# monoamine11231/Example-GUI-OpenCL-Raytracer

Measured on AMD Instinct MI355X. Metric: Mrays/s at 1920x1080 depth 4, aggregate over n_gpus; rays = path segments + shadow rays as the reference casts them (value_traced: only those the kernel really traces), higher is better.
Workload: dtype f32; 1 GPU; C2: scenes/render.map (regenerated), camera raypng.c:17-21, 1920x1080, depth 4, 2 soft-shadow samples, 4x256^2 textures + 4096x3072 skybox (procedural); frame=1920x1080, arithmetic=fast

## Files before the change

### example_gui_opencl_raytracer_amd/api.py

```python
from __future__ import annotations

import ctypes as C
import os

import numpy as np

HERE = os.path.dirname(os.path.abspath(__file__))
LIB_PATH = os.environ.get("CLWRAP_LIB") or os.path.join(HERE, "libopencl_wrap_hip.so")

MAX_KERNELS = 16
MAX_BUFFERS = 32

CL_DEVICE_TYPE_GPU = 1 << 2
CL_MEM_READ_WRITE = 1 << 0
CL_MEM_WRITE_ONLY = 1 << 1
CL_MEM_READ_ONLY = 1 << 2
CL_MEM_COPY_HOST_PTR = 1 << 5

SYMBOLS = [
    "cl_wrap_init", "cl_wrap_load_global_data", "cl_wrap_load_single_data", "cl_wrap_load_images",
    "cl_wrap_output", "cl_wrap_release",
    "clw_ext_set_depth", "clw_ext_get_depth", "clw_ext_set_strict", "clw_ext_set_fuse",
    "clw_ext_set_id_offset", "clw_ext_set_row_bands", "clw_ext_set_async", "clw_ext_sync", "clw_ext_set_stream",
    "clw_ext_timing_reset", "clw_ext_timing_get", "clw_ext_set_timing_every", "clw_ext_set_pipeline", "clw_ext_load_images_raw",
    "clw_ext_bind_device_buffer", "clw_ext_device_ptr", "clw_ext_set_debug_rgb",
    "clw_ext_enable_counters", "clw_ext_read_counters", "clw_ext_set_tile_sched", "clw_ext_read_tile_costs", "clw_ext_unit", "clw_ext_set_grid", "clw_ext_set_variant",
    "clw_ext_last_trace_flags", "clw_ext_set_shadow_through", "clw_ext_set_tpt", "clw_ext_invalidate_scene", "clw_ext_read_counters_ex", "clw_ext_unit_scene",
    "clw_host_perspective", "clw_host_write_png", "clw_host_write_png_rgba", "clw_host_read_png",
    "clw_host_free", "clw_ext_version",
    "clw_ext_set_supersample", "clw_ext_get_supersample",
    "clw_ext_set_sample_cameras", "clw_ext_get_sample_cameras", "clw_ext_set_lens", "clw_host_lens_cameras", "clw_host_shutter_cameras",
    "clw_ext_set_sphere_motion", "clw_ext_get_sample_times", "clw_host_sample_times", "clw_host_spheres_at",
    "clw_ext_set_adaptive", "clw_ext_get_adaptive", "clw_ext_read_refine_mask", "clw_host_refine_mask",
    "clw_ext_set_seed_offset", "clw_ext_get_seed_offset", "clw_ext_set_accumulate", "clw_ext_get_accumulated", "clw_ext_reset_accumulation",
    "clw_host_frame_seed", "clw_host_jitter_camera",
    "clw_ext_set_split", "clw_ext_get_split", "clw_ext_get_tpt", "clw_ext_read_tile_order", "clw_ext_unit_sched",
    "clw_ext_render_gbuffer", "clw_ext_read_gbuffer", "clw_ext_gbuffer_device_ptr", "clw_ext_pick",
    "clw_ext_get_grid", "clw_ext_set_grid_pair",
    "clw_host_overlay", "clw_ext_render_overlay", "clw_ext_read_overlay", "clw_ext_overlay_device_ptr", "clw_ext_unit_overlay",
    "clw_host_object_stats", "clw_host_merge_object_stats", "clw_ext_object_stats", "clw_ext_unit_object_stats",
    "clw_host_projection_rays", "clw_host_projection_tables", "clw_host_ortho_camera",
    "clw_ext_set_projection", "clw_ext_get_projection", "clw_ext_unit_projection",
    "clw_host_ao_dirs", "clw_host_ao_open", "clw_host_ao_resolve", "clw_ext_render_ao", "clw_ext_read_ao", "clw_ext_ao_device_ptr",
    "clw_ext_unit_ao_open", "clw_ext_unit_ao_resolve",
    "clw_host_cast_rays", "clw_host_occluded_rays", "clw_ext_cast_rays", "clw_ext_occluded_rays", "clw_ext_cast_rays_device",
]

GB_DEPTH, GB_ID, GB_NORMAL, GB_POINT, GB_ALBEDO, GB_ALL = 1, 2, 4, 8, 16, 31
ID_NONE = 0xFFFFFFFF
ID_SPHERE, ID_PLANE, ID_LIGHT = 0, 1, 2
TIMING_GBUFFER = 0x47425546
GB_CHANNELS = {"depth": (GB_DEPTH, np.float32, 1), "id": (GB_ID, np.uint32, 1), "normal": (GB_NORMAL, np.float32, 3),
               "point": (GB_POINT, np.float32, 3), "albedo": (GB_ALBEDO, np.float32, 3)}

OV_OUTLINE, OV_FILL, OV_EDGES, OV_ALL = 1, 2, 4, 7
TIMING_OVERLAY = 0x4F564C59

OBJECT_STAT = np.dtype([("id", np.uint32), ("pixels", np.uint32), ("x0", np.uint32), ("y0", np.uint32), ("x1", np.uint32), ("y1", np.uint32),
                        ("depth_min", np.float32), ("depth_max", np.float32), ("sum_x", np.uint64), ("sum_y", np.uint64)])
TIMING_OBJECTS = 0x4F424A53

PROJ_PERSPECTIVE, PROJ_ORTHO, PROJ_EQUIRECT = 0, 1, 2
PROJ_MODELS = {"perspective": PROJ_PERSPECTIVE, "ortho": PROJ_ORTHO, "equirect": PROJ_EQUIRECT}

AO_FILTER, AO_COMPOSE = 1, 2
AO_FRAME, AO_COUNTS = 0, 1
TIMING_AO = 0x414F5452
TIMING_AO_RESOLVE = 0x414F5253

RAY_QUERY = np.dtype([("origin", np.float32, 3), ("tmax", np.float32), ("dir", np.float32, 3), ("ignore", np.uint32)])
HIT = np.dtype([("t", np.float32), ("id", np.uint32), ("normal", np.float32, 3), ("point", np.float32, 3)])
CAST_SPHERES, CAST_PLANES, CAST_LIGHTS, CAST_KINDS, CAST_OPAQUE = 1, 2, 4, 7, 8
CAST_KIND_NAMES = {"sphere": CAST_SPHERES, "plane": CAST_PLANES, "light": CAST_LIGHTS}
TIMING_CAST = 0x43415354


def id_kind(ids):
    return np.asarray(ids, np.uint32) >> np.uint32(30)


def id_index(ids):
    return np.asarray(ids, np.uint32) & np.uint32(0x3FFFFFFF)


def make_id(kind, index):
    return (np.asarray(kind, np.uint32) << np.uint32(30)) | np.asarray(index, np.uint32)


def library_version() -> str:
    return load_library().clw_ext_version().decode()


def kernel_source_hash() -> str:
    return library_version().rsplit("kernels:", 1)[-1]


class cl_wrap(C.Structure):
    _fields_ = [
        ("impl", C.c_void_p),
        ("kernels_num", C.c_uint32),
        ("buffers_num", C.c_uint32 * MAX_KERNELS),
        ("buffers_ids", (C.c_uint32 * MAX_BUFFERS) * MAX_KERNELS),
        ("buffers", (C.c_void_p * MAX_BUFFERS) * MAX_KERNELS),
    ]


class clw_camera(C.Structure):
    _fields_ = [("im_corner", C.c_float * 3), ("origin", C.c_float * 3), ("up", C.c_float * 3),
                ("right", C.c_float * 3), ("w_factor", C.c_float), ("h_factor", C.c_float),
                ("width", C.c_uint32), ("height", C.c_uint32)]


class clw_sample_camera(C.Structure):
    _fields_ = [("im_corner", C.c_float * 3), ("origin", C.c_float * 3), ("up", C.c_float * 3), ("right", C.c_float * 3)]


class clw_pick(C.Structure):
    _fields_ = [("id", C.c_uint32), ("depth", C.c_float), ("point", C.c_float * 3), ("normal", C.c_float * 3), ("albedo", C.c_float * 3)]


class clw_overlay(C.Structure):
    _fields_ = [("flags", C.c_uint32), ("radius", C.c_uint32), ("outline_rgb", C.c_uint32), ("fill_rgb", C.c_uint32), ("fill_alpha", C.c_uint32),
                ("edge_rgb", C.c_uint32)]


class clw_ao(C.Structure):
    _fields_ = [("flags", C.c_uint32), ("rays", C.c_uint32), ("radius", C.c_float), ("strength", C.c_uint32)]

# ... 108 lines not shown
        L.clw_ext_get_accumulated.argtypes = [W]
        L.clw_ext_get_accumulated.restype = u32
        L.clw_ext_reset_accumulation.argtypes = [W]
        L.clw_host_frame_seed.argtypes = [u32]
        L.clw_host_frame_seed.restype = u32
        L.clw_host_jitter_camera.argtypes = [C.POINTER(clw_camera), u32, u32, C.POINTER(clw_camera)]
        L.clw_host_jitter_camera.restype = C.c_int
    if hasattr(L, "clw_ext_render_gbuffer") or not os.environ.get("CLWRAP_LIB"):
        L.clw_ext_render_gbuffer.argtypes = [W, u32]
        L.clw_ext_render_gbuffer.restype = u32
        L.clw_ext_read_gbuffer.argtypes = [W, u32, vp, u32]
        L.clw_ext_read_gbuffer.restype = u32
        L.clw_ext_gbuffer_device_ptr.argtypes = [W, u32]
        L.clw_ext_gbuffer_device_ptr.restype = vp
        L.clw_ext_pick.argtypes = [W, u32, u32, C.POINTER(clw_pick)]
        L.clw_ext_pick.restype = C.c_int
    if hasattr(L, "clw_ext_get_grid") or not os.environ.get("CLWRAP_LIB"):
        L.clw_ext_get_grid.argtypes = [W, C.POINTER(clw_grid_info)]
        L.clw_ext_get_grid.restype = C.c_int
        L.clw_ext_set_grid_pair.argtypes = [W, C.c_int]
    if hasattr(L, "clw_ext_render_overlay") or not os.environ.get("CLWRAP_LIB"):
        OV = C.POINTER(clw_overlay)
        L.clw_host_overlay.argtypes = [vp, vp, u32, u32, OV, vp, u32, vp]
        L.clw_host_overlay.restype = C.c_int
        L.clw_ext_render_overlay.argtypes = [W, OV, vp, u32]
        L.clw_ext_render_overlay.restype = u32
        L.clw_ext_read_overlay.argtypes = [W, vp, u32]
        L.clw_ext_read_overlay.restype = u32
        L.clw_ext_overlay_device_ptr.argtypes = [W]
        L.clw_ext_overlay_device_ptr.restype = vp
        L.clw_ext_unit_overlay.argtypes = [W, vp, vp, u32, u32, OV, vp, u32, vp]
        L.clw_ext_unit_overlay.restype = u32
    if hasattr(L, "clw_ext_object_stats") or not os.environ.get("CLWRAP_LIB"):
        RC, SM = C.POINTER(clw_rect), C.POINTER(clw_object_summary)
        L.clw_host_object_stats.argtypes = [vp, vp, u32, u32, u32, RC, vp, vp, u32, SM]
        L.clw_host_object_stats.restype = C.c_int
        L.clw_host_merge_object_stats.argtypes = [vp, u32, vp, u32, vp, u32]
        L.clw_host_merge_object_stats.restype = u32
        L.clw_ext_object_stats.argtypes = [W, RC, vp, u32, SM]
        L.clw_ext_object_stats.restype = C.c_int
        L.clw_ext_unit_object_stats.argtypes = [W, vp, vp, u32, u32, u32, RC, vp, vp, u32, SM]
        L.clw_ext_unit_object_stats.restype = C.c_int
    if hasattr(L, "clw_ext_set_projection") or not os.environ.get("CLWRAP_LIB"):
        CM, PR = C.POINTER(clw_camera), C.POINTER(clw_projection)
        L.clw_host_projection_rays.argtypes = [CM, PR, C.c_uint64, C.c_uint64, vp]
        L.clw_host_projection_rays.restype = C.c_int
        L.clw_host_projection_tables.argtypes = [CM, PR, vp, vp]
        L.clw_host_projection_tables.restype = C.c_int
        L.clw_host_ortho_camera.argtypes = [C.c_float * 3, C.c_float * 3, C.c_float, u32, u32, CM, PR]
        L.clw_host_ortho_camera.restype = C.c_int
        L.clw_ext_set_projection.argtypes = [W, PR]
        L.clw_ext_get_projection.argtypes = [W, PR]
        L.clw_ext_unit_projection.argtypes = [W, CM, PR, C.c_uint64, C.c_uint64, vp]
        L.clw_ext_unit_projection.restype = C.c_int
    if hasattr(L, "clw_ext_render_ao") or not os.environ.get("CLWRAP_LIB"):
        AO = C.POINTER(clw_ao)
        L.clw_host_ao_dirs.argtypes = [u32, vp]
        L.clw_host_ao_dirs.restype = C.c_int
        L.clw_host_ao_open.argtypes = [vp, vp, vp, u32, u32, u32, vp, u32, vp, u32, AO, vp, vp]
        L.clw_host_ao_open.restype = C.c_int
        L.clw_host_ao_resolve.argtypes = [vp, vp, vp, u32, u32, AO, vp]
        L.clw_host_ao_resolve.restype = C.c_int
        L.clw_ext_render_ao.argtypes = [W, AO]
        L.clw_ext_render_ao.restype = u32
        L.clw_ext_read_ao.argtypes = [W, u32, vp, u32]
        L.clw_ext_read_ao.restype = u32
        L.clw_ext_ao_device_ptr.argtypes = [W, u32]
        L.clw_ext_ao_device_ptr.restype = vp
        L.clw_ext_unit_ao_open.argtypes = [W, vp, vp, vp, u32, u32, u32, AO, vp]
        L.clw_ext_unit_ao_open.restype = u32
        L.clw_ext_unit_ao_resolve.argtypes = [W, vp, vp, vp, u32, u32, AO, vp]
        L.clw_ext_unit_ao_resolve.restype = u32
    if hasattr(L, "clw_ext_cast_rays") or not os.environ.get("CLWRAP_LIB"):
        L.clw_host_cast_rays.argtypes = [vp, u32, u32, vp, u32, vp, u32, vp, u32, vp]
        L.clw_host_cast_rays.restype = C.c_int
        L.clw_host_occluded_rays.argtypes = [vp, u32, u32, vp, u32, vp, u32, vp, u32, vp]
        L.clw_host_occluded_rays.restype = C.c_int
        L.clw_ext_cast_rays.argtypes = [W, vp, u32, u32, vp]
        L.clw_ext_cast_rays.restype = u32
        L.clw_ext_occluded_rays.argtypes = [W, vp, u32, u32, vp]
        L.clw_ext_occluded_rays.restype = u32
        L.clw_ext_cast_rays_device.argtypes = [W, vp, u32, u32, vp, vp]
        L.clw_ext_cast_rays_device.restype = u32
    L.clw_ext_unit.argtypes = [W, C.c_int, vp, u32, vp, u32, u32, u32]
    L.clw_ext_read_tile_costs.argtypes = [W, vp, u32]
    L.clw_ext_read_tile_costs.restype = u32
    L.clw_ext_set_split.argtypes = [W, C.c_int, C.c_int]
    L.clw_ext_get_split.argtypes = [W, C.POINTER(u32), C.POINTER(u32), C.POINTER(u32)]
    L.clw_ext_get_tpt.argtypes = [W, C.POINTER(u32), C.POINTER(u32), C.POINTER(u32)]
    L.clw_ext_read_tile_order.argtypes = [W, vp, u32, C.POINTER(u32)]
    L.clw_ext_read_tile_order.restype = u32
    L.clw_ext_unit_sched.argtypes = [W, vp, u32, u32, C.c_int, u32, u32, u32, u32, vp, u32]
    L.clw_ext_unit_sched.restype = u32
    L.clw_ext_read_counters.argtypes = [W, C.POINTER(C.c_uint64 * 8)]
    L.clw_ext_read_counters_ex.argtypes = [W, C.POINTER(C.c_uint64 * 32), u32]
    L.clw_ext_invalidate_scene.argtypes = [W]
    L.clw_ext_unit_scene.argtypes = [W, u32, C.c_int, vp, u32, vp, u32, u32]
    L.clw_host_perspective.argtypes = [C.c_float * 3, C.c_float * 3, C.c_float, C.c_float, u32, u32,
                                       C.POINTER(clw_camera)]
    L.clw_host_perspective.restype = C.c_int
    L.clw_host_write_png.argtypes = [C.c_char_p, vp, u32, u32]
    L.clw_host_write_png.restype = C.c_int
    L.clw_host_write_png_rgba.argtypes = [C.c_char_p, vp, u32, u32]
    L.clw_host_write_png_rgba.restype = C.c_int
    L.clw_host_read_png.argtypes = [C.c_char_p, C.POINTER(u32), C.POINTER(u32), C.POINTER(vp)]
    L.clw_host_read_png.restype = C.c_int
    L.clw_host_free.argtypes = [vp]
    L.clw_ext_version.restype = C.c_char_p
    _lib = L
    return L


def _ptr(a):
    if a is None:
        return None
    if isinstance(a, np.ndarray):
        return a.ctypes.data_as(C.c_void_p)
    return C.cast(a, C.c_void_p)


def perspective(origin, look, fov, focal, width, height) -> clw_camera:
    L = load_library()
    cam = clw_camera()
    ok = L.clw_host_perspective((C.c_float * 3)(*origin), (C.c_float * 3)(*look), fov, focal, width, height,
                                C.byref(cam))
    if not ok:
        raise ValueError("rgen_perspective rejects this camera (cpu_ray.c:58-63)")
    return cam


def lens_cameras(cam: clw_camera, aperture: float, focus: float, n: int) -> np.ndarray:
    out = np.zeros((max(int(n), 0) ** 2 or 1, 12), np.float32)
    if not load_library().clw_host_lens_cameras(C.byref(cam), aperture, focus, n, _ptr(out)):
        raise ValueError("clw_host_lens_cameras rejects these arguments (n in 2, 4, 8; aperture >= 0; focus > 0)")
    return out


def shutter_cameras(cam0: clw_camera, cam1: clw_camera, n: int) -> np.ndarray:
    out = np.zeros((max(int(n), 0) ** 2 or 1, 12), np.float32)
    if not load_library().clw_host_shutter_cameras(C.byref(cam0), C.byref(cam1), n, _ptr(out)):
        raise ValueError("clw_host_shutter_cameras rejects these arguments (n in 2, 4, 8; cameras of one size and one pair of factors)")
    return out


def sample_times(n: int) -> np.ndarray:
    out = np.zeros(max(int(n), 0) ** 2 or 1, np.float32)
    if not load_library().clw_host_sample_times(n, _ptr(out)):
        raise ValueError("clw_host_sample_times rejects this factor (n in 2, 4, 8)")
    return out


def spheres_at(spheres: np.ndarray, disp, t: float) -> np.ndarray:
    spheres = np.ascontiguousarray(spheres)
    assert spheres.dtype.itemsize == 96
    disp = np.ascontiguousarray(disp, np.float32).reshape(-1, 3)
    assert len(disp) == len(spheres)
    out = spheres.copy()
    if not load_library().clw_host_spheres_at(_ptr(spheres), len(spheres), _ptr(disp), float(t), _ptr(out)):
        raise ValueError("clw_host_spheres_at rejects these arguments")
    return out


def refine_mask(xrgb, width: int, rows: int, n: int, threshold: int) -> np.ndarray:
    xrgb = np.ascontiguousarray(xrgb, np.uint32).reshape(-1)
    width, rows, n = int(width), int(rows), int(n)
    if n not in (2, 4, 8) or width <= 0 or rows <= 0 or xrgb.size != width * rows:
# ... 33 lines not shown
def ao_dirs(rays: int) -> np.ndarray:
    out = np.empty((16, max(int(rays), 0), 4), np.float32)
    if not 0 <= int(rays) < 2 ** 32 or not load_library().clw_host_ao_dirs(int(rays), _ptr(out)):
        raise ValueError("clw_host_ao_dirs rejects this number of rays (1..32)")
    return out


def ao_open(point, normal, ids, width: int, rows: int, first_row: int, spheres, planes, ao: clw_ao, dirs=None) -> np.ndarray:
    width, rows = int(width), int(rows)
    point = np.ascontiguousarray(point, np.float32).reshape(-1)
    normal = np.ascontiguousarray(normal, np.float32).reshape(-1)
    ids = np.ascontiguousarray(ids, np.uint32).reshape(-1)
    if width <= 0 or rows <= 0 or ids.size != width * rows or point.size != 3 * ids.size or normal.size != 3 * ids.size:
        raise ValueError("clw_host_ao_open rejects these arguments (point and normal of 3, ids of 1 entry per pixel of width * rows)")
    if dirs is None:
        dirs = ao_dirs(ao.rays)
    dirs = np.ascontiguousarray(dirs, np.float32)
    ns, np_ = (0 if spheres is None else len(spheres)), (0 if planes is None else len(planes))
    out = np.empty(ids.size, np.uint8)
    if dirs.size != 64 * ao.rays or not load_library().clw_host_ao_open(_ptr(point), _ptr(normal), _ptr(ids), width, rows, int(first_row),
                                                                        _ptr(spheres) if ns else None, ns, _ptr(planes) if np_ else None, np_,
                                                                        C.byref(ao), _ptr(dirs), _ptr(out)):
        raise ValueError("clw_host_ao_open rejects these parameters (rays in 1..32, radius > 0, strength in 0..256, known flags)")
    return out


def ao_resolve(open_u8, ids, frame, width: int, rows: int, ao: clw_ao) -> np.ndarray:
    width, rows = int(width), int(rows)
    open_u8 = np.ascontiguousarray(open_u8, np.uint8).reshape(-1)
    ids = np.ascontiguousarray(ids, np.uint32).reshape(-1)
    if frame is not None:
        frame = np.ascontiguousarray(frame, np.uint32).reshape(-1)
    if width <= 0 or rows <= 0 or open_u8.size != width * rows or ids.size != width * rows or (frame is not None and frame.size != width * rows):
        raise ValueError("clw_host_ao_resolve rejects these arguments (counts, ids and frame of width * rows entries each)")
    out = np.empty(width * rows, np.uint32)
    if not load_library().clw_host_ao_resolve(_ptr(open_u8), _ptr(ids), _ptr(frame), width, rows, C.byref(ao), _ptr(out)):
        raise ValueError("clw_host_ao_resolve rejects these parameters (rays in 1..32, radius > 0, strength in 0..256, known flags, a frame with AO_COMPOSE)")
    return out


def cast_flags(kinds=("sphere", "plane"), opaque_only: bool = False) -> int:
    if isinstance(kinds, (int, np.integer)):
        flags = int(kinds)
    else:
        flags = 0
        for k in kinds:
            flags |= CAST_KIND_NAMES[k]
    return flags | (CAST_OPAQUE if opaque_only else 0)


def make_rays(origins, dirs, tmax=np.inf, ignore=None) -> np.ndarray:
    origins = np.asarray(origins, np.float32).reshape(-1, 3)
    rays = np.empty(origins.shape[0], RAY_QUERY)
    rays["origin"] = origins
    rays["dir"] = np.asarray(dirs, np.float32).reshape(-1, 3)
    rays["tmax"] = np.asarray(tmax, np.float32)
    rays["ignore"] = ID_NONE if ignore is None else np.asarray(ignore, np.uint32)
    return rays


def _cast_args(rays, spheres, planes, lights):
    rays = np.ascontiguousarray(rays, RAY_QUERY).reshape(-1)
    arrs = [None if a is None else np.ascontiguousarray(a) for a in (spheres, planes, lights)]
    counts = [0 if a is None else int(a.shape[0]) for a in arrs]
    return rays, arrs, counts


def cast_rays_host(rays, flags: int, spheres, planes, lights=None) -> np.ndarray:
    rays, (s, p, l), (ns, np_, nl) = _cast_args(rays, spheres, planes, lights)
    out = np.empty(rays.size, HIT)
    if not 0 <= int(flags) < 2 ** 32 or not load_library().clw_host_cast_rays(_ptr(rays), rays.size, int(flags), _ptr(s), ns, _ptr(p), np_, _ptr(l), nl, _ptr(out)):
        raise ValueError("clw_host_cast_rays rejects these arguments (at least one ray, fewer than 2^30, a kind bit and only CAST_* bits in flags)")
    return out


def occluded_rays_host(rays, flags: int, spheres, planes, lights=None) -> np.ndarray:
    rays, (s, p, l), (ns, np_, nl) = _cast_args(rays, spheres, planes, lights)
    out = np.empty(rays.size, np.uint8)
    if not 0 <= int(flags) < 2 ** 32 or not load_library().clw_host_occluded_rays(_ptr(rays), rays.size, int(flags), _ptr(s), ns, _ptr(p), np_, _ptr(l), nl, _ptr(out)):
        raise ValueError("clw_host_occluded_rays rejects these arguments (at least one ray, fewer than 2^30, a kind bit and only CAST_* bits in flags)")
    return out


def _rect(rect):
    if rect is None:
        return None
    if not isinstance(rect, clw_rect):
        rect = clw_rect(*(int(v) for v in rect))
    return C.byref(rect)


def _summary(s: clw_object_summary) -> dict:
    return dict(objects=int(s.objects), pixels=int(s.pixels), foreign=int(s.foreign))


def _object_table(call, first_capacity: int = 16384):
    s = clw_object_summary()
    out = np.zeros(first_capacity, OBJECT_STAT)
    if not call(_ptr(out), out.size, C.byref(s)):
        return None
    if s.objects > out.size:
        out = np.zeros(s.objects, OBJECT_STAT)
        if not call(_ptr(out), out.size, C.byref(s)):
            return None
    return out[:min(s.objects, out.size)].copy(), _summary(s)


def object_stats(ids, depth, width: int, rows: int, counts, first_row: int = 0, rect=None):
    ids = np.ascontiguousarray(ids, np.uint32).reshape(-1)
    width, rows = int(width), int(rows)
    if width <= 0 or rows <= 0 or ids.size != width * rows:
        raise ValueError("clw_host_object_stats rejects these arguments (an id channel of width * rows words)")
    if depth is not None:
        depth = np.ascontiguousarray(depth, np.float32).reshape(-1)
        if depth.size != ids.size:
            raise ValueError("clw_host_object_stats rejects these arguments (a depth channel of width * rows words)")
    counts = np.ascontiguousarray(counts, np.uint32).reshape(3)
    L = load_library()
    got = _object_table(lambda out, cap, s: L.clw_host_object_stats(_ptr(ids), _ptr(depth), width, rows, int(first_row), _rect(rect), _ptr(counts),
                                                                    out, cap, s))
    if got is None:
        raise ValueError("clw_host_object_stats rejects these arguments (an empty rectangle, more than 2^24 - 1 primitives, 2^30 pixels or more)")
    return got


def merge_object_stats(a, b) -> np.ndarray:
    a, b = np.ascontiguousarray(a, OBJECT_STAT).reshape(-1), np.ascontiguousarray(b, OBJECT_STAT).reshape(-1)
    out = np.zeros(a.size + b.size or 1, OBJECT_STAT)
    n = load_library().clw_host_merge_object_stats(_ptr(a), a.size, _ptr(b), b.size, _ptr(out), out.size)
    return out[:n].copy()


def projection(model, axis=None, ortho_width: float = 0.0, span=(360.0, 180.0)) -> clw_projection:
    p = clw_projection()
    p.model = PROJ_MODELS[model] if isinstance(model, str) else int(model)
    if axis is not None:
        p.axis[:] = [float(v) for v in axis]
    p.ortho_width, p.h_span, p.v_span = float(ortho_width), float(span[0]), float(span[1])
    return p


def projection_rays(cam: clw_camera, proj: clw_projection, id_begin: int = 0, id_end: int | None = None) -> np.ndarray:
    id_end = cam.width * cam.height if id_end is None else int(id_end)
    rays = np.zeros((max(id_end - int(id_begin), 0), 16), np.float32)
    if not load_library().clw_host_projection_rays(C.byref(cam), C.byref(proj), int(id_begin), id_end, _ptr(rays)):
        raise ValueError("clw_host_projection_rays rejects these arguments (model 0..2, a finite axis, ortho_width >= 0, spans in [0, 360] / "
                         "[0, 180], reserved 0, ids inside the frame)")
    return rays


def projection_tables(cam: clw_camera, proj: clw_projection):
    col, row = np.zeros((cam.width, 4), np.float32), np.zeros((cam.height, 4), np.float32)
    if not load_library().clw_host_projection_tables(C.byref(cam), C.byref(proj), _ptr(col), _ptr(row)):
        raise ValueError("clw_host_projection_tables rejects these arguments (an equirectangular projection the library accepts)")
    return col, row


def ortho_camera(origin, look, view_width: float, width: int, height: int):
    cam, proj = clw_camera(), clw_projection()
    if not load_library().clw_host_ortho_camera((C.c_float * 3)(*origin), (C.c_float * 3)(*look), float(view_width), int(width), int(height),
                                                C.byref(cam), C.byref(proj)):
        raise ValueError("clw_host_ortho_camera rejects these arguments (a finite look that is not vertical, view_width > 0, a frame)")
    return cam, proj


def frame_seed(f: int) -> int:
# ... 66 lines not shown

    def load_images(self, kernel_id, arg_id, *paths, mem_flags=CL_MEM_COPY_HOST_PTR):
        args = [C.c_char_p(p.encode()) for p in paths]
        self.L.cl_wrap_load_images(C.byref(self.w), C.c_uint32(kernel_id), C.c_uint32(arg_id),
                                   C.c_uint64(mem_flags), C.c_uint32(len(paths)), *args)

    def output(self, array_size, output_size, kernel_run_id, kernel_id, arg_id, host_output=None):
        self.L.cl_wrap_output(C.byref(self.w), array_size, output_size, kernel_run_id, kernel_id, arg_id,
                              _ptr(host_output))

    def release(self):
        if self.w.impl:
            self.L.cl_wrap_release(C.byref(self.w))

    def buffer_handle(self, kernel_id, arg_id) -> C.c_void_p:
        return C.c_void_p(self.w.buffers[kernel_id][arg_id])

    def set_depth(self, d): self.L.clw_ext_set_depth(C.byref(self.w), d)
    def get_depth(self): return self.L.clw_ext_get_depth(C.byref(self.w))
    def set_strict(self, s): self.L.clw_ext_set_strict(C.byref(self.w), int(s))
    def set_fuse(self, f): self.L.clw_ext_set_fuse(C.byref(self.w), int(f))
    def set_id_offset(self, first_id): self.L.clw_ext_set_id_offset(C.byref(self.w), first_id)
    def set_row_bands(self, stride, phase): self.L.clw_ext_set_row_bands(C.byref(self.w), stride, phase)
    def set_async(self, a): self.L.clw_ext_set_async(C.byref(self.w), int(a))
    def sync(self): self.L.clw_ext_sync(C.byref(self.w))
    def set_stream(self, s): self.L.clw_ext_set_stream(C.byref(self.w), C.c_void_p(s))
    def unit(self, op: int, rows: np.ndarray, out_cols: int, aux: int = 0) -> np.ndarray:
        rows = np.ascontiguousarray(rows, np.float32)
        out = np.zeros((rows.shape[0], out_cols), np.float32)
        self.L.clw_ext_unit(C.byref(self.w), op, _ptr(rows), rows.shape[1], _ptr(out), out_cols, rows.shape[0], aux)
        return out

    def read_tile_costs(self) -> np.ndarray:
        n = self.L.clw_ext_read_tile_costs(C.byref(self.w), None, 0)
        out = np.zeros(n, np.uint32)
        if n:
            self.L.clw_ext_read_tile_costs(C.byref(self.w), _ptr(out), n)
        return out

    def read_tile_order(self):
        cap = C.c_uint32()
        n = self.L.clw_ext_read_tile_order(C.byref(self.w), None, 0, C.byref(cap))
        out = np.zeros(n, np.uint32)
        if n:
            self.L.clw_ext_read_tile_order(C.byref(self.w), _ptr(out), n, C.byref(cap))
        return out, int(cap.value)

    def unit_sched(self, cost: np.ndarray, tpr: int, trows: int, clamp_outliers: int, per_share_cap: int, split_slots: int, min_quota: int,
                   max_lg: int) -> np.ndarray:
        cost = np.ascontiguousarray(cost, np.uint32).reshape(-1)
        assert cost.size == tpr * trows
        a = (int(tpr), int(trows), int(clamp_outliers), int(per_share_cap), int(split_slots), int(min_quota), int(max_lg))
        n = self.L.clw_ext_unit_sched(C.byref(self.w), _ptr(cost), *a, None, 0)
        out = np.zeros(n, np.uint32)
        self.L.clw_ext_unit_sched(C.byref(self.w), _ptr(cost), *a, _ptr(out), n)
        return out

    def get_split(self):
        v = [C.c_uint32() for _ in range(3)]
        self.L.clw_ext_get_split(C.byref(self.w), *[C.byref(x) for x in v])
        return tuple(int(x.value) for x in v)

    def get_tpt(self):
        v = [C.c_uint32() for _ in range(3)]
        self.L.clw_ext_get_tpt(C.byref(self.w), *[C.byref(x) for x in v])
        return tuple(int(x.value) for x in v)

    def set_split(self, slots=-1, min_quota=-1): self.L.clw_ext_set_split(C.byref(self.w), int(slots), int(min_quota))
    def set_shadow_through(self, f): self.L.clw_ext_set_shadow_through(C.byref(self.w), float(f))
    def set_grid(self, on): self.L.clw_ext_set_grid(C.byref(self.w), int(on))

    def get_grid(self):
        g = clw_grid_info()
        if not self.L.clw_ext_get_grid(C.byref(self.w), C.byref(g)):
            return None
        return dict(built=int(g.built), pair=int(g.pair), res=tuple(int(x) for x in g.res), ncells=int(g.ncells), pairs=int(g.pairs),
                    cell=tuple(float(x) for x in g.cell), gmin=tuple(float(x) for x in g.gmin), reg_pad=float(g.reg_pad))

    def set_grid_pair(self, on=-1):
        self.L.clw_ext_set_grid_pair(C.byref(self.w), int(on))
    def set_tile_sched(self, on): self.L.clw_ext_set_tile_sched(C.byref(self.w), int(on))
    def set_variant(self, v): self.L.clw_ext_set_variant(C.byref(self.w), int(v))
    def last_trace_flags(self): return int(self.L.clw_ext_last_trace_flags(C.byref(self.w)))
    def set_tpt(self, max_lanes=-1, min_paths=-1, pool_mb=-1): self.L.clw_ext_set_tpt(C.byref(self.w), int(max_lanes), int(min_paths), int(pool_mb))
    def timing_reset(self): self.L.clw_ext_timing_reset(C.byref(self.w))
    def set_timing_every(self, n): self.L.clw_ext_set_timing_every(C.byref(self.w), int(n))
    def set_pipeline(self, on): self.L.clw_ext_set_pipeline(C.byref(self.w), int(on))

    def timing_get(self, kernel_id):
        n, ms = C.c_uint32(), C.c_double()
        self.L.clw_ext_timing_get(C.byref(self.w), kernel_id, C.byref(n), C.byref(ms))
        return n.value, ms.value

    def load_images_raw(self, kernel_id, arg_id, rgba: np.ndarray):
        rgba = np.ascontiguousarray(rgba, np.uint8)
        layers, h, w, c = rgba.shape
        assert c == 4
        self.L.clw_ext_load_images_raw(C.byref(self.w), kernel_id, arg_id, _ptr(rgba), w, h, layers)

    def bind_device_buffer(self, kernel_id, arg_id, device_ptr, size):
        self.L.clw_ext_bind_device_buffer(C.byref(self.w), kernel_id, arg_id, C.c_void_p(device_ptr), size)

    def device_ptr(self, kernel_id, arg_id): return self.L.clw_ext_device_ptr(C.byref(self.w), kernel_id, arg_id)
    def set_debug_rgb(self, ptr): self.L.clw_ext_set_debug_rgb(C.byref(self.w), C.c_void_p(ptr))
    def set_supersample(self, n): self.L.clw_ext_set_supersample(C.byref(self.w), int(n))
    def get_supersample(self): return int(self.L.clw_ext_get_supersample(C.byref(self.w)))

    def set_seed_offset(self, s): self.L.clw_ext_set_seed_offset(C.byref(self.w), int(s) & 0xFFFFFFFF)
    def get_seed_offset(self): return int(self.L.clw_ext_get_seed_offset(C.byref(self.w)))
    def set_accumulate(self, max_frames, jitter=True): self.L.clw_ext_set_accumulate(C.byref(self.w), int(max_frames), int(jitter))
    def get_accumulated(self): return int(self.L.clw_ext_get_accumulated(C.byref(self.w)))
    def reset_accumulation(self): self.L.clw_ext_reset_accumulation(C.byref(self.w))

    def render_gbuffer(self, channels=GB_ALL) -> int:
        return int(self.L.clw_ext_render_gbuffer(C.byref(self.w), int(channels)))

    def _read_pass(self, read, dtype) -> np.ndarray:
        nbytes = int(read(None, 0))
        out = np.zeros(nbytes // np.dtype(dtype).itemsize, dtype)
        if nbytes:
            assert read(_ptr(out), nbytes) == nbytes
        return out

    def read_gbuffer(self, channel) -> np.ndarray:
        _, dtype, per = next(v for v in GB_CHANNELS.values() if v[0] == channel)
        out = self._read_pass(lambda p, cap: self.L.clw_ext_read_gbuffer(C.byref(self.w), int(channel), p, cap), dtype)
        return out.reshape(-1, 3) if per == 3 else out

    def gbuffer_device_ptr(self, channel):
        return self.L.clw_ext_gbuffer_device_ptr(C.byref(self.w), int(channel))

    def pick(self, x, y):
        p = clw_pick()
        return p if self.L.clw_ext_pick(C.byref(self.w), int(x), int(y), C.byref(p)) else None

    def render_overlay(self, style: clw_overlay, sel) -> int:
        sel = _selection(sel)
        return int(self.L.clw_ext_render_overlay(C.byref(self.w), C.byref(style), _ptr(sel) if sel.size else None, sel.size))

    def read_overlay(self) -> np.ndarray:
        return self._read_pass(lambda p, cap: self.L.clw_ext_read_overlay(C.byref(self.w), p, cap), np.uint32)

    def overlay_device_ptr(self):
        return self.L.clw_ext_overlay_device_ptr(C.byref(self.w))

    def unit_overlay(self, frame, ids, width: int, rows: int, style: clw_overlay, sel):
        frame = np.ascontiguousarray(frame, np.uint32).reshape(-1)
        ids = np.ascontiguousarray(ids, np.uint32).reshape(-1)
        assert frame.size == int(width) * int(rows) == ids.size
        sel = _selection(sel)
        out = np.empty(frame.size, np.uint32)
        n = self.L.clw_ext_unit_overlay(C.byref(self.w), _ptr(frame), _ptr(ids), int(width), int(rows), C.byref(style),
                                        _ptr(sel) if sel.size else None, sel.size, _ptr(out))
        return out if n == frame.size and n else None

    def object_stats(self, rect=None):
        return _object_table(lambda out, cap, s: self.L.clw_ext_object_stats(C.byref(self.w), _rect(rect), out, cap, s))

    def unit_object_stats(self, ids, depth, width: int, rows: int, counts, first_row: int = 0, rect=None):
        ids = np.ascontiguousarray(ids, np.uint32).reshape(-1)
        assert ids.size == int(width) * int(rows)
        if depth is not None:
            depth = np.ascontiguousarray(depth, np.float32).reshape(-1)
            assert depth.size == ids.size
        counts = np.ascontiguousarray(counts, np.uint32).reshape(3)
        return _object_table(lambda out, cap, s: self.L.clw_ext_unit_object_stats(C.byref(self.w), _ptr(ids), _ptr(depth), int(width), int(rows), int(first_row),
# ... 133 lines not shown
```

### example_gui_opencl_raytracer_amd/build.py

```python
from __future__ import annotations

import os
import shutil
import subprocess
import sys

HERE = os.path.dirname(os.path.abspath(__file__))
CSRC = os.path.join(HERE, "csrc")
ROOT_DIR = os.path.dirname(HERE)
OBJ = os.path.join(HERE, "build")
LIB = os.path.join(HERE, "libopencl_wrap_hip.so")
ARCH = "gfx950"

HIPCC = os.environ.get("HIPCC") or shutil.which("hipcc") or "/opt/rocm/bin/hipcc"
CC = os.environ.get("CC") or "gcc"

DEVICE_DEPS = ["whitted_trace.inc", "whitted_hit.inc", "whitted_shade.inc", "whitted_bounce.inc", "whitted_pop.inc", "whitted_tpt.inc", "whitted_terms.inc",
               "whitted_gbuffer.inc", "whitted_projection.inc", "whitted_ao.inc", "whitted_cast.inc", "whitted_overlay.inc", "whitted_objects.inc", "whitted_launch.inc", "whitted_launch.h", "whitted_params.h",
               "projection_host.h"]
SHIM_FLAGS = ["-O2", "-std=c++17", "-Wall"]
SHIM_DEPS = ["hip_wrap_impl.h", "whitted_params.h", "whitted_launch.h", "launch_plan.h", "scene_prep.h", "ao_host.h", "cast_host.h", "overlay_host.h", "objects_host.h", "projection_host.h",
             "png_codec.h", "../../include/opencl_wrap.h", "../../include/hip_wrap_ext.h"]
UNITS = [
    ("whitted_fast.hip", "hip", ["-O3", f"--offload-arch={ARCH}", "-fno-slp-vectorize", "-ffp-contract=off"], DEVICE_DEPS),
    ("whitted_strict.hip", "hip", ["-O3", f"--offload-arch={ARCH}", "-fno-slp-vectorize", "-ffp-contract=off"], DEVICE_DEPS),
    ("hip_wrap.cpp", "hip", SHIM_FLAGS, SHIM_DEPS),
    ("hip_wrap_passes.cpp", "hip", SHIM_FLAGS, SHIM_DEPS),
    ("scene_prep.c", "c", ["-O2", "-std=c99", "-ffp-contract=off", "-Wall", "-Wextra"], ["scene_prep.h"]),
    ("overlay_host.c", "c", ["-O2", "-std=c99", "-ffp-contract=off", "-Wall", "-Wextra"],
     ["overlay_host.h", "../../include/hip_wrap_ext.h", "../../include/opencl_wrap.h"]),
    ("ao_host.c", "c", ["-O2", "-std=c99", "-ffp-contract=off", "-Wall", "-Wextra", "-D_DEFAULT_SOURCE"],
     ["ao_host.h", "scene_prep.h", "../../include/hip_wrap_ext.h", "../../include/opencl_wrap.h"]),
    ("cast_host.c", "c", ["-O2", "-std=c99", "-ffp-contract=off", "-Wall", "-Wextra", "-D_DEFAULT_SOURCE"],
     ["cast_host.h", "scene_prep.h", "../../include/hip_wrap_ext.h", "../../include/opencl_wrap.h"]),
    ("objects_host.c", "c", ["-O2", "-std=c99", "-ffp-contract=off", "-Wall", "-Wextra"],
     ["objects_host.h", "../../include/hip_wrap_ext.h", "../../include/opencl_wrap.h"]),
    ("projection_host.c", "c", ["-O2", "-std=c99", "-ffp-contract=off", "-Wall", "-Wextra", "-D_DEFAULT_SOURCE"],
     ["projection_host.h", "../../include/hip_wrap_ext.h", "../../include/opencl_wrap.h"]),
    ("launch_plan.c", "c", ["-O2", "-std=c99", "-ffp-contract=off", "-Wall", "-Wextra"],
     ["launch_plan.h", "whitted_params.h", "../../include/hip_wrap_ext.h", "../../include/opencl_wrap.h"]),
    ("host_camera.c", "c", ["-O2", "-std=c99", "-ffp-contract=off", "-Wall", "-Wextra", "-D_DEFAULT_SOURCE"],
     ["../../include/hip_wrap_ext.h", "../../include/opencl_wrap.h"]),
    ("png_codec.c", "c", ["-O2", "-std=c99", "-D_DEFAULT_SOURCE", "-pthread", "-Wall", "-Wextra"], ["png_codec.h"]),
]


def kernel_source_hash() -> str:
    import hashlib
    h = hashlib.sha256()
    for f in sorted(set(DEVICE_DEPS + ["whitted_fast.hip", "whitted_strict.hip"])):
        h.update(f.encode() + b"\0" + open(os.path.join(CSRC, f), "rb").read())
    h.update(" ".join(UNITS[0][2]).encode())
    return h.hexdigest()[:16]


def _newer(target: str, deps) -> bool:
    if not os.path.exists(target):
        return True
    t = os.path.getmtime(target)
    return any(os.path.getmtime(d) > t for d in deps if os.path.exists(d))


def build(force: bool = False, verbose: bool = False, tag: str = "", extra_device_flags=()) -> str:
    os.makedirs(OBJ, exist_ok=True)
    objs = []
    lib = LIB if not tag else LIB.replace(".so", f"{tag}.so")
    for src, kind, flags, deps in UNITS:
        spath = os.path.join(CSRC, src)
        opath = os.path.join(OBJ, src.rsplit(".", 1)[0] + tag + ".o")
        if src.endswith(".hip"):
            flags = flags + list(extra_device_flags)
        if src == "hip_wrap.cpp":
            flags = flags + [f'-DWT_SOURCE_HASH="{kernel_source_hash()}{tag}"']
            deps = deps + DEVICE_DEPS + ["whitted_fast.hip", "whitted_strict.hip"]
        objs.append(opath)
        dpaths = [spath, __file__] + [os.path.normpath(os.path.join(CSRC, d)) for d in deps]
        if not force and not _newer(opath, dpaths):
            continue
        cmd = ([HIPCC] if kind == "hip" else [CC]) + flags + ["-fPIC", "-c", spath, "-o", opath]
        if verbose:
            print(" ".join(cmd), flush=True)
        subprocess.run(cmd, check=True)
    if force or _newer(lib, objs):
        cmd = [HIPCC, "-shared", "-o", lib] + objs + ["-lz", "-lpthread", "-Wl,-rpath,/opt/rocm/lib"]
        if verbose:
            print(" ".join(cmd), flush=True)
        subprocess.run(cmd, check=True)
    if not tag:
        exe = os.path.join(ROOT_DIR, "tools", "raybench")
        src = os.path.join(ROOT_DIR, "tools", "raybench.c")
        if force or _newer(exe, [src, lib]):
            cmd = [CC, "-O2", "-std=c99", "-D_DEFAULT_SOURCE", "-DCL_TARGET_OPENCL_VERSION=300", "-Wall", "-I", os.path.join(ROOT_DIR, "include"),
                   src, "-o", exe, "-L", HERE, "-lopencl_wrap_hip", "-Wl,-rpath,$ORIGIN/../example_gui_opencl_raytracer_amd",
                   "-Wl,-rpath,/opt/rocm/lib"]
            if verbose:
                print(" ".join(cmd), flush=True)
            subprocess.run(cmd, check=True)
    return lib


if __name__ == "__main__":
    print(build(force="--force" in sys.argv, verbose=True))
```

### example_gui_opencl_raytracer_amd/csrc/hip_wrap.cpp

```cpp
#include "hip_wrap_impl.h"

using namespace clw;

namespace clw {
[[noreturn]] void die(const char* fmt, ...) {
    va_list ap;
    va_start(ap, fmt);
    printf("ERROR:\t");
    vprintf(fmt, ap);
    printf("\n");
    va_end(ap);
    fflush(stdout);
    exit(1);
}
}

namespace {

constexpr size_t COUNTER_WORDS = CLW_NUM_COUNTERS + 16 * (size_t)CLW_STAMP_SHARDS;
constexpr size_t GRID_MAX_PAIRS = (size_t)1 << 25;

bool same_bits(const std::vector<float>& a, const float* b, size_t n) {
    return a.size() == n && (n == 0 || !memcmp(a.data(), b, n * sizeof(float)));
}
// ... 363 lines not shown
        }
        I->tables_in_flight = true;
        plan.P.ss_times = I->d_motion; plan.P.ss_disp = I->d_motion + 64;
    }
}

void bind_accumulation(Impl* I, wt_plan_out& plan) {
    Impl::Accum& A = I->acc;
    if (!plan.fused || A.frame < 0) return;
    if (A.pixels != (size_t)plan.out_pixels || !A.sum) {
        if (A.frame != 0) die("Couldn't run the kernel");
        if (A.sum) { finish(I); (void)hipFree(A.sum); A.sum = nullptr; }
        HIP_OK(hipMalloc((void**)&A.sum, (size_t)plan.out_pixels * 12), "Couldn't allocate device memory");
        A.pixels = plan.out_pixels;
    }
    wait_tables_fence(I);
    I->tables_in_flight = true;
    plan.P.acc_sum = A.sum;
}

void bind_counters(Impl* I, wt_plan_out& plan) {
    if (!plan.need_counters) return;
    if (!I->d_counters) {
        HIP_OK(hipMalloc((void**)&I->d_counters, COUNTER_WORDS * sizeof(unsigned long long)), "Couldn't allocate device memory");
        HIP_OK(hipMemsetAsync(I->d_counters, 0, COUNTER_WORDS * sizeof(unsigned long long), I->stream), "Couldn't allocate device memory");
    }
    plan.P.counters = I->d_counters;
}

void classify_blocks(Impl* I, wt_plan_out& plan) {
    whitted_params& P = plan.P;
    const uint32_t ow = P.width >> P.ss_lg, orows = P.rows >> P.ss_lg;
    Impl::Adaptive& A = I->adapt;
    if (A.w != ow || A.rows != orows || A.ss != plan.ss || !A.mask) {
        A.free_all();
        HIP_OK(hipMalloc((void**)&A.mask, (size_t)plan.trows * plan.tpr), "Couldn't allocate device memory");
        HIP_OK(hipMalloc((void**)&A.order, (size_t)plan.grid * 4), "Couldn't allocate device memory");
        HIP_OK(hipMalloc((void**)&A.count, 8 * WT_LIST_COUNT_STRIDE * 4), "Couldn't allocate device memory");
        A.w = ow; A.rows = orows; A.ss = plan.ss;
    }
    wait_tables_fence(I);
    HIP_OK(hipMemsetAsync(A.count, 0, 8 * WT_LIST_COUNT_STRIDE * 4, I->stream), "Couldn't run the kernel");
    if (wt_fast_launch_classify(P.out, ow, orows, 3u - P.ss_lg, (unsigned)I->adaptive, A.mask, A.order, A.count, plan.per_share, I->stream) != hipSuccess)
        die("Couldn't run the kernel");
    I->tables_in_flight = true;
    A.blocks = plan.trows * plan.tpr;
    P.tile_order = A.order; P.list_count = A.count;
}

bool bind_tile_order(Impl* I, Impl::Sched& S, wt_plan_out& plan, const Strip* strip) {
    whitted_params& P = plan.P;
    if (!strip) S.last_rd = -1;
    if (!plan.use_order) return false;
    const size_t ntiles = (size_t)plan.trows * plan.tpr;
    if (S.w != P.width || S.rows != P.rows || S.cap != plan.per_share_cap || S.ss != plan.ss || !S.cost[0]) {
        S.free_all();
        for (int i = 0; i < 2; i++) {
            HIP_OK(hipMalloc((void**)&S.cost[i], ntiles * 4), "Couldn't allocate device memory");
            HIP_OK(hipMalloc((void**)&S.order[i], (size_t)plan.grid * 4), "Couldn't allocate device memory");
            HIP_OK(hipEventCreateWithFlags(&S.built[i], hipEventDisableTiming), "Couldn't create a timing event");
        }
        HIP_OK(hipEventCreateWithFlags(&S.traced, hipEventDisableTiming), "Couldn't create a timing event");
        S.w = P.width; S.rows = P.rows; S.cap = plan.per_share_cap; S.ss = plan.ss; S.o.wr = 0;
    }
    const int wr = S.o.wr;
    P.tile_cost = S.cost[wr];
    const wt_order_choice c = wt_order_choose(&S.o);
    if (c.wait_wr) HIP_OK(hipStreamWaitEvent(I->stream, S.built[wr], 0), "Couldn't run the kernel");
    if (c.wait_rd) HIP_OK(hipStreamWaitEvent(I->stream, S.built[c.rd], 0), "Couldn't run the kernel");
    P.tile_order = c.rd >= 0 ? S.order[c.rd] : nullptr;
    if (!strip) S.last_rd = c.rd;
    const bool have_cams = plan.n_cams != 0;
    const bool changed = !S.o.sig_valid || !same_raygen(plan.sig, S.sig) || S.sig_depth != I->depth || S.sig_scene != I->scene_generation || S.sig_has_cams != have_cams ||
                         (have_cams && memcmp(&S.sig_cams, &plan.cam_table, sizeof plan.cam_table)) || !same_bits(S.sig_motion, plan.motion_table, plan.motion_floats);
    if (P.cost_sum) HIP_OK(hipMemsetAsync(S.cost[wr], 0, ntiles * 4, I->stream), "Couldn't run the kernel");
    if (changed) {
        S.sig_motion.assign(plan.motion_table, plan.motion_table + plan.motion_floats);
        S.sig_has_cams = have_cams; if (have_cams) S.sig_cams = plan.cam_table;
        S.sig = plan.sig; S.sig_depth = I->depth; S.sig_scene = I->scene_generation;
    }
    return wt_order_rebuild(&S.o, changed, plan.flags & WT_F_GRID) != 0;
}

void bind_tail_pool(Impl* I, wt_plan_out& plan) {
    if (!plan.tail_wanted) return;
    whitted_params& P = plan.P;
    const size_t need = (size_t)plan.tpt_slice * 4u * plan.tpt_nslots;
    if (I->tpt_pool_bytes != need) {
        finish(I);
        if (I->d_tpt_pool) (void)hipFree(I->d_tpt_pool);
        if (I->d_tpt_flags) (void)hipFree(I->d_tpt_flags);
        I->d_tpt_pool = nullptr; I->d_tpt_flags = nullptr; I->tpt_pool_bytes = 0;
        if (hipMalloc((void**)&I->d_tpt_pool, need) == hipSuccess && hipMalloc((void**)&I->d_tpt_flags, plan.tpt_nslots * 4u) == hipSuccess) {
            HIP_OK(hipMemsetAsync(I->d_tpt_flags, 0, plan.tpt_nslots * 4u, I->stream), "Couldn't allocate device memory");
            I->tpt_pool_bytes = need;
        } else {
            (void)hipGetLastError();
            if (I->d_tpt_pool) (void)hipFree(I->d_tpt_pool);
            I->d_tpt_pool = nullptr;
        }
    }
    if (I->tpt_pool_bytes) { P.tpt_pool = I->d_tpt_pool; P.tpt_flags = I->d_tpt_flags; P.tpt_jump = I->d_tpt_jump; }
    else P.tpt_slice_words = P.tpt_cap = P.tpt_slots = P.tpt_max = P.tpt_min = 0u;
}

void sort_tile_costs(Impl* I, Impl::Sched& S, const wt_plan_out& plan, bool rebuild) {
    const int wr = S.o.wr;
    if (rebuild) {
        if (!I->sched_stream) HIP_OK(hipStreamCreateWithFlags(&I->sched_stream, hipStreamNonBlocking), "Couldn't create a command queue for the given device");
        HIP_OK(hipEventRecord(S.traced, I->stream), "Couldn't run the kernel");
        HIP_OK(hipStreamWaitEvent(I->sched_stream, S.traced, 0), "Couldn't run the kernel");
        if (wt_fast_launch_sched(S.cost[wr], S.order[wr], plan.tpr, plan.trows, plan.per_share, (plan.flags & WT_F_GRID) ? 1u : 0u, plan.per_share_cap,
                                 plan.split ? I->split_slots : 0u, I->split_min_quota, plan.split_max_lg, I->sched_stream) != hipSuccess)
            die("Couldn't run the kernel");
        HIP_OK(hipEventRecord(S.built[wr], I->sched_stream), "Couldn't run the kernel");
    }
    wt_order_launched(&S.o, rebuild);
}

bool trace_launch(cl_wrap* w, Impl* I, cl_uint kid, size_t array_size, const Strip* strip, TracePass pass) {
    Buffer* rays = rays_of(w, I, kid);
    const uint32_t total = total_of(I->kernels[kid]);
    Buffer* out = buffer_arg(w, kid, 10);
    ensure_allocated(I, out);
    if (wt_plan_range(array_size, total, out->size) == 0) return false;
    prepare_bound_scene(w, I, kid);

    wt_plan_in in;
    wt_plan_out plan;
    plan_input(I, rays, array_size, total, out->size, strip, pass, in);
    wt_plan(&in, &plan);
    if (plan.status == WT_PLAN_REFUSED) die("%s", plan.message);
    if (plan.samples_decided) keep_samples(I, plan);
    if (plan.status == WT_PLAN_NONE) return false;

    Impl::Sched& S = I->scheds[strip ? strip->slot : 0];
    bind_buffers(w, I, kid, rays, out, plan);
    bind_tables(I, plan);
    bind_accumulation(I, plan);
    bind_counters(I, plan);
    bool sort = false;
    if (pass == PASS_REFINE) classify_blocks(I, plan);
    else if (plan.P.tiled) sort = bind_tile_order(I, S, plan, strip);
    I->last_trace_flags = plan.flags;
    bind_tail_pool(I, plan);
    LaunchTimer t(I, kid, pass == PASS_PLAIN);
    hipError_t e = WT_LAUNCH(I, trace)(&plan.P, plan.flags, plan.grid, plan.dyn_lds, I->stream);
    if (e != hipSuccess) die("Couldn't run the kernel");
    t.done();
    if (plan.P.tile_cost) sort_tile_costs(I, S, plan, sort);
    return true;
}

void check_modes(const Impl* I, const Buffer* rays, bool accumulating) {
    wt_plan_in in{};
    char message[200];
    in.fuse = I->fuse; in.supersample = I->supersample; in.adaptive = I->adaptive; in.aperture = I->aperture;
    in.n_cams = (uint32_t)I->cams.size(); in.n_disp = (uint32_t)I->motion_disp.size();
    in.rays_generated = 1 + (int32_t)I->proj.model;
    if (rays) { in.rays_generated = rays->gen_valid ? 1 + (int32_t)I->proj.model : 0; in.rays_exposed = rays->exposed; }
    if (wt_plan_mode_check(&in, accumulating, message)) die("%s", message);
}

void run_accumulated(cl_wrap* w, Impl* I, cl_uint kid, size_t array_size, const Strip* strip) {
    Kernel& k = I->kernels[kid];
    Buffer* rays = rays_of(w, I, kid);
    check_modes(I, rays, true);
    Impl::Accum& A = I->acc;
    Impl::AccKey key;
    key.gen = rays->gen;
    key.total = total_of(k); key.n_out = (uint64_t)array_size;
    key.depth = I->depth; key.strict = I->strict; key.fuse = I->fuse; key.ss = I->supersample; key.max_frames = I->acc_max; key.jitter = I->acc_jitter;
    key.through = I->through; key.seed = I->seed_offset;
    const cl_uint args[6] = {1, 2, 3, 8, 9, 10};
    key.buf[0] = rays; key.size[0] = rays->size;
    for (int a = 0; a < 6; a++) { Buffer* b = buffer_arg(w, kid, args[a]); ensure_allocated(I, b); key.buf[1 + a] = b; key.dptr[1 + a] = b->dptr; key.size[1 + a] = b->size; }
    for (int a = 0; a < 3; a++) key.counts[a] = read_count(k, 4 + (cl_uint)a);
    { const Buffer* t = key.buf[4]; const Buffer* s = key.buf[5]; key.img[0] = t->w; key.img[1] = t->h; key.img[2] = t->layers; key.img[3] = s->w; key.img[4] = s->h; }
    key.epoch = A.epoch;
    if (!A.key_valid || !same_acc_key(key, A.key)) { A.K = 0; A.key = key; A.key_valid = true; }
    if (A.K >= (uint32_t)I->acc_max) return;
    A.frame = (int)A.K;
    const bool launched = trace_launch(w, I, kid, array_size, strip, PASS_PLAIN);
    A.frame = -1;
    if (launched) A.K++;
}

void run_raytracer(cl_wrap* w, Impl* I, cl_uint kid, size_t array_size, const Strip* strip = nullptr) {
    I->adapt.blocks = 0;
    if (I->acc_max > 0) { run_accumulated(w, I, kid, array_size, strip); return; }
    I->acc.key_valid = false;
    if (I->adaptive < 0) { trace_launch(w, I, kid, array_size, strip, PASS_PLAIN); return; }
    check_modes(I, nullptr, false);
    LaunchTimer t(I, kid);
    trace_launch(w, I, kid, array_size, strip, PASS_BASE);
    trace_launch(w, I, kid, array_size, strip, PASS_REFINE);
    t.done();
}

bool pipelined_output(cl_wrap* w, Impl* I, size_t array_size, size_t output_size, cl_uint kid, cl_uint out_kernel,
                      cl_int out_arg, void* host_output) {
    if (!I->pipeline || I->async || !host_output || !I->fuse || I->counting || I->debug_rgb || (I->variant & WT_V_LINEAR_IDS)) return false;
    if (I->acc_max > 0) return false;
    if (I->proj.model != CLW_PROJ_PERSPECTIVE) return false;
    if (I->adaptive >= 0) return false;
    if (out_kernel != kid || out_arg != 10 || !is_registered(w, kid, 10)) return false;
    Buffer* rays = find_rays(w, I, kid);
    uint32_t total;
    if (!rays || !rays->gen_valid || rays->exposed || !find_total(I->kernels[kid], total)) return false;
    const RaygenArgs& g = rays->gen;
    Buffer* out = (Buffer*)w->buffers[kid][10];
    const uint64_t n = g.n_items;
    if (g.band_stride > 1 || g.id_offset % g.width != 0 || n % g.width != 0) return false;
    if (array_size < n || total < n || out->size < n * 4 || output_size != n * 4) return false;
    const uint32_t rows = (uint32_t)(n / g.width);
    if (n * 4 < (16u << 20) || rows < 4 * 64 || I->depth > WT_SHALLOW_LEVELS + 1) return false;
    ensure_allocated(I, out);

    const int nch = Impl::MAX_CHUNKS;
    const uint32_t base = rows / nch / 64 * 64;
    if (!I->copy_stream) {
        HIP_OK(hipStreamCreateWithFlags(&I->copy_stream, hipStreamNonBlocking), "Couldn't create a command queue for the given device");
        for (hipEvent_t& e : I->chunk_done) HIP_OK(hipEventCreateWithFlags(&e, hipEventDisableTiming), "Couldn't create a timing event");
    }
    for (int c = 0; c < nch; c++) {
        Strip st{(uint32_t)c * base, c == nch - 1 ? rows - (uint32_t)c * base : base, 1 + c};
        run_raytracer(w, I, kid, array_size, &st);
        HIP_OK(hipEventRecord(I->chunk_done[c], I->stream), "Couldn't run the kernel");
    }
    for (int c = 0; c < nch; c++) {
// ... 192 lines not shown
    use_device(I);
    precheck_buffer_arg(wrap, kernel_id, arg_id);
    std::vector<uint8_t> all;
    uint32_t W = 0, H = 0;
    va_list vars;
    va_start(vars, image_num);
    for (cl_uint i = 0; i < image_num; i++) {
        const char* filename = va_arg(vars, const char*);
        uint32_t w = 0, h = 0;
        uint8_t* px = nullptr;
        int rc = wpng_read_rgba(filename, &w, &h, &px);
        switch (rc) {
            case WPNG_OK: break;
            case WPNG_ERR_OPEN: va_end(vars); die("Cannot open file \"%s\"", filename);
            case WPNG_ERR_NOT_PNG: va_end(vars); die("\"%s\" is not a PNG file", filename);
            case WPNG_ERR_FORMAT: va_end(vars); die("\"%s\" must have a depth of 8 bits and be RGB", filename);
            default: va_end(vars); die("Could not decode PNG file \"%s\" (code %d)", filename, rc);
        }
        if (i == 0) { W = w; H = h; all.reserve((size_t)w * h * 4 * image_num); }
        if (w != W || h != H) { free(px); va_end(vars); die("All images must have same dimensions"); }
        all.insert(all.end(), px, px + (size_t)w * h * 4);
        free(px);
    }
    va_end(vars);
    install_images(wrap, I, kernel_id, arg_id, all.data(), W, H, image_num);
}

void cl_wrap_output(cl_wrap* wrap, size_t array_size, size_t output_size, cl_uint kernel_run_id,
                    cl_uint kernel_id, cl_int arg_id, void* host_output) {
    Impl* I = impl_of(wrap);
    use_device(I);
    check_kernel_id(wrap, kernel_run_id);
    if (I->kernels[kernel_run_id].kind == K_RAYGEN) run_raygen(wrap, I, kernel_run_id, array_size);
    else if (pipelined_output(wrap, I, array_size, output_size, kernel_run_id, kernel_id, arg_id, host_output)) return;
    else run_raytracer(wrap, I, kernel_run_id, array_size);

    if (!host_output) {
        if (!I->async) finish(I);
        return;
    }
    check_kernel_id(wrap, kernel_id);
    if (arg_id < 0 || arg_id >= __MAX_BUFFERS || !is_registered(wrap, kernel_id, (cl_uint)arg_id))
        die("Failed to transfer device memory to host");
    Buffer* b = (Buffer*)wrap->buffers[kernel_id][arg_id];
    materialise_rays(I, b);
    ensure_allocated(I, b);
    if (output_size > b->size) die("Failed to transfer device memory to host");
    if (output_size &&
        hipMemcpyAsync(host_output, b->dptr, output_size, hipMemcpyDeviceToHost, I->stream) != hipSuccess)
        die("Failed to transfer device memory to host");
    finish(I);
}

void cl_wrap_release(cl_wrap* wrap) {
    if (!wrap || !wrap->impl) return;
    Impl* I = (Impl*)wrap->impl;
    use_device(I);
    (void)hipStreamSynchronize(I->stream);
    for (Buffer* b : I->live) {
        if (b->owned && b->dptr) (void)hipFree(b->dptr);
        delete b;
    }
    if (I->d_geom) (void)hipFree(I->d_geom);
    if (I->d_ptex) (void)hipFree(I->d_ptex);
    if (I->d_counters) (void)hipFree(I->d_counters);
    if (I->d_tpt_pool) (void)hipFree(I->d_tpt_pool);
    if (I->d_tpt_flags) (void)hipFree(I->d_tpt_flags);
    if (I->d_tpt_jump) (void)hipFree(I->d_tpt_jump);
    if (I->d_cams) (void)hipFree(I->d_cams);
    if (I->d_motion) (void)hipFree(I->d_motion);
    if (I->acc.sum) (void)hipFree(I->acc.sum);
    I->gb.release();
    I->ov.release();
    I->obj.release();
    I->ao.release();
    I->cast.free_buffers();
    I->ptab.free_all();
    I->adapt.free_all();
    if (I->tables_fence) (void)hipEventDestroy(I->tables_fence);
    for (uint32_t* q : {I->d_grid_start, I->d_grid_items, I->d_grid_box}) if (q) (void)hipFree(q);
    if (I->d_grid_geom) (void)hipFree(I->d_grid_geom);
    if (I->sched_stream) (void)hipStreamSynchronize(I->sched_stream);
    for (auto& sc : I->scheds) sc.free_all();
    if (I->sched_stream) (void)hipStreamDestroy(I->sched_stream);
    if (I->copy_stream) (void)hipStreamDestroy(I->copy_stream);
    for (hipEvent_t e : I->chunk_done) if (e) (void)hipEventDestroy(e);
    for (auto& t : I->timing) { (void)hipEventDestroy(t.start); (void)hipEventDestroy(t.stop); }
    for (auto& p : I->free_events) { (void)hipEventDestroy(p.first); (void)hipEventDestroy(p.second); }
    if (I->own_stream) (void)hipStreamDestroy(I->own_stream);
    delete I;
    memset(wrap, 0, sizeof *wrap);
}

void clw_ext_set_depth(cl_wrap* wrap, int depth) {
    if (depth < 1 || depth > CLW_MAX_DEPTH) die("Trace depth must be in [1, %d]", CLW_MAX_DEPTH);
    impl_of(wrap)->depth = depth;
}
int clw_ext_get_depth(const cl_wrap* wrap) { return impl_of(wrap)->depth; }
void clw_ext_set_strict(cl_wrap* wrap, int strict) { impl_of(wrap)->strict = strict ? 1 : 0; }
void clw_ext_set_fuse(cl_wrap* wrap, int fuse) { impl_of(wrap)->fuse = fuse ? 1 : 0; }
void clw_ext_set_id_offset(cl_wrap* wrap, uint64_t first_id) { impl_of(wrap)->id_offset = first_id; }
void clw_ext_set_row_bands(cl_wrap* wrap, uint32_t stride, uint32_t phase) {
    if (stride == 0 || phase >= stride) die("Row bands need 0 <= phase < stride");
    Impl* I = impl_of(wrap);
    I->band_stride = stride; I->band_phase = phase;
}
void clw_ext_set_async(cl_wrap* wrap, int async) { impl_of(wrap)->async = async ? 1 : 0; }
void clw_ext_sync(cl_wrap* wrap) { Impl* I = impl_of(wrap); use_device(I); finish(I); }
void clw_ext_set_stream(cl_wrap* wrap, void* hip_stream) {
    Impl* I = impl_of(wrap);
    hipStream_t next = hip_stream ? (hipStream_t)hip_stream : I->own_stream;
    if (next != I->stream && I->tables_in_flight) {
        use_device(I);
        if (!I->tables_fence) HIP_OK(hipEventCreateWithFlags(&I->tables_fence, hipEventDisableTiming), "Couldn't create a timing event");
        HIP_OK(hipEventRecord(I->tables_fence, I->stream), "Couldn't run the kernel");
        I->tables_fence_pending = true; I->tables_in_flight = false;
    }
    I->stream = next;
}
void clw_ext_unit(cl_wrap* wrap, int op, const float* in, uint32_t stride_in, float* out, uint32_t stride_out, uint32_t n,
                  uint32_t aux) {
    Impl* I = impl_of(wrap);
    use_device(I);
    if (n == 0) return;
    float *din = nullptr, *dout = nullptr;
    HIP_OK(hipMalloc((void**)&din, (size_t)n * stride_in * 4), "Couldn't allocate device memory");
    HIP_OK(hipMalloc((void**)&dout, (size_t)n * stride_out * 4), "Couldn't allocate device memory");
    HIP_OK(hipMemcpy(din, in, (size_t)n * stride_in * 4, hipMemcpyHostToDevice), "Couldn't transfer the data from host to the device");
    HIP_OK(hipMemset(dout, 0, (size_t)n * stride_out * 4), "Couldn't allocate device memory");
    HIP_OK(hipDeviceSynchronize(), "The device kernel failed");
    hipError_t e = WT_LAUNCH(I, unit)(op, din, dout, n, stride_in, stride_out, aux, I->stream);
    if (e != hipSuccess) die("Couldn't run the kernel");
    finish(I);
    HIP_OK(hipMemcpy(out, dout, (size_t)n * stride_out * 4, hipMemcpyDeviceToHost), "Failed to transfer device memory to host");
    (void)hipFree(din); (void)hipFree(dout);
}
void clw_ext_unit_scene(cl_wrap* wrap, cl_uint kernel_id, int op, const float* in, uint32_t stride_in, float* out,
                        uint32_t stride_out, uint32_t n) {
    Impl* I = impl_of(wrap);
    use_device(I);
    check_kernel_id(wrap, kernel_id);
    if (I->kernels[kernel_id].kind != K_RAYTRACER) die("Wrong kernel ID given");
    if (n == 0) return;
    whitted_params P{};
    int flags = 0;
    size_t dyn_lds = 0;
    bind_scene(wrap, I, kernel_id, P, flags, dyn_lds);
    P.depth = I->depth;
    float *din = nullptr, *dout = nullptr;
    HIP_OK(hipMalloc((void**)&din, (size_t)n * stride_in * 4), "Couldn't allocate device memory");
    HIP_OK(hipMalloc((void**)&dout, (size_t)n * stride_out * 4), "Couldn't allocate device memory");
    HIP_OK(hipMemcpy(din, in, (size_t)n * stride_in * 4, hipMemcpyHostToDevice), "Couldn't transfer the data from host to the device");
    HIP_OK(hipMemset(dout, 0, (size_t)n * stride_out * 4), "Couldn't allocate device memory");
    HIP_OK(hipDeviceSynchronize(), "The device kernel failed");
    hipError_t e = WT_LAUNCH(I, unit_scene)(&P, flags, op, din, dout, n, stride_in, stride_out, dyn_lds, I->stream);
    if (e != hipSuccess) die("Couldn't run the kernel");
    finish(I);
    HIP_OK(hipMemcpy(out, dout, (size_t)n * stride_out * 4, hipMemcpyDeviceToHost), "Failed to transfer device memory to host");
    (void)hipFree(din); (void)hipFree(dout);
}
uint32_t clw_ext_read_tile_costs(cl_wrap* wrap, uint32_t* out, uint32_t capacity) {
    Impl* I = impl_of(wrap);
    use_device(I);
    finish(I);
    const Impl::Sched& S = I->scheds[0];
    if (!S.cost[0]) return 0;
    uint32_t n = ((S.rows + 7) / 8) * ((S.w + 7) / 8);
    if (out && capacity >= n) HIP_OK(hipMemcpy(out, S.cost[S.o.wr ^ 1], (size_t)n * 4, hipMemcpyDeviceToHost), "Failed to transfer device memory to host");
    return n;
}
uint32_t clw_ext_read_tile_order(cl_wrap* wrap, uint32_t* out, uint32_t capacity, uint32_t* per_share_cap) {
    Impl* I = impl_of(wrap);
    use_device(I);
    finish(I);
    if (I->sched_stream) HIP_OK(hipStreamSynchronize(I->sched_stream), "The device kernel failed");
    const Impl::Sched& S = I->scheds[0];
    if (per_share_cap) *per_share_cap = 0;
    if (S.last_rd < 0 || !S.order[S.last_rd]) return 0;
    if (per_share_cap) *per_share_cap = S.cap;
    const uint32_t n = 8u * S.cap;
    if (out && capacity >= n) HIP_OK(hipMemcpy(out, S.order[S.last_rd], (size_t)n * 4, hipMemcpyDeviceToHost), "Failed to transfer device memory to host");
    return n;
}
uint32_t clw_ext_unit_sched(cl_wrap* wrap, const uint32_t* cost, uint32_t tpr, uint32_t trows, int clamp_outliers, uint32_t per_share_cap,
                            uint32_t split_slots, uint32_t min_quota, uint32_t max_lg, uint32_t* out, uint32_t out_words) {
    Impl* I = impl_of(wrap);
    use_device(I);
    if (tpr == 0 || trows == 0 || tpr > 0xFFFu || trows > 0xFFFu || max_lg > 4u) die("clw_ext_unit_sched: %u x %u tiles, max_lg %u", tpr, trows, max_lg);
    const uint32_t per_share = ((trows + 7u) / 8u) * tpr;
    if (per_share_cap < per_share) die("clw_ext_unit_sched: per_share_cap %u is below the %u tiles of a share", per_share_cap, per_share);
    const uint64_t words = 8ull * ((uint64_t)per_share << max_lg) + 8ull * per_share_cap;
    if (words > 0xFFFFFFFFull) die("clw_ext_unit_sched: the table is too large");
    if (!out || out_words < words) return (uint32_t)words;
    const size_t ntiles = (size_t)trows * tpr;
    unsigned *dcost = nullptr, *dorder = nullptr;
    HIP_OK(hipMalloc((void**)&dcost, ntiles * 4), "Couldn't allocate device memory");
    HIP_OK(hipMalloc((void**)&dorder, (size_t)words * 4), "Couldn't allocate device memory");
    HIP_OK(hipMemcpy(dcost, cost, ntiles * 4, hipMemcpyHostToDevice), "Couldn't transfer the data from host to the device");
    std::vector<uint32_t> fill((size_t)words, CLW_SCHED_SENTINEL);
    HIP_OK(hipMemcpy(dorder, fill.data(), (size_t)words * 4, hipMemcpyHostToDevice), "Couldn't transfer the data from host to the device");
    HIP_OK(hipDeviceSynchronize(), "The device kernel failed");
    if (wt_fast_launch_sched(dcost, dorder, tpr, trows, per_share, clamp_outliers ? 1u : 0u, per_share_cap, split_slots, min_quota, max_lg, I->stream) != hipSuccess)
        die("Couldn't run the kernel");
    finish(I);
    HIP_OK(hipMemcpy(out, dorder, (size_t)words * 4, hipMemcpyDeviceToHost), "Failed to transfer device memory to host");
    (void)hipFree(dcost); (void)hipFree(dorder);
    return (uint32_t)words;
}
void clw_ext_set_split(cl_wrap* wrap, int slots, int min_quota) {
    Impl* I = impl_of(wrap);
    if (slots >= 0) I->split_slots = (unsigned)std::max(1, slots);
    if (min_quota >= 0) I->split_min_quota = (unsigned)min_quota;
    for (auto& sc : I->scheds) sc.reset();
}
void clw_ext_get_split(const cl_wrap* wrap, uint32_t* slots, uint32_t* min_quota, uint32_t* extra_per_share) {
    const Impl* I = impl_of(wrap);
    if (slots) *slots = I->split_slots;
    if (min_quota) *min_quota = I->split_min_quota;
    if (extra_per_share) *extra_per_share = WT_SPLIT_EXTRA_PER_SHARE;
}
void clw_ext_set_shadow_through(cl_wrap* wrap, float factor) { impl_of(wrap)->through = factor; }
void clw_ext_set_grid(cl_wrap* wrap, int on) { impl_of(wrap)->use_grid = on ? 1 : 0; }
int clw_ext_get_grid(const cl_wrap* wrap, clw_grid_info* out) {
    const Impl* I = impl_of(wrap);
    if (!I->d_geom || !out) return 0;
    memset(out, 0, sizeof *out);
    if (!I->grid_ok) return 1;
    out->built = 1; out->pair = I->grid_pair ? 1 : 0;
    out->ncells = I->grid.ncells; out->pairs = (uint64_t)I->grid_pairs; out->reg_pad = I->grid.reg_pad;
    for (int a = 0; a < 3; a++) { out->res[a] = I->grid.res[a]; out->cell[a] = I->grid.cell[a]; out->gmin[a] = I->grid.gmin[a]; }
    return 1;
}
void clw_ext_set_grid_pair(cl_wrap* wrap, int on) {
    if (on < -1 || on > 1) die("The grid's shadow walk must be -1 (default), 0 (single) or 1 (paired)");
    Impl* I = impl_of(wrap);
    I->grid_pair_req = on;
    I->prep_s = I->prep_p = I->prep_l = nullptr;
    I->acc.epoch++;
}
void clw_ext_set_tile_sched(cl_wrap* wrap, int on) { Impl* I = impl_of(wrap); I->sched = on ? 1 : 0; for (auto& sc : I->scheds) sc.reset(); }
void clw_ext_set_variant(cl_wrap* wrap, int variant) { impl_of(wrap)->variant = variant; }
int clw_ext_last_trace_flags(cl_wrap* wrap) { return impl_of(wrap)->last_trace_flags; }
void clw_ext_set_tpt(cl_wrap* wrap, int max_lanes, int min_paths, int pool_mb) {
    Impl* I = impl_of(wrap);
    if (max_lanes >= 0) I->tpt_max = (unsigned)std::min(max_lanes, 64);
    if (min_paths >= 0) I->tpt_min = (unsigned)min_paths;
    if (pool_mb >= 0) I->tpt_pool_mb = (unsigned)pool_mb;
}
void clw_ext_get_tpt(const cl_wrap* wrap, uint32_t* max_lanes, uint32_t* min_paths, uint32_t* pool_mb) {
    const Impl* I = impl_of(wrap);
    if (max_lanes) *max_lanes = I->tpt_max;
    if (min_paths) *min_paths = I->tpt_min;
    if (pool_mb) *pool_mb = I->tpt_pool_mb;
}
void clw_ext_set_debug_rgb(cl_wrap* wrap, void* p) { impl_of(wrap)->debug_rgb = (float*)p; }
void clw_ext_set_supersample(cl_wrap* wrap, int n) {
    if (n != 1 && n != 2 && n != 4 && n != 8) die("The supersampling factor must be 1, 2, 4 or 8");
    impl_of(wrap)->supersample = n;
}
int clw_ext_get_supersample(const cl_wrap* wrap) { return impl_of(wrap)->supersample; }
void clw_ext_set_adaptive(cl_wrap* wrap, int threshold) {
    if (threshold < -1 || threshold > 256) die("The adaptive supersampling threshold must be in [0, 256], or -1 for off");
    impl_of(wrap)->adaptive = threshold;
}
int clw_ext_get_adaptive(const cl_wrap* wrap) { return impl_of(wrap)->adaptive; }
uint32_t clw_ext_read_refine_mask(cl_wrap* wrap, uint8_t* out, uint32_t cap) {
    Impl* I = impl_of(wrap);
    use_device(I);
    finish(I);
    const uint32_t n = I->adapt.blocks;
    if (out && n && cap >= n) HIP_OK(hipMemcpy(out, I->adapt.mask, n, hipMemcpyDeviceToHost), "Failed to transfer device memory to host");
    return n;
}
void clw_ext_set_sample_cameras(cl_wrap* wrap, const clw_sample_camera* cams, uint32_t count) {
    Impl* I = impl_of(wrap);
    if (cams && count) I->cams.assign(cams, cams + count); else I->cams.clear();
    I->aperture = 0.0f;
}
uint32_t clw_ext_get_sample_cameras(const cl_wrap* wrap, clw_sample_camera* out, uint32_t cap) {
    const Impl* I = impl_of(wrap);
    const uint32_t n = (uint32_t)I->cams_used.size();
    if (out && n && cap >= n) memcpy(out, I->cams_used.data(), (size_t)n * sizeof(clw_sample_camera));
    return n;
}
void clw_ext_set_sphere_motion(cl_wrap* wrap, const float* disp, uint32_t ns, const float* times, uint32_t count) {
    Impl* I = impl_of(wrap);
    bool any = false;
    if (disp) for (size_t i = 0; i < 3 * (size_t)ns; i++) {
        if (!std::isfinite(disp[i])) die("Moving spheres: displacement %u of sphere %u is not finite", (unsigned)(i % 3), (unsigned)(i / 3));
        any |= disp[i] != 0.0f;
    }
    if (times) for (uint32_t k = 0; k < count; k++) if (!std::isfinite(times[k])) die("Moving spheres: sample time %u is not finite", (unsigned)k);
    I->motion_disp.clear(); I->motion_times.clear(); I->motion_explicit_times = false;
    if (!any) return;
    I->motion_disp.assign(disp, disp + 3 * (size_t)ns);
    if (times) { I->motion_times.assign(times, times + count); I->motion_explicit_times = true; }
}
uint32_t clw_ext_get_sample_times(const cl_wrap* wrap, float* out, uint32_t cap) {
    const Impl* I = impl_of(wrap);
    const uint32_t n = (uint32_t)I->times_used.size();
    if (out && n && cap >= n) memcpy(out, I->times_used.data(), (size_t)n * sizeof(float));
    return n;
}
void clw_ext_set_lens(cl_wrap* wrap, float aperture, float focus) {
    if (!(aperture >= 0.0f) || !std::isfinite(aperture)) die("The lens aperture must be a finite number >= 0");
    if (!(focus > 0.0f) || !std::isfinite(focus)) die("The lens focus distance must be a finite number > 0");
    Impl* I = impl_of(wrap);
    I->aperture = aperture; I->focus = focus;
    I->cams.clear();
}

void clw_ext_set_seed_offset(cl_wrap* wrap, uint32_t s) { impl_of(wrap)->seed_offset = s; }
uint32_t clw_ext_get_seed_offset(const cl_wrap* wrap) { return impl_of(wrap)->seed_offset; }
void clw_ext_set_accumulate(cl_wrap* wrap, int max_frames, int jitter) {
    if (max_frames < 0 || max_frames > 65536) die("Frame accumulation: the number of frames must be in [0, 65536] (0 = off)");
    if (jitter != 0 && jitter != 1) die("Frame accumulation: jitter must be 0 or 1");
    Impl* I = impl_of(wrap);
    I->acc_max = max_frames; I->acc_jitter = jitter;
}
uint32_t clw_ext_get_accumulated(cl_wrap* wrap) { Impl* I = impl_of(wrap); return I->acc_max > 0 ? I->acc.K : 0u; }
void clw_ext_reset_accumulation(cl_wrap* wrap) { impl_of(wrap)->acc.epoch++; }

void clw_ext_set_projection(cl_wrap* wrap, const clw_projection* proj) {
    Impl* I = impl_of(wrap);
    clw_projection p{};
// ... 142 lines not shown
```

### example_gui_opencl_raytracer_amd/csrc/hip_wrap_impl.h

```cpp
#ifndef HIP_WRAP_IMPL_H
#define HIP_WRAP_IMPL_H
#include <hip/hip_runtime.h>

#include <algorithm>
#include <cstdarg>
#include <cstdint>
#include <cstdio>
#include <cstdlib>
#include <cmath>
#include <cstring>
#include <string>
#include <vector>

#include "../../include/hip_wrap_ext.h"
#include "ao_host.h"
#include "cast_host.h"
#include "launch_plan.h"
#include "objects_host.h"
#include "overlay_host.h"
#include "png_codec.h"
#include "projection_host.h"
#include "scene_prep.h"
#include "whitted_launch.h"
#include "whitted_params.h"

namespace clw {

[[noreturn]] void die(const char* fmt, ...);

#define HIP_OK(call, what)                                                        \
    do {                                                                          \
        hipError_t e_ = (call);                                                   \
        if (e_ != hipSuccess) die("%s (%s)", what, hipGetErrorString(e_));        \
    } while (0)

enum KernelKind { K_RAYGEN = 0, K_RAYTRACER = 1 };

typedef wt_raygen RaygenArgs;

struct Buffer {
    void* dptr = nullptr;
    size_t size = 0;
    bool owned = true;
    bool lazy = false;
    bool image = false;
    uint32_t w = 0, h = 0, layers = 0;
    std::vector<uint8_t> shadow;
    bool gen_valid = false;
    bool exposed = false;
    bool gen_materialised = false;
    RaygenArgs gen{};
    clw_projection gen_proj{};
};

struct ArgValue {
    bool set = false;
    size_t size = 0;
    uint8_t bytes[32] = {0};
};

struct Kernel {
    KernelKind kind;
    std::string name;
    ArgValue values[__MAX_BUFFERS];
};

struct TimingEntry { hipEvent_t start, stop; cl_uint kernel; };

struct Impl {
    int device = 0;
    hipStream_t own_stream = nullptr;
    hipStream_t stream = nullptr;
    std::vector<Kernel> kernels;
    std::vector<Buffer*> live;
    int depth = 15;
    int strict = 0;
    int fuse = 1;
    int async = 0;
    int variant = 0;
    int last_trace_flags = -1;
    int counting = 0;
    float through = 0.8f;
    int stamps = 0;
    uint64_t id_offset = 0;
    uint32_t band_stride = 1, band_phase = 0;
    int supersample = 1;
    float* debug_rgb = nullptr;
    int adaptive = -1;
    struct Adaptive {
        uint8_t* mask = nullptr; uint32_t* order = nullptr; uint32_t* count = nullptr;
        uint32_t w = 0, rows = 0; int ss = 0;
        uint32_t blocks = 0;
        void free_all() {
            for (void* q : {(void*)mask, (void*)order, (void*)count}) if (q) (void)hipFree(q);
            mask = nullptr; order = nullptr; count = nullptr; w = rows = 0; ss = 0;
        }
    } adapt;
    std::vector<clw_sample_camera> cams;
    float aperture = 0.0f, focus = 1.0f;
    std::vector<clw_sample_camera> cams_used;
    float* d_cams = nullptr;
    wt_cam_table cams_dev{}; bool cams_dev_valid = false;
    hipEvent_t tables_fence = nullptr; bool tables_fence_pending = false, tables_in_flight = false;
// ... 53 lines not shown
    struct Objects {
        uint32_t* ids = nullptr; float* depth = nullptr;
        uint32_t n = 0;
        void* table = nullptr; void* result = nullptr;
        uint32_t slots = 0;
        void alloc_buffers(uint32_t items) {
            HIP_OK(hipMalloc((void**)&ids, (size_t)items * 4), "Couldn't allocate device memory");
            HIP_OK(hipMalloc((void**)&depth, (size_t)items * 4), "Couldn't allocate device memory");
        }
        void free_buffers() { if (ids) (void)hipFree(ids); if (depth) (void)hipFree(depth); ids = nullptr; depth = nullptr; n = 0; }
        void size_table(uint32_t count) {
            if (slots == count) return;
            free_table();
            HIP_OK(hipMalloc(&table, 16 + (size_t)count * sizeof(clw_object_stat)), "Couldn't allocate device memory");
            HIP_OK(hipMalloc(&result, sizeof(clw_object_summary) + (size_t)count * sizeof(clw_object_stat)), "Couldn't allocate device memory");
            slots = count;
        }
        void free_table() { if (table) (void)hipFree(table); if (result) (void)hipFree(result); table = result = nullptr; slots = 0; }
        void release() { free_buffers(); free_table(); }
    } obj;
    struct AO : RangePass {
        float* point = nullptr; float* normal = nullptr; uint32_t* ids = nullptr; uint8_t* open = nullptr; uint32_t* frame = nullptr;
        float* dirs = nullptr; uint32_t dirs_K = 0;
        void alloc_buffers(uint32_t items) {
            HIP_OK(hipMalloc((void**)&point, (size_t)items * 12), "Couldn't allocate device memory");
            HIP_OK(hipMalloc((void**)&normal, (size_t)items * 12), "Couldn't allocate device memory");
            HIP_OK(hipMalloc((void**)&ids, (size_t)items * 4), "Couldn't allocate device memory");
            HIP_OK(hipMalloc((void**)&open, (size_t)items), "Couldn't allocate device memory");
            HIP_OK(hipMalloc((void**)&frame, (size_t)items * 4), "Couldn't allocate device memory");
        }
        void free_buffers() {
            for (void* q : {(void*)point, (void*)normal, (void*)ids, (void*)open, (void*)frame}) if (q) (void)hipFree(q);
            point = normal = nullptr; ids = nullptr; open = nullptr; frame = nullptr; n = 0; written = 0;
        }
        void release() { free_buffers(); if (dirs) (void)hipFree(dirs); dirs = nullptr; drop_done(); }
    } ao;
    struct Cast {
        void* rays = nullptr; void* hits = nullptr; uint8_t* blocked = nullptr;
        uint32_t cap = 0;
        void free_buffers() {
            for (void* q : {rays, hits, (void*)blocked}) if (q) (void)hipFree(q);
            rays = hits = nullptr; blocked = nullptr; cap = 0;
        }
    } cast;
    const Buffer *prep_s = nullptr, *prep_p = nullptr, *prep_l = nullptr;
    uint32_t prep_ns = 0, prep_np = 0, prep_nl = 0;
    float* d_geom = nullptr; size_t geom_f4 = 0;
    float* d_ptex = nullptr;
    bool have_lpt = false;
    uint64_t scene_generation = 0;
    uint32_t *d_grid_start = nullptr, *d_grid_items = nullptr, *d_grid_box = nullptr;
    float* d_grid_geom = nullptr;
    wprep_grid grid{}; bool grid_ok = false, grid_pair = false; int use_grid = 1;
    size_t grid_pairs = 0;
    int grid_pair_req = -1;
    unsigned long long* d_counters = nullptr;
    int sched = 1;
    struct Sched {
        unsigned* cost[2] = {nullptr, nullptr}; unsigned* order[2] = {nullptr, nullptr};
        hipEvent_t built[2] = {nullptr, nullptr};
        wt_order_state o{};
        hipEvent_t traced = nullptr;
        uint32_t w = 0, rows = 0, cap = 0;
        int ss = 1;
        int last_rd = -1;
        RaygenArgs sig{}; int sig_depth = 0; uint64_t sig_scene = 0;
        wt_cam_table sig_cams{}; bool sig_has_cams = false;
        std::vector<float> sig_motion;
        void reset() { o.have[0] = o.have[1] = 0; o.sig_valid = 0; o.newest = 0; last_rd = -1; }
        void free_all() {
            for (int i = 0; i < 2; i++) {
                if (cost[i]) (void)hipFree(cost[i]);
                if (order[i]) (void)hipFree(order[i]);
                if (built[i]) (void)hipEventDestroy(built[i]);
                cost[i] = order[i] = nullptr; built[i] = nullptr;
            }
            if (traced) { (void)hipEventDestroy(traced); traced = nullptr; }
            reset();
        }
    };
    hipStream_t sched_stream = nullptr;
    static constexpr int MAX_CHUNKS = 4;
    Sched scheds[1 + MAX_CHUNKS];
    int pipeline = 1;
    hipStream_t copy_stream = nullptr;
    hipEvent_t chunk_done[MAX_CHUNKS] = {nullptr, nullptr, nullptr, nullptr};
    std::vector<TimingEntry> timing;
    unsigned occ_tiles_per_depth = WT_OCC_TILES_PER_DEPTH;
    uint32_t* d_tpt_pool = nullptr; uint32_t* d_tpt_flags = nullptr; size_t tpt_pool_bytes = 0;
    uint32_t* d_tpt_jump = nullptr;
    unsigned tpt_max = WT_TPT_MAX_LANES, tpt_min = WT_TPT_MIN_PATHS, tpt_pool_mb = WT_TPT_POOL_MB;
    int tpt_clock = 0;
    unsigned split_slots = WT_SPLIT_SLOTS;
    unsigned split_min_quota = WT_SPLIT_MIN_QUOTA;
    bool timing_on = false;
    uint32_t timing_every = 1, timing_tick = 0;
    std::vector<std::pair<hipEvent_t, hipEvent_t>> free_events;
};

inline Impl* impl_of(const cl_wrap* w) {
    if (!w || !w->impl) die("cl_wrap is not initialised");
    return (Impl*)w->impl;
}

inline void use_device(Impl* I) {
    int cur = -1;
    if (hipGetDevice(&cur) != hipSuccess || cur != I->device) HIP_OK(hipSetDevice(I->device), "Cannot select the HIP device");
}

inline bool is_registered(const cl_wrap* w, cl_uint kernel_id, cl_uint arg_id) {
    for (cl_uint i = 0; i < w->buffers_num[kernel_id]; i++)
        if (w->buffers_ids[kernel_id][i] == arg_id) return true;
    return false;
}

inline Buffer* lookup_handle(Impl* I, const void* handle) {
    for (Buffer* b : I->live)
        if ((const void*)b == handle) return b;
    return nullptr;
}

inline void ensure_allocated(Impl* I, Buffer* b) {
    (void)I;
    if (b->dptr || b->size == 0) return;
    HIP_OK(hipMalloc(&b->dptr, b->size), "Couldn't allocate device memory");
    b->lazy = false;
}

inline std::pair<hipEvent_t, hipEvent_t> take_events(Impl* I) {
    if (!I->free_events.empty()) {
        auto p = I->free_events.back();
        I->free_events.pop_back();
        return p;
    }
    hipEvent_t a, b;
    HIP_OK(hipEventCreate(&a), "Couldn't create a timing event");
    HIP_OK(hipEventCreate(&b), "Couldn't create a timing event");
    return {a, b};
}

struct LaunchTimer {
    Impl* I; cl_uint kernel; bool on; std::pair<hipEvent_t, hipEvent_t> ev;
    LaunchTimer(Impl* I_, cl_uint k, bool wanted = true) : I(I_), kernel(k), on(wanted && I_->timing_on && I_->timing.size() < 16384 && (I_->timing_tick++ % I_->timing_every) == 0) {
        if (on) { ev = take_events(I); HIP_OK(hipEventRecord(ev.first, I->stream), "Couldn't run the kernel"); }
    }
    void done() {
        if (on) { HIP_OK(hipEventRecord(ev.second, I->stream), "Couldn't run the kernel"); I->timing.push_back({ev.first, ev.second, kernel}); }
    }
};

inline void finish(Impl* I) {
    hipError_t e = hipStreamSynchronize(I->stream);
    if (e != hipSuccess) { printf("%d\n", (int)e); die("The device kernel failed"); }
}

template <class T> struct DeviceTemp {
    T* p = nullptr;
    explicit DeviceTemp(size_t bytes) { HIP_OK(hipMalloc((void**)&p, bytes), "Couldn't allocate device memory"); }
    DeviceTemp(const void* host, size_t bytes) {
        if (!host) return;
        HIP_OK(hipMalloc((void**)&p, bytes), "Couldn't allocate device memory");
        HIP_OK(hipMemcpy(p, host, bytes, hipMemcpyHostToDevice), "Couldn't transfer the data from host to the device");
    }
    ~DeviceTemp() { if (p) (void)hipFree(p); }
    DeviceTemp(const DeviceTemp&) = delete;
    DeviceTemp& operator=(const DeviceTemp&) = delete;
// ... 53 lines not shown
```

### example_gui_opencl_raytracer_amd/csrc/launch_plan.c

```c
#include "launch_plan.h"

#include <stdarg.h>
#include <stdio.h>
#include <string.h>

static int refuse(char* message, const char* fmt, ...) {
    va_list ap;
    va_start(ap, fmt);
    vsnprintf(message, 200, fmt, ap);
    va_end(ap);
    return WT_PLAN_REFUSED;
}

static uint64_t min_u64(uint64_t a, uint64_t b) { return a < b ? a : b; }

static void camera_of(const wt_raygen* g, clw_camera* c) {
    memcpy(c->im_corner, g->corner, 12); memcpy(c->origin, g->origin, 12); memcpy(c->up, g->up, 12); memcpy(c->right, g->right, 12);
    c->w_factor = g->w_factor; c->h_factor = g->h_factor; c->width = g->width; c->height = g->height;
}

static inline uint64_t range_of(uint64_t array_size, uint32_t total, uint64_t out_size) {
    const uint64_t rounded = (array_size + WT_LAUNCH_ROUND - 1) / WT_LAUNCH_ROUND * WT_LAUNCH_ROUND;
    const uint64_t n = min_u64(rounded, total);
    return min_u64(n, out_size / 4);
// ... 171 lines not shown
    const int moving = in->n_disp != 0;
    if (moving) {
        if (ss == 1) return o->status = refuse(o->message, "Moving spheres need samples: a displacement table with supersampling factor 1 (clw_ext_set_supersample / CLWRAP_SUPERSAMPLE)");
        if (in->explicit_times && in->n_times != (uint32_t)(ss * ss))
            return o->status = refuse(o->message, "Moving spheres: %u sample times, but supersampling factor %d needs %d", (unsigned)in->n_times, ss, ss * ss);
        if (in->n_disp != 3 * (uint64_t)in->ns)
            return o->status = refuse(o->message, "Moving spheres: the displacement table is for %u spheres, the scene has %u", (unsigned)(in->n_disp / 3), (unsigned)in->ns);
        if ((flags & WT_F_GRID) || in->ns > WT_GRID_MIN_SPHERES)
            return o->status = refuse(o->message, "Moving spheres: scenes of more than %u spheres (the uniform grid is built for one set of centres) are not supported", (unsigned)WT_GRID_MIN_SPHERES);
        if (flags & WT_F_GEOM_LDS) {
            if (in->geom_f4 + in->ns <= WT_GEOM_LDS_MAX_F4) dyn_lds += in->ns * 16u;
            else { flags &= ~WT_F_GEOM_LDS; dyn_lds = 0; }
        }
    }
    o->fused = in->fuse && in->rays_generated && !in->rays_exposed && !projection;
    if (o->fused) {
        const int st = plan_fused(in, o, who, moving);
        if (st != WT_PLAN_LAUNCH) return o->status = st;
    } else {
        if (ss > 1) return o->status = refuse(o->message, "%s needs the fused raygen + trace launch (CLWRAP_FUSE=1, rays generated by this library and not rewritten)", who);
        if ((uint64_t)P->n_items * 64 > in->rays_size) return o->status = refuse(o->message, "Couldn't run the kernel");
        o->out_pixels = P->n_items;
        P->id_offset = in->id_offset;
        P->width = 1; P->height = 1;
        P->unit_dirs = (in->rays_generated && !in->rays_exposed && !projection && in->ns <= WT_GRID_MIN_SPHERES) ? 1u : 0u;
        if (in->rays_generated) {
            P->id_offset = in->gen.id_offset; P->width = in->gen.width; P->height = in->gen.height;
            P->band_stride = in->gen.band_stride; P->band_phase = in->gen.band_phase;
        } else if (in->band_stride > 1) return o->status = refuse(o->message, "Row bands need a raygen launch");
        flags |= WT_F_RAYS;
    }
    if (in->depth > WT_SHALLOW_LEVELS + 1) flags |= WT_F_DEEP;
    if (!(flags & WT_F_GEOM_LDS)) P->vis = 0;
    if (in->counting || in->stamps || in->tpt_clock) {
        if (in->counting) flags |= WT_F_COUNT;
        P->tpt_clock = in->tpt_clock ? 1u : 0u;
        o->need_counters = 1;
    }
    if (P->tiled) {
        o->trows = (P->rows + 7) / 8; o->tpr = (P->width + 7) / 8;
        o->per_share = ((o->trows + 7) / 8) * o->tpr;
        o->per_share_cap = o->per_share;
    }
    const uint32_t base_grid = grid_of(P);
    o->grid = base_grid;
    if ((flags & WT_F_DEEP) && !in->strict && (uint64_t)base_grid >= (uint64_t)in->occ_tiles_per_depth * (unsigned)in->depth && !(in->variant & WT_V_NO_OCC))
        flags |= WT_F_OCC;
    if ((flags & WT_F_DEEP) && !(flags & WT_F_OCC) && !(in->variant & WT_V_NO_TAIL) && in->tpt_max != 0u && !moving) {
        const uint64_t tpt_per_node = (in->strict ? 29u : 27u) + (in->strict ? 4u : 1u) * (uint64_t)in->nl;
        const uint64_t tpt_fixed = (25u + 36u) * 64u + (uint64_t)in->depth * 3u * 64u;
        const uint64_t tpt_nslots = 8u * (uint64_t)WT_TPT_SLOTS_PER_XCC;
        const uint64_t tpt_slice = min_u64(WT_TPT_SLICE_WORDS_MAX, ((uint64_t)in->tpt_pool_mb << 18) / tpt_nslots) & ~(uint64_t)63;
        const uint64_t tpt_cap = min_u64(tpt_slice > tpt_fixed ? ((tpt_slice - tpt_fixed) / tpt_per_node) & ~(uint64_t)63 : 0, 64960u);
        o->tail_wanted = tpt_cap >= WT_TPT_MIN_CAP;
        o->tpt_slice = (uint32_t)tpt_slice; o->tpt_cap = (uint32_t)tpt_cap; o->tpt_nslots = (uint32_t)tpt_nslots;
    }
    o->split_max_lg = ss == 1 ? 4u : (ss == 2 ? 2u : (ss == 4 ? 1u : 0u));
    if (in->pass == WT_PASS_REFINE) {
        if (o->trows > WT_TILE_LIST_MAX || o->tpr > WT_TILE_LIST_MAX)
            return o->status = refuse(o->message, "Adaptive supersampling: %u x %u blocks are more than a tile list can address (4095 each way)", o->tpr, o->trows);
    } else if (P->tiled && in->sched && !(in->variant & WT_V_NO_TILE_ORDER) && o->trows <= WT_TILE_LIST_MAX && o->tpr <= WT_TILE_LIST_MAX) {
        o->use_order = 1;
        o->split = o->tail_wanted && !(flags & WT_F_GRID) && in->split_min_quota != 0u && !(in->variant & WT_V_NO_SPLIT) && o->split_max_lg != 0u;
        if (o->split) { o->per_share_cap = o->per_share + WT_SPLIT_EXTRA_PER_SHARE; o->grid = 8 * o->per_share_cap; }
        P->cost_sum = (o->tail_wanted && !(flags & WT_F_GRID)) ? 1u : 0u;
    }
    if ((flags & WT_F_DEEP) && !(flags & WT_F_COUNT) && !(in->variant & WT_V_FULL_STACK)) flags |= in->depth <= 8 ? WT_F_D8 : (in->depth <= 16 ? WT_F_D16 : 0);
    if (!in->strict && flags == WT_F_GEOM_LDS && in->ns >= 1u && in->ns <= WT_SHAPE_MAX_SPHERES && in->np <= WT_SHAPE_MAX_PLANES && in->nl == WT_SHAPE_LIGHTS &&
        (in->np == 0u || P->lpt) && !(in->variant & WT_V_NO_SHAPE))
        flags = (int)WT_SHAPE_FLAGS(in->ns, in->np, in->nl);
    if (P->ss_lg) flags |= WT_F_SS;
    if (P->ss_lg && moving) flags |= WT_F_MOVE;
    if (in->pass == WT_PASS_REFINE) flags |= WT_F_LIST;
    if (in->strict && !(flags & WT_F_DEEP) && (flags & (WT_F_COUNT | WT_F_GRID)) && (P->seed_offset != 0u || (o->fused && in->acc_frame >= 0))) flags |= WT_F_ACC;
    if (o->tail_wanted) {
        P->tpt_slice_words = o->tpt_slice; P->tpt_cap = o->tpt_cap; P->tpt_slots = WT_TPT_SLOTS_PER_XCC;
        P->tpt_max = in->tpt_max < 64u ? in->tpt_max : 64u; P->tpt_min = in->tpt_min;
    }
    o->flags = flags;
    o->dyn_lds = dyn_lds;
    return o->status = WT_PLAN_LAUNCH;
}

wt_order_choice wt_order_choose(wt_order_state* s) {
    wt_order_choice c;
    c.rd = s->have[s->newest] ? s->newest : -1;
    if (c.rd >= 0 && s->frame - s->newest_frame <= 1 && s->have[c.rd ^ 1]) c.rd ^= 1;
    s->frame++;
    c.wait_wr = s->have[s->wr] != 0;
    c.wait_rd = c.rd >= 0 && c.rd != s->wr;
    return c;
}

int wt_order_rebuild(wt_order_state* s, int sig_changed, int grid_build) {
    int rebuild = !s->sig_valid || sig_changed;
    if (rebuild) { s->sig_valid = 1; s->sig_age = 0; }
    else if (grid_build && s->sig_age < 2) rebuild = 1;
    if (s->sig_age < 255) s->sig_age++;
    return rebuild;
}

void wt_order_launched(wt_order_state* s, int rebuilt) {
    if (rebuilt) { s->have[s->wr] = 1; s->newest = s->wr; s->newest_frame = s->frame - 1; }
    s->wr ^= 1;
}

uint64_t wt_plan_range(uint64_t array_size, uint32_t total, uint64_t out_size) { return range_of(array_size, total, out_size); }
int wt_plan_projection(const wt_plan_in* in) { return projection_of(in); }
uint32_t wt_plan_lane_sample(uint32_t lane, uint32_t n) { return lane_sample(lane, n); }
uint32_t wt_plan_grid(const whitted_params* P) { return grid_of(P); }
void wt_plan_fused_range(const wt_raygen* g, uint32_t n_items, whitted_params* P) { fused_range(g, n_items, P); }
wt_geom_class wt_plan_geometry(int strict, int variant, uint32_t ns, uint32_t np, uint32_t geom_f4, int have_lpt, int grid_usable) {
    return geometry_of(strict, variant, ns, np, geom_f4, have_lpt, grid_usable);
}

wt_cast_class wt_plan_cast(int variant, uint32_t ns, uint32_t geom_f4, int grid_usable, uint32_t n, uint32_t batches_req) {
    const wt_geom_class gc = geometry_of(0, variant, ns, 0u, geom_f4, 0, grid_usable);
    wt_cast_class c = {gc.flags, (gc.flags & WT_F_GEOM_LDS) ? gc.dyn_lds : 0u, 0u, 1u};
    if (n == 0u || n >= (1u << 30)) return c;
    if (gc.flags & WT_F_GEOM_LDS) c.batches = WT_CAST_BATCHES_LDS;
    if (batches_req > 0u) c.batches = batches_req < WT_CAST_BATCHES_MAX ? batches_req : WT_CAST_BATCHES_MAX;
    const uint32_t waves = (n + 63u) / 64u;
    c.groups = (waves + c.batches - 1u) / c.batches;
    return c;
}

void wt_plan_sizes(uint32_t out[3]) {
    out[0] = (uint32_t)sizeof(wt_plan_in); out[1] = (uint32_t)sizeof(wt_plan_out); out[2] = (uint32_t)offsetof(wt_plan_out, message);
}

void wt_plan_many(const wt_plan_in* in, size_t n, int32_t* status, int32_t* flags) {
    static wt_plan_out o;
    for (size_t i = 0; i < n; i++) {
        status[i] = wt_plan_mode_check(&in[i], in[i].acc_frame >= 0, o.message);
        if (!status[i]) status[i] = wt_plan(&in[i], &o);
        flags[i] = status[i] == WT_PLAN_LAUNCH ? o.flags : -1;
    }
}
```

### example_gui_opencl_raytracer_amd/csrc/launch_plan.h

```cpp
#ifndef LAUNCH_PLAN_H
#define LAUNCH_PLAN_H
#include <stddef.h>
#include <stdint.h>

#include "../../include/hip_wrap_ext.h"
#include "whitted_params.h"

#ifdef __cplusplus
extern "C" {
#endif

enum { WT_V_GEOM_GLOBAL = 1, WT_V_LINEAR_IDS = 2, WT_V_NO_TILE_ORDER = 4, WT_V_NO_GRID = 8, WT_V_NO_TAIL = 16, WT_V_NO_OCC = 64,
       WT_V_NO_LPT = 128, WT_V_NO_VIS = 256, WT_V_TIMELINE = 512, WT_V_VIS_VERIFY = 1024, WT_V_FULL_STACK = 2048, WT_V_NO_SPLIT = 4096,
       WT_V_NO_SHAPE = 8192, WT_V_UNTRIMMED = 16384 };

enum {
    WT_LAUNCH_ROUND = 256,
    WT_GEOM_LDS_MAX_F4 = 1024,
    WT_SHALLOW_LEVELS = 3,
    WT_GRID_MIN_SPHERES = 256,
    WT_OCC_TILES_PER_DEPTH = 9000,
    WT_TPT_MAX_LANES = 40, WT_TPT_MIN_PATHS = 4, WT_TPT_POOL_MB = 8192, WT_TPT_MIN_CAP = 160, WT_TPT_SLOTS_PER_XCC = 1024,
    WT_TPT_SLICE_WORDS_MAX = 1 << 18,
    WT_SPLIT_EXTRA_PER_SHARE = 1024, WT_SPLIT_MIN_QUOTA = 1500, WT_SPLIT_SLOTS = 512,
    WT_TILE_LIST_MAX = 0xFFF
};

typedef struct {
    float corner[3], origin[3], up[3], right[3];
    float w_factor, h_factor;
    uint32_t width, height;
    uint64_t id_offset;
    uint32_t n_items;
    uint32_t band_stride, band_phase;
} wt_raygen;

enum { WT_PASS_PLAIN = 0, WT_PASS_BASE = 1, WT_PASS_REFINE = 2 };

typedef struct {
    int32_t depth, strict, fuse, counting, stamps, tpt_clock, variant;
    int32_t supersample;
    int32_t adaptive;
    uint32_t seed_offset;
    int32_t acc_frame, acc_jitter;
    float aperture, focus, through;
    uint32_t tpt_max, tpt_pool_mb, tpt_min, split_min_quota, occ_tiles_per_depth;
    int32_t sched;
    uint32_t diag;
    uint64_t id_offset;
    uint32_t band_stride;
    int32_t scene_ok;
    uint32_t ns, np, nl, geom_f4;
    int32_t have_lpt, grid_usable;
    int32_t args_ok;
    int32_t rays_generated, rays_exposed;
    wt_raygen gen;
    uint64_t rays_size;
    uint64_t array_size, out_size;
    uint32_t total;
    int32_t has_strip;
    uint32_t strip_row0, strip_rows;
    int32_t pass;
    const clw_sample_camera* cams;
    const float* times;
    const float* disp;
    uint32_t n_cams, n_times, n_disp;
    int32_t explicit_times;
} wt_plan_in;

enum { WT_PLAN_LAUNCH = 0, WT_PLAN_NONE = 1 , WT_PLAN_REFUSED = 2 };

typedef struct {
    int32_t status;
    int32_t flags;
    uint32_t grid, dyn_lds;
    whitted_params P;
    uint64_t out_offset;
    uint32_t out_pixels;
    int32_t fused;
    int32_t need_counters;
    int32_t ss;
    uint32_t trows, tpr, per_share, per_share_cap;
    int32_t use_order;
    int32_t split;
    uint32_t split_max_lg;
    int32_t tail_wanted;
    uint32_t tpt_slice, tpt_cap, tpt_nslots;
    wt_raygen sig;
    int32_t samples_decided;
    uint32_t n_cams, n_times;
    uint32_t motion_floats;
    char message[200];
    clw_sample_camera cams_used[64];
    float times_used[64];
    wt_cam_table cam_table;
    float motion_table[2 * WT_CAM_TABLE_FLOATS];
} wt_plan_out;

int wt_plan(const wt_plan_in* in, wt_plan_out* out);
int wt_plan_mode_check(const wt_plan_in* in, int accumulating, char* message);
int wt_plan_projection(const wt_plan_in* in);
uint64_t wt_plan_range(uint64_t array_size, uint32_t total, uint64_t out_size);
uint32_t wt_plan_lane_sample(uint32_t lane, uint32_t n);
uint32_t wt_plan_grid(const whitted_params* P);
void wt_plan_fused_range(const wt_raygen* g, uint32_t n_items, whitted_params* P);
typedef struct { int32_t flags; uint32_t dyn_lds, lpt, vis; } wt_geom_class;
wt_geom_class wt_plan_geometry(int strict, int variant, uint32_t ns, uint32_t np, uint32_t geom_f4, int have_lpt, int grid_usable);
enum { WT_CAST_BATCHES_LDS = 1, WT_CAST_BATCHES_MAX = 64 };
typedef struct { int32_t flags; uint32_t dyn_lds, groups, batches; } wt_cast_class;
wt_cast_class wt_plan_cast(int variant, uint32_t ns, uint32_t geom_f4, int grid_usable, uint32_t n, uint32_t batches_req);

typedef struct {
    int32_t have[2];
    int32_t wr;
    int32_t newest;
    int32_t sig_valid, sig_age;
    uint64_t frame, newest_frame;
} wt_order_state;
typedef struct { int32_t rd , wait_wr, wait_rd ; } wt_order_choice;
wt_order_choice wt_order_choose(wt_order_state* s);
int wt_order_rebuild(wt_order_state* s, int sig_changed, int grid_build);
void wt_order_launched(wt_order_state* s, int rebuilt);

int wt_fast_has_trace(int flags);
int wt_strict_has_trace(int flags);
void wt_plan_sizes(uint32_t out[3]);
void wt_plan_many(const wt_plan_in* in, size_t n, int32_t* status, int32_t* flags);

#ifdef __cplusplus
}
#endif
#endif
```

### example_gui_opencl_raytracer_amd/csrc/whitted_hit.inc

```
            cost++;
            if (COUNT) {
                c_iter++;
                unsigned long long live = __builtin_amdgcn_ballot_w64(true);
                if (lane == (unsigned)__builtin_ctzll(live)) c_witer += 64u;
            }
            const rayq r = UNIT_CT ? wt_rayq<true>(o, d) : wt_rayq<false>(o, d, P.unit_dirs != 0u);

            if (COUNT) c_probe++;
            bool lit = false;
            float tl = INFINITY;
            f3 lcol = mk3(0, 0, 0);
            auto probe_chunk = [&](auto nc, const unsigned base) {
                constexpr int N = decltype(nc)::value;
                float4 l0[N]; float bq[N], Dq[N]; bool ok[N]; bool any = false;
#pragma unroll
                for (int k = 0; k < N; k++) l0[k] = wt_geom<GEOM_LDS>(P, sg, g_lgt + 2 * (base + k));
#pragma unroll
                for (int k = 0; k < N; k++) {
                    const sph_pre pre = wt_sphere_pre(r.o, l0[k]);
                    ok[k] = wt_sphere_disc(pre, r.d, r.a4, bq[k], Dq[k]);
                    any |= ok[k];
                }
                if (__builtin_amdgcn_ballot_w64(any)) {
#pragma unroll
                    for (int k = 0; k < N; k++) {
                        float t;
                        const bool hit = wt_sphere_root(bq[k], Dq[k], r.a2, t) && ok[k];
                        if (hit && !(t >= tl)) {
                            float4 l1 = wt_geom<GEOM_LDS>(P, sg, g_lgt + 2 * (base + k) + 1);
                            tl = t;
                            f3 hp = wt_madd3(d, t, o);
                            float dist = wt_sqrt(dot3(o - hp, o - hp));
                            lcol = mk3(l1.x, l1.y, l1.z) * (1 / dist * dist);
                            lit = true;
                        }
                    }
                }
            };
            for (unsigned base = 0; base < SH::nl(P); base += 4u) {
                const unsigned left = SH::nl(P) - base;
                if (left >= 4u) probe_chunk(wt_int<4>{}, base);
                else if (left == 3u) probe_chunk(wt_int<3>{}, base);
                else if (left == 2u) probe_chunk(wt_int<2>{}, base);
                else probe_chunk(wt_int<1>{}, base);
            }
            if (__builtin_amdgcn_ballot_w64(lit)) {
                if (lit) {
                    if (GRID) {
                        if (wt_grid_occluded(P, r, tl)) lit = false;
                    }
                    for (unsigned i = 0; !GRID && i < SH::ns(P); i++) {
                        float4 s = wt_sphere_at<GEOM_LDS>(P, sg, i, WT_MOTION);
                        float t;
                        bool hit = wt_sphere(r, s, t);
                        if (hit && t <= tl && !(__float_as_uint(s.w) >> 31)) lit = false;
                    }
                    for (unsigned i = 0; i < SH::np(P); i++) {
                        float4 n = wt_geom<GEOM_LDS>(P, sg, g_pln + 2 * i);
                        float4 p0 = wt_geom<GEOM_LDS>(P, sg, g_pln + 2 * i + 1);
                        float t;
                        bool hit = wt_plane(r, n, p0, t);
                        if (hit && t <= tl) lit = false;
                    }
                }
            }
            WT_STAMP(WT_ST_PROBE);
            if (lit) {
                WT_HIT_COLOUR(lcol);
                ended = true;
            } else {
                if (COUNT) c_seg++;
                float tbest = INFINITY;
                int best = -1;
                if (GRID) {
                    best = wt_grid_nearest(P, r, tbest);
                } else {
                    for (unsigned base = 0; base < SH::ns(P); base += 4u) {
                        float4 s4[4]; float bq[4], Dq[4]; bool ok[4]; bool any = false;
#pragma unroll
                        for (int k = 0; k < 4; k++) s4[k] = wt_sphere_at<GEOM_LDS>(P, sg, min(base + k, SH::ns(P) - 1u), WT_MOTION);
#pragma unroll
                        for (int k = 0; k < 4; k++) {
                            const sph_pre pre = wt_sphere_pre(r.o, s4[k]);
                            ok[k] = wt_sphere_disc(pre, r.d, r.a4, bq[k], Dq[k]) && (base + k < SH::ns(P));
                            any |= ok[k];
                        }
                        if (__builtin_amdgcn_ballot_w64(any)) {
#pragma unroll
                            for (int k = 0; k < 4; k++) {
                                if (__builtin_amdgcn_ballot_w64(ok[k]) == 0) continue;
                                float t;
                                const bool hit = wt_sphere_root(bq[k], Dq[k], r.a2, t) && ok[k];
                                if (hit && !(t >= tbest)) { tbest = t; best = (int)(base + k); }
                            }
                        }
                    }
                }
                for (unsigned i = 0; i < SH::np(P); i++) {
                    float4 n = wt_geom<GEOM_LDS>(P, sg, g_pln + 2 * i);
                    float4 p0 = wt_geom<GEOM_LDS>(P, sg, g_pln + 2 * i + 1);
                    float t;
                    bool hit = wt_plane(r, n, p0, t);
                    if (hit && !(t >= tbest)) { tbest = t; best = (int)(SH::ns(P) + i); }
                }
                WT_STAMP(WT_ST_NEAREST);
                if (best < 0) {
                    if (COUNT) c_sky++;
                    WT_HIT_COLOUR(wt_texel_rgb(wt_skybox_fetch(P, d)));
                    ended = true;
                } else {
                    ip = wt_madd3(d, tbest, o);
                    prim = (unsigned)best;
                    textured = false;
                    if ((unsigned)best < SH::ns(P)) {
                        float4 s = wt_sphere_at<GEOM_LDS>(P, sg, (unsigned)best, WT_MOTION);
                        nrm = wt_normalize(ip - mk3(s.x, s.y, s.z));
                    } else {
                        unsigned pi = (unsigned)best - SH::ns(P);
                        float4 n = wt_geom<GEOM_LDS>(P, sg, g_pln + 2 * pi);
                        nrm = mk3(n.x, n.y, n.z);
                        if (n.w != 0.0f) {
                            if (COUNT) c_tex++;
                            texpx = wt_plane_texel_fetch(P, pi, ip);
                            textured = true;
                        }
                    }
                    wt_mat_set_b(m, wt_mat_f4(P, prim, 1u, SH::ns(P)));
                    {
                        const float4 a_ = wt_mat_f4(P, prim, 0u, SH::ns(P));
                        m.rgb = mk3(a_.x, a_.y, a_.z);
                        wt_mat_set_c(m, wt_mat_f4(P, prim, 2u, SH::ns(P)));
                    }
                    ip = wt_madd3(nrm, WT_EPSILON, ip);
                    cost += 3u;
                    {
                        const f3 c_ = textured ? wt_texel_rgb(texpx) : m.rgb;
                        WT_HIT_AMBIENT(c_ * f, m.ambient);
                    }
                    view = wt_normalize(o - ip);
                    ks = f * m.specular; kd = f * m.diffuse;
                    shade = true;
                }
            }
```

### example_gui_opencl_raytracer_amd/csrc/whitted_launch.h

```cpp
#ifndef WHITTED_LAUNCH_H
#define WHITTED_LAUNCH_H
#include <hip/hip_runtime.h>
#include "projection_host.h"
#include "whitted_params.h"

#define WT_BOTH(ret, name, args) extern "C" ret wt_fast_##name args; extern "C" ret wt_strict_##name args;
#define WT_FAST_ONLY(ret, name, args) extern "C" ret wt_fast_##name args;

WT_BOTH(hipError_t, launch_trace, (const whitted_params* P, int flags, unsigned grid, size_t dyn_lds, hipStream_t s))
WT_BOTH(int, has_trace, (int flags))
WT_BOTH(hipError_t, launch_raygen, (const raygen_params* P, hipStream_t s))
WT_BOTH(hipError_t, launch_raygen_proj, (const raygen_params* P, const wt_projection* T, hipStream_t s))
WT_BOTH(hipError_t, launch_sched, (const unsigned* cost, unsigned* order, unsigned tpr, unsigned trows, unsigned per_share, unsigned clamp_outliers,
                                   unsigned per_share_cap, unsigned split_slots, unsigned min_quota, unsigned max_lg, hipStream_t s))
WT_FAST_ONLY(hipError_t, launch_classify, (const unsigned* frame, unsigned width, unsigned rows, unsigned lgb, unsigned threshold, unsigned char* mask,
                                           unsigned* order, unsigned* count, unsigned cap, hipStream_t s))
WT_BOTH(hipError_t, launch_cams, (const wt_cam_table* T, float* dst, hipStream_t s))
WT_BOTH(hipError_t, launch_unit, (int op, const float* in, float* out, unsigned n, unsigned stride_in, unsigned stride_out, unsigned aux, hipStream_t s))
WT_BOTH(hipError_t, launch_unit_scene, (const whitted_params* P, int flags, int op, const float* in, float* out, unsigned n, unsigned stride_in,
                                        unsigned stride_out, size_t dyn_lds, hipStream_t s))
WT_BOTH(hipError_t, launch_gbuffer, (const whitted_params* P, int flags, unsigned grid, size_t dyn_lds, float* depth, unsigned* id, float* normal,
                                     float* point, float* albedo, const wt_projection* T, hipStream_t s))
WT_BOTH(hipError_t, launch_overlay, (const unsigned* frame, const unsigned* ids, unsigned* out, unsigned width, unsigned rows, unsigned flags,
                                     const unsigned style[5], const unsigned* sel, unsigned count, hipStream_t s))
WT_BOTH(hipError_t, launch_objects, (const unsigned* ids, const unsigned* depth, unsigned width, unsigned rows, unsigned first_row,
                                     const unsigned clip[4], const unsigned counts[3], void* table, void* result, hipStream_t s))
WT_BOTH(hipError_t, launch_ao_trace, (const whitted_params* P, int flags, const float* point, const float* normal, const unsigned* ids,
                                      const float* dirs, unsigned char* open, unsigned width, unsigned rows, unsigned first_row, unsigned K,
                                      float radius, hipStream_t s))
WT_BOTH(hipError_t, launch_ao_resolve, (const unsigned char* open, const unsigned* ids, const unsigned* frame, unsigned* out, unsigned width,
                                        unsigned rows, unsigned ao_flags, unsigned K, unsigned strength, hipStream_t s))
WT_BOTH(hipError_t, launch_cast, (const whitted_params* P, int flags, unsigned groups, unsigned batches, size_t dyn_lds, const void* rays, unsigned n,
                                  unsigned cast_flags, void* hits, unsigned char* blocked, hipStream_t s))
#undef WT_BOTH
#undef WT_FAST_ONLY

#ifdef WT_STRICT
#if WT_STRICT
#define WT_NAME(name) wt_strict_##name
#else
#define WT_NAME(name) wt_fast_##name
#endif
#define WT_LAUNCHER(name) extern "C" hipError_t WT_NAME(launch_##name)
#else
#define WT_LAUNCH(I, name) ((I)->strict ? wt_strict_launch_##name : wt_fast_launch_##name)
#endif
#endif
```

### example_gui_opencl_raytracer_amd/csrc/whitted_launch.inc

```
namespace WT_NS {
#include "whitted_trace.inc"
#include "whitted_gbuffer.inc"
#include "whitted_projection.inc"
#include "whitted_ao.inc"
#include "whitted_cast.inc"
#include "whitted_overlay.inc"
#include "whitted_objects.inc"
}

template <int FLAGS>
static hipError_t wt_launch_one(const whitted_params* P, unsigned grid, size_t dyn_lds, hipStream_t s) {
    hipLaunchKernelGGL(WT_NS::wt_trace<FLAGS>, dim3(grid), dim3(WT_BLOCK), dyn_lds, s, *P);
    return hipGetLastError();
}

typedef hipError_t (*wt_trace_launcher)(const whitted_params*, unsigned, size_t, hipStream_t);
static wt_trace_launcher wt_find_trace(int flags) {
#if !WT_STRICT
    if (flags & WT_F_SHAPE) {
        switch (flags) {
#define WT_SHAPE_CASE(ns, np) case WT_SHAPE_FLAGS(ns, np, WT_SHAPE_LIGHTS): return wt_launch_one<WT_SHAPE_FLAGS(ns, np, WT_SHAPE_LIGHTS)>; \
                              case WT_SHAPE_FLAGS(ns, np, WT_SHAPE_LIGHTS) | WT_F_SS: return wt_launch_one<WT_SHAPE_FLAGS(ns, np, WT_SHAPE_LIGHTS) | WT_F_SS>; \
                              case WT_SHAPE_FLAGS(ns, np, WT_SHAPE_LIGHTS) | WT_F_SS | WT_F_LIST: return wt_launch_one<WT_SHAPE_FLAGS(ns, np, WT_SHAPE_LIGHTS) | WT_F_SS | WT_F_LIST>; \
                              case WT_SHAPE_FLAGS(ns, np, WT_SHAPE_LIGHTS) | WT_F_SS | WT_F_MOVE: return wt_launch_one<WT_SHAPE_FLAGS(ns, np, WT_SHAPE_LIGHTS) | WT_F_SS | WT_F_MOVE>;
#define WT_SHAPE_CASES(ns) WT_SHAPE_CASE(ns, 0) WT_SHAPE_CASE(ns, 1) WT_SHAPE_CASE(ns, 2)
            WT_SHAPE_CASES(1) WT_SHAPE_CASES(2) WT_SHAPE_CASES(3) WT_SHAPE_CASES(4)
#undef WT_SHAPE_CASES
#undef WT_SHAPE_CASE
        }
        return nullptr;
    }
#endif
    switch (flags & (255 | WT_F_SS | WT_F_MOVE | WT_F_LIST | WT_F_ACC)) {
#define WT_CASE(F) case F: return wt_launch_one<F>;
#define WT_CASE2(F) WT_CASE(F) WT_CASE((F) | WT_F_SS) WT_CASE((F) | WT_F_SS | WT_F_LIST)
#define WT_CASE3(F) WT_CASE2(F) WT_CASE((F) | WT_F_SS | WT_F_MOVE)
        WT_CASE3(0) WT_CASE3(1) WT_CASE3(2) WT_CASE3(3) WT_CASE3(4) WT_CASE3(5) WT_CASE3(6) WT_CASE3(7)
        WT_CASE(8) WT_CASE(9) WT_CASE(10) WT_CASE(11) WT_CASE(12) WT_CASE(13) WT_CASE(14) WT_CASE(15)
        WT_CASE2(16) WT_CASE2(17) WT_CASE2(18) WT_CASE2(19) WT_CASE(24) WT_CASE(25) WT_CASE(26) WT_CASE(27)
        WT_CASE3(66) WT_CASE3(70) WT_CASE(74) WT_CASE(78) WT_CASE2(82) WT_CASE(90)
        WT_CASE3(130) WT_CASE3(134) WT_CASE(138) WT_CASE(142) WT_CASE2(146) WT_CASE(154)
#if WT_STRICT
        WT_CASE3(1 | WT_F_ACC) WT_CASE3(5 | WT_F_ACC) WT_CASE(9 | WT_F_ACC) WT_CASE(13 | WT_F_ACC)
        WT_CASE2(16 | WT_F_ACC) WT_CASE2(17 | WT_F_ACC) WT_CASE(24 | WT_F_ACC) WT_CASE(25 | WT_F_ACC)
#endif
#if !WT_STRICT
        WT_CASE3(98) WT_CASE3(102) WT_CASE(106) WT_CASE(110) WT_CASE2(114) WT_CASE(122)
        WT_CASE3(162) WT_CASE3(166) WT_CASE(170) WT_CASE(174) WT_CASE2(178) WT_CASE(186)
        WT_CASE3(34) WT_CASE3(35) WT_CASE3(38) WT_CASE3(39) WT_CASE(42) WT_CASE(43) WT_CASE(46) WT_CASE(47)
        WT_CASE2(50) WT_CASE2(51) WT_CASE(58) WT_CASE(59)
#endif
#undef WT_CASE3
#undef WT_CASE2
#undef WT_CASE
    }
    return nullptr;
}

WT_LAUNCHER(trace)(const whitted_params* P, int flags, unsigned grid, size_t dyn_lds,
                                      hipStream_t s) {
    const wt_trace_launcher run = wt_find_trace(flags);
    return run ? run(P, grid, dyn_lds, s) : hipErrorInvalidValue;
}

extern "C" int WT_NAME(has_trace)(int flags) { return wt_find_trace(flags) != nullptr; }

WT_LAUNCHER(raygen)(const raygen_params* P, hipStream_t s) {
    unsigned grid = (P->n_items + WT_RG_BLOCK - 1) / WT_RG_BLOCK;
    hipLaunchKernelGGL(WT_NS::wt_raygen, dim3(grid), dim3(WT_RG_BLOCK), 0, s, *P);
    return hipGetLastError();
}

WT_LAUNCHER(sched)(const unsigned* cost, unsigned* order, unsigned tpr, unsigned trows,
                                      unsigned per_share, unsigned clamp_outliers, unsigned per_share_cap, unsigned split_slots,
                                      unsigned min_quota, unsigned max_lg, hipStream_t s) {
    hipLaunchKernelGGL(WT_NS::wt_sched_build, dim3(8), dim3(256), 0, s, cost, order, tpr, trows, per_share, clamp_outliers, per_share_cap,
                       split_slots, min_quota, max_lg);
    return hipGetLastError();
}

#if !WT_STRICT
WT_LAUNCHER(classify)(const unsigned* frame, unsigned width, unsigned rows, unsigned lgb, unsigned threshold,
                                         unsigned char* mask, unsigned* order, unsigned* count, unsigned cap, hipStream_t s) {
    const unsigned b = 1u << lgb, nbc = (width + b - 1u) / b, nbr = (rows + b - 1u) / b;
    const unsigned per_wave = 64u >> (2u * lgb), wpr = (nbc + per_wave - 1u) / per_wave;
    const unsigned long long waves = (unsigned long long)nbr * wpr;
    if (lgb > 2u || waves == 0ull || waves > 0xFFFFFFFFull) return hipErrorInvalidValue;
    hipLaunchKernelGGL(WT_NS::wt_refine_classify, dim3((unsigned)((waves + 3ull) / 4ull)), dim3(256), 0, s, frame, width, rows, lgb, threshold, nbc, nbr,
                       wpr, mask, order, count, cap);
    return hipGetLastError();
}
#endif

WT_LAUNCHER(cams)(const wt_cam_table* T, float* dst, hipStream_t s) {
    hipLaunchKernelGGL(WT_NS::wt_cams_store, dim3(1), dim3(64), 0, s, *T, (float4*)dst);
    return hipGetLastError();
}

WT_LAUNCHER(unit)(int op, const float* in, float* out, unsigned n, unsigned stride_in,
                                     unsigned stride_out, unsigned aux, hipStream_t s) {
    hipLaunchKernelGGL(WT_NS::wt_unit, dim3((n + 63) / 64), dim3(64), 0, s, op, in, out, n, stride_in, stride_out, aux);
    return hipGetLastError();
}

WT_LAUNCHER(unit_scene)(const whitted_params* P, int flags, int op, const float* in, float* out, unsigned n,
                                           unsigned stride_in, unsigned stride_out, size_t dyn_lds, hipStream_t s) {
    const dim3 grid((n + 63) / 64), block(64);
    if (flags & WT_F_GRID) hipLaunchKernelGGL((WT_NS::wt_unit_scene<false, true>), grid, block, 0, s, *P, op, in, out, n, stride_in, stride_out);
    else if (flags & WT_F_GEOM_LDS) hipLaunchKernelGGL((WT_NS::wt_unit_scene<true, false>), grid, block, dyn_lds, s, *P, op, in, out, n, stride_in, stride_out);
    else hipLaunchKernelGGL((WT_NS::wt_unit_scene<false, false>), grid, block, 0, s, *P, op, in, out, n, stride_in, stride_out);
    return hipGetLastError();
}

WT_LAUNCHER(gbuffer)(const whitted_params* P, int flags, unsigned grid, size_t dyn_lds, float* depth, unsigned* id,
                                        float* normal, float* point, float* albedo, const wt_projection* T, hipStream_t s) {
    const WT_NS::wt_gbuffer_out G = {depth, id, normal, point, albedo};
    const dim3 g(grid), block(WT_BLOCK);
    if (T->model != CLW_PROJ_PERSPECTIVE) {
        if (flags & WT_F_GRID) hipLaunchKernelGGL((WT_NS::wt_gbuffer<false, true, true>), g, block, 0, s, *P, G, *T);
        else if (flags & WT_F_GEOM_LDS) hipLaunchKernelGGL((WT_NS::wt_gbuffer<true, false, true>), g, block, dyn_lds, s, *P, G, *T);
        else hipLaunchKernelGGL((WT_NS::wt_gbuffer<false, false, true>), g, block, 0, s, *P, G, *T);
    } else if (flags & WT_F_GRID) hipLaunchKernelGGL((WT_NS::wt_gbuffer<false, true, false>), g, block, 0, s, *P, G, *T);
    else if (flags & WT_F_GEOM_LDS) hipLaunchKernelGGL((WT_NS::wt_gbuffer<true, false, false>), g, block, dyn_lds, s, *P, G, *T);
    else hipLaunchKernelGGL((WT_NS::wt_gbuffer<false, false, false>), g, block, 0, s, *P, G, *T);
    return hipGetLastError();
}

WT_LAUNCHER(raygen_proj)(const raygen_params* P, const wt_projection* T, hipStream_t s) {
    if (P->n_items == 0u || P->width == 0u || (T->model != CLW_PROJ_ORTHO && T->model != CLW_PROJ_EQUIRECT) ||
        (T->model == CLW_PROJ_EQUIRECT && (!T->col || !T->row || T->width != P->width || T->height != P->height)))
        return hipErrorInvalidValue;
    unsigned grid = (P->n_items + WT_RG_BLOCK - 1) / WT_RG_BLOCK;
    hipLaunchKernelGGL(WT_NS::wt_raygen_proj, dim3(grid), dim3(WT_RG_BLOCK), 0, s, *P, *T);
    return hipGetLastError();
}

WT_LAUNCHER(overlay)(const unsigned* frame, const unsigned* ids, unsigned* out, unsigned width, unsigned rows, unsigned flags,
                                        const unsigned style[5], const unsigned* sel, unsigned count, hipStream_t s) {
    const unsigned long long tpr = (width + (WT_OV_TILE_W - 1ull)) / WT_OV_TILE_W, trows = (rows + (WT_OV_TILE_H - 1ull)) / WT_OV_TILE_H;
    if (width == 0u || rows == 0u || width > 0x7FFFFFFFu || tpr * trows > 0x7FFFFFFFull || count > 64u || flags < 1u || flags > 7u ||
        ((flags & WT_OV_OUTLINE) && (style[0] < 1u || style[0] > 4u)))
        return hipErrorInvalidValue;
    WT_NS::wt_overlay_args A = {};
    A.frame = frame; A.ids = ids; A.out = out; A.width = width; A.rows = rows; A.tiles_per_row = (unsigned)tpr;
    A.radius = style[0]; A.outline_rgb = style[1] & 0x00FFFFFFu; A.fill_rgb = style[2] & 0x00FFFFFFu; A.fill_alpha = style[3];
    A.edge_rgb = style[4] & 0x00FFFFFFu; A.count = count;
// ... 96 lines not shown
```

### example_gui_opencl_raytracer_amd/csrc/whitted_params.h

```cpp
#ifndef WHITTED_PARAMS_H
#define WHITTED_PARAMS_H
#include <stdint.h>

#define CLW_MAX_DEPTH 32
#define CLW_NUM_COUNTERS 32
#define CLW_STAMP_SHARDS 1024

#define WT_BLOCK 64
#ifndef WT_VIS_MAX_SPHERES
#define WT_VIS_MAX_SPHERES 16
#endif
enum { WT_F_COUNT = 1, WT_F_DEEP = 2, WT_F_GEOM_LDS = 4, WT_F_RAYS = 8, WT_F_GRID = 16,
       WT_F_OCC = 32 ,
       WT_F_D8 = 64, WT_F_D16 = 128 ,
       WT_F_SHAPE = 256 ,
       WT_F_SS = 1 << 17 ,
       WT_F_MOVE = 1 << 18 ,
       WT_F_LIST = 1 << 19 ,
       WT_F_ACC = 1 << 20  };
#define WT_SHAPE_FLAGS(ns, np, nl) (WT_F_GEOM_LDS | WT_F_SHAPE | ((ns) << 9) | ((np) << 12) | ((nl) << 14))
enum { WT_SHAPE_MAX_SPHERES = 4, WT_SHAPE_MAX_PLANES = 2, WT_SHAPE_LIGHTS = 3 };

typedef struct {
    float corner[3], origin[3], up[3], right[3];
    float w_factor, h_factor;
    uint32_t width, height;
    uint64_t id_offset;
    uint32_t n_items;
    uint32_t tiled;
    uint32_t rows;
    uint32_t row_offset;
    uint32_t band_stride, band_phase;
    const uint32_t* tile_order;
    uint32_t* tile_cost;
    uint32_t* tpt_pool;
    uint32_t* tpt_flags;
    const uint32_t* tpt_jump;
    uint32_t tpt_slice_words, tpt_cap, tpt_slots, tpt_max, tpt_min;
    uint32_t tpt_clock;
    uint32_t cost_sum;
    int32_t depth;
    uint32_t untrimmed;
    const float* geom;
    const float* ptex;
    const uint8_t* spheres_raw;
    const uint8_t* planes_raw;
    uint32_t ns, np, nl;
    float through;
    uint32_t geom_f4;
    uint32_t unit_dirs;
    uint32_t lpt;
    uint32_t vis;
    uint32_t diag;
    const uint32_t* grid_start;
    const uint32_t* grid_items;
    const uint32_t* grid_box;
    const float* grid_geom;
    float grid_min[3], grid_inv[3], grid_cell[3];
    uint32_t grid_pair;
    int32_t grid_res[3];
    const uint32_t* tex; int32_t tex_w, tex_h, tex_layers;
    const uint32_t* sky; int32_t sky_w, sky_h;
    const float* rays;
    uint32_t* out;
    float* out_rgb;
    unsigned long long* counters;
    uint32_t ss_lg;
    const float* ss_cams;
    const float* ss_disp;
    const float* ss_times;
    const uint32_t* list_count;
    float* acc_sum;
    float acc_scale;
    uint32_t seed_offset;
} whitted_params;

#define WT_LIST_COUNT_STRIDE 32
#define WT_CAM_TABLE_FLOATS (64 * 12)
typedef struct { float v[WT_CAM_TABLE_FLOATS]; } wt_cam_table;

typedef struct {
    float corner[3], origin[3], up[3], right[3];
    float w_factor, h_factor;
    uint32_t width, height;
    uint64_t id_offset;
    uint32_t n_items;
    uint32_t band_stride, band_phase;
    float* rays;
} raygen_params;

#endif
```

### example_gui_opencl_raytracer_amd/csrc/whitted_trace.inc

```

#ifndef WT_STRICT
#error "WT_STRICT must be defined (0: fast, 1: strict)"
#endif

#define WT_EPSILON 0.001f
#define WT_THROUGH 0.8f
#define WT_DEFAULT_N 1.0f
#define WT_SOFT 2
#ifndef WT_LDS_LEVELS
#if WT_STRICT
#define WT_LDS_LEVELS 3
#else
#define WT_LDS_LEVELS 2
#endif
#endif
#ifndef WT_LDS_LEVELS_DEEP
#define WT_LDS_LEVELS_DEEP 3
#endif
#ifndef WT_LDS_LEVELS_DEEP_OCC
#define WT_LDS_LEVELS_DEEP_OCC 1
#endif
#ifndef WT_MIN_WAVES
#define WT_MIN_WAVES (WT_STRICT ? 2 : 3)
#endif
// ... 968 lines not shown
            if (__builtin_amdgcn_ballot_w64(live != 0u) == 0) break;
        }
        const float4 n = wt_geom<GEOM_LDS>(P, sg, g_pln + 2 * i);
        const float4 p0 = wt_geom<GEOM_LDS>(P, sg, g_pln + 2 * i + 1);
        const float num = wt_plane_pre(ip, n, p0);
        bool skip[NR / WT_SOFT];
#pragma unroll
        for (int k = 0; k < NR / WT_SOFT; k++) skip[k] = false;
        if (CULL && SH::lpt(P) && chunk != ~0u) {
            const float4 mu = wt_geom<GEOM_LDS>(P, sg, g_pln + 2 * SH::np(P) + 2 * SH::nl(P) + chunk * SH::np(P) + i);
            const float mus[3] = {mu.x, mu.y, mu.z};
            const float an = 1e-5f * fabsf(num) * mu.w;
#pragma unroll
            for (int k = 0; k < NR / WT_SOFT && k < 3; k++) {
                const bool cannot = (num * mus[k] < 0.0f) && (fabsf(mus[k]) > __builtin_fmaf(4e-6f, dlc[k], an));
                skip[k] = __builtin_amdgcn_ballot_w64(!cannot) == 0;
            }
        }
#pragma unroll
        for (int q = 0; q < NR; q++) {
            if (!skip[q / WT_SOFT]) {
                if (wt_plane_blocks(num, n, rd[q], tl[q])) op[q] = 0.0f;
            }
        }
    }
}

template <bool MOVE = false>
__device__ __forceinline__ void wt_stage_scene(const whitted_params& P, float4* s_geom, unsigned tid, unsigned nthreads) {
    for (unsigned i = tid; i < P.geom_f4; i += nthreads) s_geom[i] = ((const float4*)P.geom)[i];
    if (MOVE) for (unsigned i = tid; i < P.ns; i += nthreads) s_geom[P.geom_f4 + i] = ((const float4*)P.ss_disp)[i];
    __syncthreads();
}

#include "whitted_terms.inc"

template <int FLAGS>
struct wt_cfg {
    static constexpr bool deep = (FLAGS & 2) != 0, occ = (FLAGS & 32) != 0, grid = (FLAGS & 16) != 0;
    static constexpr int lds_levels = deep ? (occ ? WT_LDS_LEVELS_DEEP_OCC : WT_LDS_LEVELS_DEEP) : WT_LDS_LEVELS;
    static constexpr int max_levels = !deep ? 3 : ((FLAGS & 64) ? 7 : ((FLAGS & 128) ? 15 : CLW_MAX_DEPTH - 1));
    static constexpr int min_waves = deep ? (occ ? WT_OCC_WAVES : WT_MIN_WAVES) : ((grid && !WT_STRICT) ? WT_GRID_SHALLOW_WAVES : WT_SHALLOW_WAVES);
};
template <bool SUM>
__device__ __forceinline__ unsigned wt_wave_reduce(unsigned c) {
#define WT_DPP_STEP(ctrl, rows) do { const unsigned t_ = (unsigned)__builtin_amdgcn_update_dpp(0, (int)c, ctrl, rows, 0xF, false); \
                                     c = SUM ? c + t_ : max(c, t_); } while (0)
    WT_DPP_STEP(0x111, 0xF);
    WT_DPP_STEP(0x112, 0xF);
    WT_DPP_STEP(0x114, 0xF);
    WT_DPP_STEP(0x118, 0xF);
    WT_DPP_STEP(0x142, 0xA);
    WT_DPP_STEP(0x143, 0xC);
#undef WT_DPP_STEP
    return (unsigned)__builtin_amdgcn_readlane((int)c, 63);
}

__device__ __forceinline__ float wt_ss_resolve(float v, const unsigned lg) {
#define WT_SS_DPP(ctrl) v = v + __int_as_float(__builtin_amdgcn_update_dpp(0, __float_as_int(v), ctrl, 0xF, 0xF, false))
    WT_SS_DPP(0xB1);
    if (lg >= 2u) WT_SS_DPP(0x4E);
    if (lg >= 3u) WT_SS_DPP(0x141);
    WT_SS_DPP(0x128);
#undef WT_SS_DPP
    if (lg >= 2u) {
        const auto p = __builtin_amdgcn_permlane16_swap(__float_as_uint(v), __float_as_uint(v), false, false);
        v = __uint_as_float(p[0]) + __uint_as_float(p[1]);
    }
    if (lg >= 3u) {
        const auto p = __builtin_amdgcn_permlane32_swap(__float_as_uint(v), __float_as_uint(v), false, false);
        v = __uint_as_float(p[0]) + __uint_as_float(p[1]);
    }
    return v;
}

__device__ __forceinline__ void wt_acc_fold(float* __restrict__ s, const float scale, float& r, float& g, float& b) {
    float sr = r, sg = g, sb = b;
    if (scale != 1.0f) { sr = s[0] + r; sg = s[1] + g; sb = s[2] + b; }
    s[0] = sr; s[1] = sg; s[2] = sb;
    r = fminf(sr * scale, 1.0f); g = fminf(sg * scale, 1.0f); b = fminf(sb * scale, 1.0f);
}

typedef const __attribute__((address_space(4))) whitted_params* wt_kparams_t;
template <int FLAGS>
__device__ __forceinline__ void wt_trace_body(const wt_kparams_t Pk, const unsigned wg) {
    constexpr bool COUNT = (FLAGS & WT_F_COUNT) != 0;
    constexpr bool DEEP = (FLAGS & WT_F_DEEP) != 0;
    constexpr bool GEOM_LDS = (FLAGS & WT_F_GEOM_LDS) != 0;
    constexpr bool FROM_RAYS = (FLAGS & WT_F_RAYS) != 0;
    constexpr bool GRID = (FLAGS & WT_F_GRID) != 0;
    constexpr bool SS = (FLAGS & WT_F_SS) != 0;
    constexpr bool MOVE = SS && !GRID && (FLAGS & WT_F_MOVE) != 0;
    constexpr bool LIST = SS && (FLAGS & WT_F_LIST) != 0;
    constexpr bool SEEDED = !wt_acc_flagged(FLAGS) || (FLAGS & WT_F_ACC) != 0;
    constexpr bool ACC = SEEDED && !FROM_RAYS;
    constexpr bool UNIT_CT = !WT_STRICT && GEOM_LDS && !FROM_RAYS && !GRID;
    constexpr bool CLASSES = WT_STRICT != 0 && GEOM_LDS && !GRID;

    constexpr int LDSL = wt_cfg<FLAGS>::lds_levels;
    __shared__ float s_stk[LDSL * WT_REC * WT_BLOCK];
    __shared__ unsigned short s_tpt_bs[(DEEP && !wt_cfg<FLAGS>::occ) ? WT_TPT_MAX_BATCHES + 2 : 1];
    __shared__ unsigned s_tpt_px[(DEEP && !wt_cfg<FLAGS>::occ) ? 3 * 64 : 1];
    constexpr bool SPHCULL = DEEP && !GRID && (wt_cfg<FLAGS>::occ || WT_STRICT != 0);
    __shared__ int s_cull[SPHCULL ? 8 : 1];
    extern __shared__ float4 s_geom[];

    const whitted_params& P = *(const whitted_params*)Pk;
#if WT_TIMELINE
    const unsigned long long tl_entry = __builtin_amdgcn_s_memrealtime();
#endif
    if (LIST) { if ((wg >> 3) >= P.list_count[WT_LIST_COUNT_STRIDE * (wg & 7u)]) return; }

    if (GEOM_LDS) wt_stage_scene<MOVE>(P, s_geom, threadIdx.x, WT_BLOCK);
    const float4* sg = s_geom;
#if WT_TIMELINE
    const unsigned long long tl_staged = __builtin_amdgcn_s_memrealtime();
#endif
    WT_STAMP_DECL

    const unsigned tid = threadIdx.x;
    const unsigned lane = tid & 63u;

    bool valid;
    unsigned item;
    unsigned x = 0, y = 0;
    unsigned tile = 0xFFFFFFFFu;
    unsigned part_lg = 0u, part = 0u;
    if (P.tiled) {
        const unsigned tpr = (P.width + 7u) >> 3;
        const unsigned b = wg;
        unsigned trow, tcol;
        if (P.tile_order) {
            const unsigned t = P.tile_order[b];
            tcol = t & 0xFFFu; trow = (t >> 12) & 0xFFFu;
            part_lg = (t >> 24) & 7u; part = (t >> 27) & 15u;
            tile = (t == 0xFFFFFFFFu) ? t : trow * tpr + tcol;
        } else {
            const unsigned k = b & 7u, j = b >> 3;
            trow = (j / tpr) * 8u + k;
            tcol = j % tpr;
            tile = trow * tpr + tcol;
        }
        x = tcol * 8u + (lane & 7u);
        y = trow * 8u + (lane >> 3);
        valid = (tile != 0xFFFFFFFFu) && (x < P.width) && (y < P.rows) && ((lane >> (6u - part_lg)) == part);
        item = y * P.width + x;
    } else {
        item = wg * WT_BLOCK + tid;
        valid = item < P.n_items;
        if (P.band_stride > 1u) { y = item / P.width; x = item % P.width; }
    }
#if WT_TIMELINE
    asm volatile("" :: "v"(item), "v"(x), "v"(y));
    const unsigned long long tl_mapped = __builtin_amdgcn_s_memrealtime();
#endif
    unsigned long long gid = P.id_offset + item;
    unsigned gy = y;
    if (P.band_stride > 1u) {
        gy = ((y >> 3) * P.band_stride + P.band_phase) * 8u + (y & 7u);
        gid = (unsigned long long)gy * P.width + x;
    } else if (P.tiled) {
        gy = P.row_offset + y;
    }

    constexpr int SCRL = wt_cfg<FLAGS>::max_levels - LDSL;
    float deep[SCRL > 0 ? SCRL * WT_REC : 1];

    f3 o = mk3(0, 0, 0), d = mk3(0, 0, 1), rgb = mk3(0, 0, 0);
    int depth = 0;
    if (valid) {
        if (FROM_RAYS) {
            const float4* rr = (const float4*)(P.rays + 16 * (size_t)item);
            float4 ro = rr[0], rd = rr[1], rc = rr[2];
            o = mk3(ro.x, ro.y, ro.z); d = mk3(rd.x, rd.y, rd.z); rgb = mk3(rc.x, rc.y, rc.z);
            depth = __float_as_int(rr[3].x);
        } else if (SS && P.ss_cams) {
            const float4* c = (const float4*)P.ss_cams + 3u * lane;
            const float4 c0 = c[0], c1 = c[1], c2 = c[2];
            d = wt_primary_dir_xy(mk3(c0.x, c0.y, c0.z), mk3(c2.y, c2.z, c2.w), mk3(c1.z, c1.w, c2.x), P.w_factor, P.h_factor, x, gy);
            o = mk3(c0.w, c1.x, c1.y);
        } else {
            if (P.tiled || P.band_stride > 1u) d = wt_primary_dir_xy(P.corner, P.right, P.up, P.w_factor, P.h_factor, x, gy);
            else d = wt_primary_dir(P.corner, P.right, P.up, P.w_factor, P.h_factor, (unsigned)gid, P.width);
            o = mk3(P.origin[0], P.origin[1], P.origin[2]);
        }
    }
    wt_motion mv = {false, 0.0f, 0u};
    if (MOVE) { mv.on = true; mv.t = P.ss_times[lane]; mv.off = P.geom_f4; }
    float n1 = WT_DEFAULT_N, f = 1.0f;
    int sp = 0;
    unsigned rng = (unsigned)gid;
    if (SEEDED) rng += P.seed_offset;
    const int D = P.depth;
    bool active = valid && depth < D;

    unsigned c_seg = 0, c_shadow = 0, c_probe = 0, c_sky = 0, c_tex = 0, c_push = 0, c_iter = 0, c_witer = 0;
    unsigned c_traced = 0;
    unsigned c_known = 0, c_visbad = 0;
    unsigned c_tptrun = 0, c_tptfail = 0, c_tptnodes = 0;

    typedef wt_shape<FLAGS> SH;
    const unsigned g_pln = SH::ns(P), g_lgt = SH::ns(P) + 2 * SH::np(P);

    const unsigned long long t_begin = ((GRID || WT_COST_LIFETIME) && P.tile_cost) ? __builtin_amdgcn_s_memtime() : 0ull;
#if WT_TIMELINE
    const unsigned long long tl_begin = __builtin_amdgcn_s_memrealtime();
    unsigned long long tl_end = tl_begin;
#endif
    unsigned cost = 0;
#ifndef WT_LCH
#define WT_LCH 3
#endif
    constexpr int LCH = WT_LCH, NR = LCH * WT_SOFT;

    constexpr bool TPT = DEEP && !wt_cfg<FLAGS>::occ;
    unsigned tpt_thresh = (TPT && P.tpt_cap != 0u) ? (part_lg != 0u ? 64u : P.tpt_max) : 0u;
    WT_STAMP(WT_ST_PROLOG);
    for (;;) {
    while ((unsigned)__builtin_popcountll(__builtin_amdgcn_ballot_w64(active)) > tpt_thresh) {
        if (active) {
            WT_STAMP(WT_ST_LOOP);
            bool ended = false, shade = false;
            f3 ip, nrm, view;
            mat_t m;
            float ks, kd;
            unsigned prim, texpx;
            bool textured;
#include "whitted_hit.inc"
            WT_STAMP(WT_ST_RESOLVE);
            if (shade) {
#include "whitted_shade.inc"
#include "whitted_bounce.inc"
            WT_STAMP(WT_ST_BOUNCE);
            }
#include "whitted_pop.inc"
            WT_STAMP(WT_ST_POP);
        }
    }
    if (!TPT || __builtin_amdgcn_ballot_w64(active) == 0) break;
    {
        bool tpt_done = false;
#include "whitted_tpt.inc"
        if (tpt_done) break;
        tpt_thresh = 0u;
    }
    }
    if (P.tiled && P.tile_cost) {
        unsigned c = cost;
        if (GRID || WT_COST_LIFETIME) c = (unsigned)min((__builtin_amdgcn_s_memtime() - t_begin) >> 8, 0xFFFFFFFFull);
        else if (P.untrimmed) {
            if (P.cost_sum) for (int off = 32; off > 0; off >>= 1) c += (unsigned)__shfl_xor((int)c, off);
            else for (int off = 32; off > 0; off >>= 1) c = max(c, (unsigned)__shfl_xor((int)c, off));
        }
        else if (P.cost_sum) c = wt_wave_reduce<true>(c);
        else c = wt_wave_reduce<false>(c);
#if WT_TIMELINE
        if (P.diag && P.diag < 256u) c = ((unsigned)((tl_begin >> (P.diag - 1u)) & 0xFFFFull) << 16) | (unsigned)((__builtin_amdgcn_s_memrealtime() >> (P.diag - 1u)) & 0xFFFFull);
        tl_end = __builtin_amdgcn_s_memrealtime();
#endif
        if (lane == 0 && tile != 0xFFFFFFFFu && y < P.rows) {
            if (P.cost_sum && !(WT_TIMELINE && P.diag)) atomicAdd(P.tile_cost + tile, c);
            else P.tile_cost[tile] = c;
        }
    }


    if (SS) {
        const unsigned lg = P.ss_lg, m = (1u << lg) - 1u;
        const float inv = __uint_as_float((127u - 2u * lg) << 23);
        const float mr = wt_ss_resolve(fminf(fmaxf(rgb.x, 0.0f), 1.0f), lg) * inv;
        const float mg = wt_ss_resolve(fminf(fmaxf(rgb.y, 0.0f), 1.0f), lg) * inv;
        const float mb = wt_ss_resolve(fminf(fmaxf(rgb.z, 0.0f), 1.0f), lg) * inv;
        if (valid && (lane & (m | (m << 3))) == 0u) {
            const size_t px = (size_t)(y >> lg) * (P.width >> lg) + (x >> lg);
            float vr = mr, vg = mg, vb = mb;
            if (ACC && P.acc_sum) wt_acc_fold(P.acc_sum + 3 * px, P.acc_scale, vr, vg, vb);
            if (P.out_rgb) {
                float* q = P.out_rgb + 3 * px;
                q[0] = vr; q[1] = vg; q[2] = vb;
            }
            P.out[px] = ((unsigned)(vr * 255.0f) << 16) | ((unsigned)(vg * 255.0f) << 8) | (unsigned)(vb * 255.0f);
        }
    } else
    if (valid) {
        if (ACC && P.acc_sum) {
            rgb = mk3(fminf(fmaxf(rgb.x, 0.0f), 1.0f), fminf(fmaxf(rgb.y, 0.0f), 1.0f), fminf(fmaxf(rgb.z, 0.0f), 1.0f));
            wt_acc_fold(P.acc_sum + 3 * (size_t)item, P.acc_scale, rgb.x, rgb.y, rgb.z);
        }
        if (P.out_rgb) {
            float* q = P.out_rgb + 3 * (size_t)item;
            q[0] = rgb.x; q[1] = rgb.y; q[2] = rgb.z;
        }
        float cr = fminf(fmaxf(rgb.x, 0.0f), 1.0f) * 255.0f;
        float cg = fminf(fmaxf(rgb.y, 0.0f), 1.0f) * 255.0f;
        float cb = fminf(fmaxf(rgb.z, 0.0f), 1.0f) * 255.0f;
        P.out[item] = ((unsigned)cr << 16) | ((unsigned)cg << 8) | (unsigned)cb;
    }

#ifdef WT_STAMPS
    WT_STAMP(WT_ST_LOOP);
    __syncthreads();
    if (P.counters && lane == 0) {
        unsigned long long* sh = P.counters + CLW_NUM_COUNTERS + 16u * (wg & 1023u);
        for (int k = 0; k < WT_ST_N; k++) atomicAdd(sh + k, (unsigned long long)s_st[k]);
        atomicAdd(sh + WT_ST_N, 1ull);
    }
#endif
    if (COUNT) {
        unsigned v[14] = {c_seg, c_shadow, c_probe, c_sky, c_tex, c_push, c_iter, c_witer, c_traced, c_known, c_visbad, c_tptfail, c_tptrun, c_tptnodes};
#pragma unroll
        for (int k = 0; k < 14; k++) {
            unsigned x = v[k];
            for (int off = 32; off > 0; off >>= 1) x += __shfl_xor(x, off);
            if (lane == 0 && x) atomicAdd(P.counters + (k < 10 ? k : 18 + k), (unsigned long long)x);
        }
    }
#if WT_TIMELINE
    if (P.diag >= 256u && P.tiled && P.tile_cost && lane == 0 && tile != 0xFFFFFFFFu && y < P.rows) {
        __builtin_amdgcn_s_waitcnt(0);
        if (P.diag == 256u) P.tile_cost[tile] = ((unsigned)min(tl_begin - tl_entry, 0xFFFFull) << 16) | (unsigned)min(__builtin_amdgcn_s_memrealtime() - tl_end, 0xFFFFull);
        else P.tile_cost[tile] = ((unsigned)min(tl_staged - tl_entry, 1023ull) << 22) | ((unsigned)min(tl_mapped - tl_staged, 2047ull) << 11) | (unsigned)min(tl_begin - tl_mapped, 2047ull);
    }
#endif
}
template <int FLAGS>
__global__ void __launch_bounds__(WT_BLOCK, wt_cfg<FLAGS>::min_waves) wt_trace(const whitted_params P_arg) {
    const wt_kparams_t Pk = (wt_kparams_t)__builtin_amdgcn_kernarg_segment_ptr();
    wt_trace_body<FLAGS>(Pk, blockIdx.x);
}

__global__ void __launch_bounds__(64) wt_cams_store(const wt_cam_table T_arg, float4* __restrict__ dst) {
    typedef const __attribute__((address_space(4))) float4* kargs_t;
    const float4* src = (const float4*)(kargs_t)__builtin_amdgcn_kernarg_segment_ptr();
    (void)T_arg;
#pragma unroll
    for (unsigned k = 0; k < WT_CAM_TABLE_FLOATS / 4u / 64u; k++) dst[k * 64u + threadIdx.x] = src[k * 64u + threadIdx.x];
}

#define WT_RG_BLOCK 256
__global__ void __launch_bounds__(WT_RG_BLOCK) wt_raygen(const raygen_params P) {
    constexpr int RS = WT_RG_BLOCK + 1;
    __shared__ float4 s_rec[4 * RS];
    const unsigned tid = threadIdx.x;
    const size_t base = (size_t)blockIdx.x * WT_RG_BLOCK;
    const size_t item = base + tid;
    float4 r0 = make_float4(0, 0, 0, 0), r1 = r0;
    if (item < P.n_items) {
        unsigned long long gid = P.id_offset + item;
        if (P.band_stride > 1u) {
            const unsigned y = (unsigned)(item / P.width), x = (unsigned)(item % P.width);
            gid = (unsigned long long)(((y >> 3) * P.band_stride + P.band_phase) * 8u + (y & 7u)) * P.width + x;
        }
        f3 d = wt_primary_dir(P.corner, P.right, P.up, P.w_factor, P.h_factor, (unsigned)gid, P.width);
        r0 = make_float4(P.origin[0], P.origin[1], P.origin[2], 0.0f);
        r1 = make_float4(d.x, d.y, d.z, 0.0f);
    }
    s_rec[0 * RS + tid] = r0;
    s_rec[1 * RS + tid] = r1;
    s_rec[2 * RS + tid] = make_float4(0, 0, 0, 0);
    s_rec[3 * RS + tid] = make_float4(0, 0, 0, 0);
    __syncthreads();
    float4* dst = (float4*)P.rays + base * 4;
    const size_t limit = ((size_t)P.n_items - base < WT_RG_BLOCK ? (size_t)P.n_items - base : WT_RG_BLOCK) * 4;
#pragma unroll
    for (int k = 0; k < 4; k++) {
        size_t q = (size_t)k * WT_RG_BLOCK + tid;
        if (q < limit) dst[q] = s_rec[(q & 3) * RS + (q >> 2)];
    }
}

__global__ void __launch_bounds__(256) wt_sched_build(const unsigned* __restrict__ cost, unsigned* __restrict__ order,
                                                      unsigned tpr, unsigned trows, unsigned per_share, unsigned clamp_outliers,
                                                      unsigned per_share_cap, unsigned split_slots, unsigned min_quota, unsigned max_lg) {
    __shared__ unsigned hist[256];
    __shared__ unsigned base[256];
    __shared__ unsigned s_max, s_cnt, s_entries;
    __shared__ unsigned long long s_sum;
    const unsigned k = blockIdx.x, tid = threadIdx.x;
    hist[tid] = 0;
    if (tid == 0) { s_max = 1u; s_cnt = 0u; s_sum = 0ull; s_entries = 0u; }
    __syncthreads();
    unsigned cnt = 0u;
    unsigned long long sum = 0ull;
    for (unsigned j = tid; j < per_share; j += 256) {
        const unsigned trow = (j / tpr) * 8u + k;
        if (trow < trows) { sum += cost[trow * tpr + (j % tpr)]; cnt++; }
    }
    atomicAdd(&s_sum, sum); atomicAdd(&s_cnt, cnt);
    __syncthreads();
    unsigned quota = 0xFFFFFFFFu;
    if (split_slots != 0u) {
        const unsigned long long q = s_sum / split_slots;
        quota = (unsigned)(q > 0x7FFFFFFFull ? 0x7FFFFFFFull : q);
        if (quota < min_quota) quota = min_quota;
        if (quota == 0u) quota = 1u;
        bool fitted = false;
        for (int trial = 0; trial < 24; trial++) {
            if (tid == 0) s_entries = 0u;
            __syncthreads();
            unsigned e = 0u;
            for (unsigned j = tid; j < per_share; j += 256) {
                const unsigned trow = (j / tpr) * 8u + k;
                if (trow < trows) { unsigned lg = 0u; const unsigned c = cost[trow * tpr + (j % tpr)]; while (lg < max_lg && (c >> lg) > quota) lg++; e += 1u << lg; }
            }
            atomicAdd(&s_entries, e);
            __syncthreads();
            const bool fits = s_entries <= per_share_cap;
            __syncthreads();
            if (fits) { fitted = true; break; }
            quota = quota > 0x3FFFFFFFu ? 0xFFFFFFFFu : quota * 2u;
        }
// ... 86 lines not shown
}
#endif

enum { WT_U_SPHERE = 0, WT_U_PLANE = 1, WT_U_REFLECT = 2, WT_U_REFRACT = 3, WT_U_SCHLICK = 4, WT_U_CUBE = 5,
       WT_U_XORSHIFT = 6, WT_U_EMOD = 7, WT_U_SINCOS = 8, WT_U_POW = 9, WT_U_NORMALIZE = 10 };
__global__ void __launch_bounds__(64) wt_unit(int op, const float* __restrict__ in, float* __restrict__ out, unsigned n,
                                              unsigned stride_in, unsigned stride_out, unsigned aux) {
    const unsigned i = blockIdx.x * 64 + threadIdx.x;
    if (i >= n) return;
    const float* a = in + (size_t)i * stride_in;
    float* r = out + (size_t)i * stride_out;
    switch (op) {
        case WT_U_SPHERE: {
            const rayq q = wt_rayq<false>(mk3(a[0], a[1], a[2]), mk3(a[3], a[4], a[5]));
            float t;
            bool hit = wt_sphere(q, make_float4(a[6], a[7], a[8], a[9] * a[9]), t);
            r[0] = hit ? 1.0f : 0.0f; r[1] = hit ? t : 0.0f;
        } break;
        case WT_U_PLANE: {
            const rayq q = wt_rayq<false>(mk3(a[0], a[1], a[2]), mk3(a[3], a[4], a[5]));
            float t;
            bool hit = wt_plane(q, make_float4(a[6], a[7], a[8], 0.0f), make_float4(a[9], a[10], a[11], 0.0f), t);
            r[0] = hit ? 1.0f : 0.0f; r[1] = hit ? t : 0.0f;
        } break;
        case WT_U_REFLECT: {
            f3 v = wt_reflect(mk3(a[0], a[1], a[2]), mk3(a[3], a[4], a[5]));
            r[0] = v.x; r[1] = v.y; r[2] = v.z;
        } break;
        case WT_U_REFRACT: {
            f3 v = mk3(0, 0, 0);
            bool ok = wt_refract(a[0], a[1], mk3(a[2], a[3], a[4]), mk3(a[5], a[6], a[7]), v);
            r[0] = ok ? 1.0f : 0.0f; r[1] = v.x; r[2] = v.y; r[3] = v.z;
        } break;
        case WT_U_SCHLICK:
            r[0] = wt_schlick(a[0], a[1], mk3(a[2], a[3], a[4]), mk3(a[5], a[6], a[7]));
            break;
        case WT_U_CUBE: {
            int u, v;
            wt_cube_uv(mk3(a[0], a[1], a[2]), aux, u, v);
            r[0] = __int_as_float(u); r[1] = __int_as_float(v);
        } break;
        case WT_U_XORSHIFT: {
            unsigned st = __float_as_uint(a[0]);
            float v = wt_xorshift(st);
            r[0] = __uint_as_float(st); r[1] = v;
        } break;
        case WT_U_EMOD:
            r[0] = __int_as_float(wt_emod(__float_as_int(a[0]), __float_as_int(a[1])));
            break;
        case WT_U_SINCOS: {
            float sn, cs;
            if (aux) wt_sincos_angle<true>(a[0], sn, cs); else wt_sincos_angle<false>(a[0], sn, cs);
            r[0] = sn; r[1] = cs;
        } break;
        case WT_U_POW:
            r[0] = wt_pow(a[0], a[1]);
            break;
        case WT_U_NORMALIZE: {
            float len;
            f3 v = wt_normalize_len(mk3(a[0], a[1], a[2]), len);
            r[0] = v.x; r[1] = v.y; r[2] = v.z; r[3] = len;
        } break;
        default: break;
    }
}

enum { WT_US_HIT = 0, WT_US_SHADOW = 1, WT_US_TEXEL = 2 };
template <bool GEOM_LDS, bool GRID>
__global__ void __launch_bounds__(64) wt_unit_scene(const whitted_params P, int op, const float* __restrict__ in,
                                                    float* __restrict__ out, unsigned n, unsigned stride_in, unsigned stride_out) {
    extern __shared__ float4 s_geom[];
    const unsigned tid = threadIdx.x, lane = tid & 63u;
    constexpr bool UNIT_CT = false;
    if (GEOM_LDS) wt_stage_scene(P, s_geom, tid, 64u);
    const float4* sg = s_geom;
    typedef wt_shape<0> SH;
    const unsigned g_pln = P.ns, g_lgt = P.ns + 2 * P.np;
    const unsigned i = blockIdx.x * 64 + tid;
    if (i >= n) return;
    const float* a = in + (size_t)i * stride_in;
    float* res = out + (size_t)i * stride_out;
    WT_STAMP_DECL
    constexpr bool COUNT = false, FROM_RAYS = false;
    unsigned cost = 0, c_iter = 0, c_witer = 0, c_probe = 0, c_seg = 0, c_sky = 0, c_tex = 0;
    const wt_motion mv = {false, 0.0f, 0u};
    (void)lane; (void)c_iter; (void)c_witer; (void)c_probe; (void)c_seg; (void)c_sky; (void)c_tex;
    if (op == WT_US_HIT) {
        f3 o = mk3(a[0], a[1], a[2]), d = mk3(a[3], a[4], a[5]), rgb = mk3(0, 0, 0);
        const float f = 1.0f;
        bool ended = false, shade = false;
        f3 ip = mk3(0, 0, 0), nrm = mk3(0, 0, 0), view = mk3(0, 0, 0);
        mat_t m;
        m.rgb = mk3(0, 0, 0); m.ambient = m.diffuse = m.specular = m.shininess = 0.0f;
        m.transparent = m.dielectric = 0u; m.n = 0.0f; m.reflectivity = 0.0f;
        float ks = 0.0f, kd = 0.0f;
        unsigned prim = 0u, texpx = 0u;
        bool textured = false;
        {
#include "whitted_hit.inc"
            res[0] = lit ? 1.0f : 0.0f;
            if (lit) { res[1] = rgb.x; res[2] = rgb.y; res[3] = rgb.z; }
        }
        (void)ended; (void)view; (void)ks; (void)kd; (void)cost;
        res[4] = shade ? 1.0f : 0.0f;
        if (shade) {
            if (textured) m.rgb = wt_texel_rgb(texpx);
            res[5] = ip.x; res[6] = ip.y; res[7] = ip.z; res[8] = nrm.x; res[9] = nrm.y; res[10] = nrm.z;
            res[11] = m.rgb.x; res[12] = m.rgb.y; res[13] = m.rgb.z; res[14] = m.ambient; res[15] = m.diffuse; res[16] = m.specular;
            res[17] = m.shininess; res[18] = (float)m.transparent; res[19] = (float)m.dielectric; res[20] = m.n; res[21] = m.reflectivity;
        }
    } else if (op == WT_US_SHADOW) {
        const f3 to = mk3(a[0], a[1], a[2]), from = mk3(a[3], a[4], a[5]);
        constexpr int NR = WT_SOFT * 3;
        f3 rd[NR]; float tl[NR], a4[NR], a2[NR], opq[NR];
#pragma unroll
        for (int q = 0; q < NR; q++) { rd[q] = mk3(0, 0, 0); tl[q] = 0.0f; a4[q] = 0.0f; a2[q] = 0.0f; opq[q] = 0.0f; }
        rd[0] = wt_normalize_len(to - from, tl[0]);
        const rayq rq = wt_shadow_rayq_scene<GEOM_LDS>(P, from, rd[0]);
        a4[0] = rq.a4; a2[0] = rq.a2; opq[0] = 1.0f;
        if (GRID) {
            opq[0] = wt_grid_shadow(P, from, rd[0], rq.a4, rq.a2, tl[0]);
            for (unsigned k = 0; k < P.np; k++) {
                const float4 pn = wt_geom<GEOM_LDS>(P, sg, g_pln + 2 * k);
                const float4 p0 = wt_geom<GEOM_LDS>(P, sg, g_pln + 2 * k + 1);
                if (wt_plane_blocks(wt_plane_pre(from, pn, p0), pn, rd[0], tl[0])) opq[0] = 0.0f;
            }
        } else {
            const float dlc[NR / WT_SOFT] = {0.0f, 0.0f, 0.0f};
            wt_shadow_batch<GEOM_LDS, NR, false>(P, sg, g_pln, from, rd, tl, a4, a2, opq, ~0u, dlc);
        }
        res[0] = opq[0];
    } else if (op == WT_US_TEXEL) {
        whitted_params Q = P;
        Q.ptex = a;
        const f3 c = wt_texel_rgb(wt_plane_texel_fetch(Q, 0u, mk3(a[8], a[9], a[10])));
        res[0] = c.x; res[1] = c.y; res[2] = c.z;
    }
}
```

### include/hip_wrap_ext.h

```cpp
#ifndef HIP_WRAP_EXT_H
#define HIP_WRAP_EXT_H
#include "opencl_wrap.h"
#include <stdint.h>

#ifdef __cplusplus
extern "C" {
#endif

#define CLW_MAX_DEPTH 32

void clw_ext_set_depth(cl_wrap* wrap, int depth);
int  clw_ext_get_depth(const cl_wrap* wrap);

void clw_ext_set_strict(cl_wrap* wrap, int strict);

void clw_ext_set_fuse(cl_wrap* wrap, int fuse);

void clw_ext_set_id_offset(cl_wrap* wrap, uint64_t first_id);

void clw_ext_set_row_bands(cl_wrap* wrap, uint32_t stride, uint32_t phase);

void clw_ext_set_async(cl_wrap* wrap, int async);
void clw_ext_sync(cl_wrap* wrap);

// ... 108 lines not shown
                          clw_projection* proj);
void clw_ext_set_projection(cl_wrap* wrap, const clw_projection* proj);
void clw_ext_get_projection(const cl_wrap* wrap, clw_projection* out);
int clw_ext_unit_projection(cl_wrap* wrap, const struct clw_camera* cam, const clw_projection* proj, uint64_t id_begin, uint64_t id_end,
                            float* out_rays);

#define CLW_AO_FILTER  1u
#define CLW_AO_COMPOSE 2u
typedef struct clw_ao {
    uint32_t flags;
    uint32_t rays;
    float    radius;
    uint32_t strength;
} clw_ao;
int clw_host_ao_dirs(uint32_t K, float* dirs4 );
int clw_host_ao_open(const float* point, const float* normal, const uint32_t* ids, uint32_t width, uint32_t rows, uint32_t first_row,
                     const void* spheres, uint32_t ns, const void* planes, uint32_t np, const clw_ao* ao, const float* dirs4,
                     uint8_t* open_u8);
int clw_host_ao_resolve(const uint8_t* open_u8, const uint32_t* ids, const uint32_t* frame , uint32_t width,
                        uint32_t rows, const clw_ao* ao, uint32_t* out_u32);
uint32_t clw_ext_render_ao(cl_wrap* wrap, const clw_ao* ao);
uint32_t clw_ext_read_ao(cl_wrap* wrap, uint32_t what, void* out, uint32_t capacity_bytes);
void*    clw_ext_ao_device_ptr(cl_wrap* wrap, uint32_t what);
uint32_t clw_ext_unit_ao_open(cl_wrap* wrap, const float* point, const float* normal, const uint32_t* ids, uint32_t width, uint32_t rows,
                              uint32_t first_row, const clw_ao* ao, uint8_t* open_u8);
uint32_t clw_ext_unit_ao_resolve(cl_wrap* wrap, const uint8_t* open_u8, const uint32_t* ids, const uint32_t* frame, uint32_t width,
                                 uint32_t rows, const clw_ao* ao, uint32_t* out);
#define CLW_TIMING_AO         0x414F5452u
#define CLW_TIMING_AO_RESOLVE 0x414F5253u

typedef struct clw_ray { float origin[3]; float tmax; float dir[3]; uint32_t ignore; } clw_ray;
typedef struct clw_hit { float t; uint32_t id; float normal[3]; float point[3]; } clw_hit;
#define CLW_CAST_SPHERES 1u
#define CLW_CAST_PLANES  2u
#define CLW_CAST_LIGHTS  4u
#define CLW_CAST_KINDS   7u
#define CLW_CAST_OPAQUE  8u
int clw_host_cast_rays(const clw_ray* rays, uint32_t n, uint32_t flags, const void* spheres, uint32_t ns, const void* planes, uint32_t np,
                       const void* lights, uint32_t nl, clw_hit* hits);
int clw_host_occluded_rays(const clw_ray* rays, uint32_t n, uint32_t flags, const void* spheres, uint32_t ns, const void* planes, uint32_t np,
                           const void* lights, uint32_t nl, uint8_t* blocked);
uint32_t clw_ext_cast_rays(cl_wrap* wrap, const clw_ray* rays, uint32_t n, uint32_t flags, clw_hit* hits);
uint32_t clw_ext_occluded_rays(cl_wrap* wrap, const clw_ray* rays, uint32_t n, uint32_t flags, uint8_t* blocked);
uint32_t clw_ext_cast_rays_device(cl_wrap* wrap, const void* d_rays, uint32_t n, uint32_t flags, void* d_hits, void* d_blocked);
#define CLW_TIMING_CAST 0x43415354u

void clw_ext_enable_counters(cl_wrap* wrap, int enable);
void clw_ext_read_counters(cl_wrap* wrap, uint64_t out[8]);
void clw_ext_read_counters_ex(cl_wrap* wrap, uint64_t* out, uint32_t n);

void clw_ext_set_shadow_through(cl_wrap* wrap, float factor);

void clw_ext_set_grid(cl_wrap* wrap, int on);
typedef struct {
    int32_t built, pair;
    int32_t res[3];
    uint32_t ncells;
    uint64_t pairs;
    float cell[3], gmin[3], reg_pad;
} clw_grid_info;
int clw_ext_get_grid(const cl_wrap* wrap, clw_grid_info* out);
void clw_ext_set_grid_pair(cl_wrap* wrap, int on);

void clw_ext_set_tile_sched(cl_wrap* wrap, int on);

uint32_t clw_ext_read_tile_costs(cl_wrap* wrap, uint32_t* out, uint32_t capacity);

void clw_ext_unit(cl_wrap* wrap, int op, const float* in, uint32_t stride_in, float* out, uint32_t stride_out,
                  uint32_t n, uint32_t aux);

#define CLW_SCHED_SENTINEL 0xA5A5A5A5u
uint32_t clw_ext_unit_sched(cl_wrap* wrap, const uint32_t* cost, uint32_t tpr, uint32_t trows, int clamp_outliers, uint32_t per_share_cap,
                            uint32_t split_slots, uint32_t min_quota, uint32_t max_lg, uint32_t* out, uint32_t out_words);
uint32_t clw_ext_read_tile_order(cl_wrap* wrap, uint32_t* out, uint32_t capacity, uint32_t* per_share_cap);
void clw_ext_set_split(cl_wrap* wrap, int slots, int min_quota);
void clw_ext_get_split(const cl_wrap* wrap, uint32_t* slots, uint32_t* min_quota, uint32_t* extra_per_share);

void clw_ext_unit_scene(cl_wrap* wrap, cl_uint kernel_id, int op, const float* in, uint32_t stride_in, float* out,
                        uint32_t stride_out, uint32_t n);

void clw_ext_set_variant(cl_wrap* wrap, int variant);
int clw_ext_last_trace_flags(cl_wrap* wrap);

void clw_ext_set_tpt(cl_wrap* wrap, int max_lanes, int min_paths, int pool_mb);
void clw_ext_get_tpt(const cl_wrap* wrap, uint32_t* max_lanes, uint32_t* min_paths, uint32_t* pool_mb);

typedef struct clw_camera {
    float im_corner[3], origin[3], up[3], right[3];
    float w_factor, h_factor;
    uint32_t width, height;
} clw_camera;
int clw_host_perspective(const float origin[3], const float look[3], float fov, float focal,
                         uint32_t width, uint32_t height, clw_camera* out);

int clw_host_lens_cameras(const clw_camera* base, float aperture, float focus, uint32_t n, clw_sample_camera* out);
int clw_host_shutter_cameras(const clw_camera* open, const clw_camera* close, uint32_t n, clw_sample_camera* out);
int clw_host_sample_times(uint32_t n, float* out);
int clw_host_spheres_at(const void* rspheres, uint32_t ns, const float* disp, float t, void* out);

uint32_t clw_host_frame_seed(uint32_t f);
int clw_host_jitter_camera(const clw_camera* base, uint32_t f, uint32_t n, clw_camera* out);

int clw_host_refine_mask(const uint32_t* xrgb, uint32_t width, uint32_t rows, uint32_t n, int threshold, uint8_t* out);

int clw_host_write_png(const char* path, const uint32_t* xrgb, uint32_t width, uint32_t height);
int clw_host_write_png_rgba(const char* path, const uint8_t* rgba, uint32_t width, uint32_t height);
int clw_host_read_png(const char* path, uint32_t* width, uint32_t* height, uint8_t** rgba_malloced);
void clw_host_free(void* p);

const char* clw_ext_version(void);

#ifdef __cplusplus
}
#endif
#endif
```

Before: 351,000 Mrays/s.

## Add per-tile primary-ray cull table to skip spheres/lights in first hit

Adds a per-8x8-tile cull table, built on the device by a new kernel, that marks whether any sphere or light can be hit by primary rays in that tile. A trace kernel twin reads the tile's bits and uses them to skip the sphere and light tests on the first segment only. The table is cached per view and scene and built only when the same view is seen a second time, so the first frame pays nothing. The cost is an extra kernel argument load, a second template instantiation per flavour, and the risk of wrong culls near tile edges, which the conservative angular margins are meant to guard against.

```diff
diff --git a/example_gui_opencl_raytracer_amd/api.py b/example_gui_opencl_raytracer_amd/api.py
--- a/example_gui_opencl_raytracer_amd/api.py
+++ b/example_gui_opencl_raytracer_amd/api.py
@@ -44,6 +44,7 @@
     "clw_host_ao_dirs", "clw_host_ao_open", "clw_host_ao_resolve", "clw_ext_render_ao", "clw_ext_read_ao", "clw_ext_ao_device_ptr",
     "clw_ext_unit_ao_open", "clw_ext_unit_ao_resolve",
     "clw_host_cast_rays", "clw_host_occluded_rays", "clw_ext_cast_rays", "clw_ext_occluded_rays", "clw_ext_cast_rays_device",
+    "clw_host_primary_cull", "clw_ext_read_primary_cull",
 ]
 
 GB_DEPTH, GB_ID, GB_NORMAL, GB_POINT, GB_ALBEDO, GB_ALL = 1, 2, 4, 8, 16, 31
@@ -318,6 +319,11 @@
         L.clw_ext_occluded_rays.restype = u32
         L.clw_ext_cast_rays_device.argtypes = [W, vp, u32, u32, vp, vp]
         L.clw_ext_cast_rays_device.restype = u32
+    if hasattr(L, "clw_ext_read_primary_cull") or not os.environ.get("CLWRAP_LIB"):
+        L.clw_host_primary_cull.argtypes = [C.POINTER(clw_camera), u32, u32, u32, u32, vp, u32, vp, u32, vp]
+        L.clw_host_primary_cull.restype = u32
+        L.clw_ext_read_primary_cull.argtypes = [W, vp, u32, C.POINTER(C.c_uint64)]
+        L.clw_ext_read_primary_cull.restype = u32
     L.clw_ext_unit.argtypes = [W, C.c_int, vp, u32, vp, u32, u32, u32]
     L.clw_ext_read_tile_costs.argtypes = [W, vp, u32]
     L.clw_ext_read_tile_costs.restype = u32
@@ -517,6 +523,23 @@
     return out
 
 
+CULL_SPHERES, CULL_LIGHTS = 1, 2
+VARIANT_NO_CULL = 32768
+
+
+def host_primary_cull(cam: clw_camera, spheres, lights, rows: int | None = None, row_offset: int = 0, band_stride: int = 1, band_phase: int = 0) -> np.ndarray:
+    rows = int(cam.height) if rows is None else int(rows)
+    s = None if spheres is None else np.ascontiguousarray(spheres)
+    l = None if lights is None else np.ascontiguousarray(lights)
+    ns, nl = (0 if a is None else int(a.shape[0]) for a in (s, l))
+    trows, tpr = (rows + 7) // 8, (int(cam.width) + 7) // 8
+    out = np.empty(max(trows * tpr, 1), np.uint8)
+    n = load_library().clw_host_primary_cull(C.byref(cam), int(row_offset), rows, int(band_stride), int(band_phase), _ptr(s), ns, _ptr(l), nl, _ptr(out))
+    if n != trows * tpr or n == 0:
+        raise ValueError("clw_host_primary_cull rejects these arguments (a frame with tiles, band_phase below band_stride)")
+    return out[:n].reshape(trows, tpr)
+
+
 def _rect(rect):
     if rect is None:
         return None
@@ -749,6 +772,15 @@
     def set_tile_sched(self, on): self.L.clw_ext_set_tile_sched(C.byref(self.w), int(on))
     def set_variant(self, v): self.L.clw_ext_set_variant(C.byref(self.w), int(v))
     def last_trace_flags(self): return int(self.L.clw_ext_last_trace_flags(C.byref(self.w)))
+
+    def read_primary_cull(self):
+        builds = C.c_uint64()
+        n = self.L.clw_ext_read_primary_cull(C.byref(self.w), None, 0, C.byref(builds))
+        if n == 0:
+            return None, int(builds.value)
+        out = np.empty(n, np.uint8)
+        self.L.clw_ext_read_primary_cull(C.byref(self.w), _ptr(out), n, C.byref(builds))
+        return out, int(builds.value)
     def set_tpt(self, max_lanes=-1, min_paths=-1, pool_mb=-1): self.L.clw_ext_set_tpt(C.byref(self.w), int(max_lanes), int(min_paths), int(pool_mb))
     def timing_reset(self): self.L.clw_ext_timing_reset(C.byref(self.w))
     def set_timing_every(self, n): self.L.clw_ext_set_timing_every(C.byref(self.w), int(n))
diff --git a/example_gui_opencl_raytracer_amd/build.py b/example_gui_opencl_raytracer_amd/build.py
--- a/example_gui_opencl_raytracer_amd/build.py
+++ b/example_gui_opencl_raytracer_amd/build.py
@@ -16,11 +16,11 @@
 CC = os.environ.get("CC") or "gcc"
 
 DEVICE_DEPS = ["whitted_trace.inc", "whitted_hit.inc", "whitted_shade.inc", "whitted_bounce.inc", "whitted_pop.inc", "whitted_tpt.inc", "whitted_terms.inc",
-               "whitted_gbuffer.inc", "whitted_projection.inc", "whitted_ao.inc", "whitted_cast.inc", "whitted_overlay.inc", "whitted_objects.inc", "whitted_launch.inc", "whitted_launch.h", "whitted_params.h",
+               "whitted_gbuffer.inc", "whitted_projection.inc", "whitted_ao.inc", "whitted_cast.inc", "whitted_overlay.inc", "whitted_objects.inc", "whitted_cull.inc", "primary_cull_host.h", "whitted_launch.inc", "whitted_launch.h", "whitted_params.h",
                "projection_host.h"]
 SHIM_FLAGS = ["-O2", "-std=c++17", "-Wall"]
 SHIM_DEPS = ["hip_wrap_impl.h", "whitted_params.h", "whitted_launch.h", "launch_plan.h", "scene_prep.h", "ao_host.h", "cast_host.h", "overlay_host.h", "objects_host.h", "projection_host.h",
-             "png_codec.h", "../../include/opencl_wrap.h", "../../include/hip_wrap_ext.h"]
+             "primary_cull_host.h", "png_codec.h", "../../include/opencl_wrap.h", "../../include/hip_wrap_ext.h"]
 UNITS = [
     ("whitted_fast.hip", "hip", ["-O3", f"--offload-arch={ARCH}", "-fno-slp-vectorize", "-ffp-contract=off"], DEVICE_DEPS),
     ("whitted_strict.hip", "hip", ["-O3", f"--offload-arch={ARCH}", "-fno-slp-vectorize", "-ffp-contract=off"], DEVICE_DEPS),
@@ -35,6 +35,8 @@
      ["cast_host.h", "scene_prep.h", "../../include/hip_wrap_ext.h", "../../include/opencl_wrap.h"]),
     ("objects_host.c", "c", ["-O2", "-std=c99", "-ffp-contract=off", "-Wall", "-Wextra"],
      ["objects_host.h", "../../include/hip_wrap_ext.h", "../../include/opencl_wrap.h"]),
+    ("primary_cull_host.c", "c", ["-O2", "-std=c99", "-ffp-contract=off", "-Wall", "-Wextra", "-D_DEFAULT_SOURCE"],
+     ["primary_cull_host.h", "scene_prep.h", "../../include/hip_wrap_ext.h", "../../include/opencl_wrap.h"]),
     ("projection_host.c", "c", ["-O2", "-std=c99", "-ffp-contract=off", "-Wall", "-Wextra", "-D_DEFAULT_SOURCE"],
      ["projection_host.h", "../../include/hip_wrap_ext.h", "../../include/opencl_wrap.h"]),
     ("launch_plan.c", "c", ["-O2", "-std=c99", "-ffp-contract=off", "-Wall", "-Wextra"],
diff --git a/example_gui_opencl_raytracer_amd/csrc/hip_wrap.cpp b/example_gui_opencl_raytracer_amd/csrc/hip_wrap.cpp
--- a/example_gui_opencl_raytracer_amd/csrc/hip_wrap.cpp
+++ b/example_gui_opencl_raytracer_amd/csrc/hip_wrap.cpp
@@ -469,6 +469,40 @@
     return wt_order_rebuild(&S.o, changed, plan.flags & WT_F_GRID) != 0;
 }
 
+const unsigned char* bind_primary_cull(Impl* I, Impl::Cull& C, const wt_plan_in& in, const wt_plan_out& plan) {
+    C.last_used = false;
+    if (!wt_plan_cull(&in, &plan)) return nullptr;
+    const whitted_params& P = plan.P;
+    wt_cull_view V;
+    memset(&V, 0, sizeof V);
+    memcpy(V.corner, P.corner, sizeof V.corner); memcpy(V.origin, P.origin, sizeof V.origin);
+    memcpy(V.up, P.up, sizeof V.up); memcpy(V.right, P.right, sizeof V.right);
+    V.w_factor = P.w_factor; V.h_factor = P.h_factor;
+    V.width = P.width; V.rows = P.rows; V.row_offset = P.row_offset; V.band_stride = P.band_stride; V.band_phase = P.band_phase;
+    if (!wt_cull_view_ok(&V)) return nullptr;
+    const uint32_t tiles = plan.trows * plan.tpr;
+    const size_t bytes = ((size_t)tiles + 3u) & ~(size_t)3u;
+    const bool current = C.valid && C.scene == I->scene_generation && C.tiles == tiles && !memcmp(&C.view, &V, sizeof V);
+    if (!current) {
+        const bool again = C.seen && C.seen_scene == I->scene_generation && C.seen_tiles == tiles && !memcmp(&C.seen_view, &V, sizeof V);
+        C.valid = false;
+        if (!again) { C.seen = true; C.seen_view = V; C.seen_scene = I->scene_generation; C.seen_tiles = tiles; return nullptr; }
+    }
+    wait_tables_fence(I);
+    if (C.bytes != bytes || !C.table) {
+        if (C.table) { finish(I); C.free_all(); }
+        HIP_OK(hipMalloc((void**)&C.table, bytes), "Couldn't allocate device memory");
+        C.bytes = bytes;
+    }
+    if (!current) {
+        if (wt_fast_launch_cull(&P, C.table, I->stream) != hipSuccess) die("Couldn't run the kernel");
+        C.view = V; C.scene = I->scene_generation; C.tiles = tiles; C.valid = true; C.builds++;
+    }
+    I->tables_in_flight = true;
+    C.last_used = true;
+    return C.table;
+}
+
 void bind_tail_pool(Impl* I, wt_plan_out& plan) {
     if (!plan.tail_wanted) return;
     whitted_params& P = plan.P;
@@ -531,8 +565,9 @@
     else if (plan.P.tiled) sort = bind_tile_order(I, S, plan, strip);
     I->last_trace_flags = plan.flags;
     bind_tail_pool(I, plan);
+    const unsigned char* tile_cull = bind_primary_cull(I, I->culls[strip ? strip->slot : 0], in, plan);
     LaunchTimer t(I, kid, pass == PASS_PLAIN);
-    hipError_t e = WT_LAUNCH(I, trace)(&plan.P, plan.flags, plan.grid, plan.dyn_lds, I->stream);
+    hipError_t e = WT_LAUNCH(I, trace)(&plan.P, tile_cull, plan.flags, plan.grid, plan.dyn_lds, I->stream);
     if (e != hipSuccess) die("Couldn't run the kernel");
     t.done();
     if (plan.P.tile_cost) sort_tile_costs(I, S, plan, sort);
@@ -891,6 +926,7 @@
     if (I->d_grid_geom) (void)hipFree(I->d_grid_geom);
     if (I->sched_stream) (void)hipStreamSynchronize(I->sched_stream);
     for (auto& sc : I->scheds) sc.free_all();
+    for (auto& c : I->culls) c.free_all();
     if (I->sched_stream) (void)hipStreamDestroy(I->sched_stream);
     if (I->copy_stream) (void)hipStreamDestroy(I->copy_stream);
     for (hipEvent_t e : I->chunk_done) if (e) (void)hipEventDestroy(e);
@@ -1050,6 +1086,16 @@
 void clw_ext_set_tile_sched(cl_wrap* wrap, int on) { Impl* I = impl_of(wrap); I->sched = on ? 1 : 0; for (auto& sc : I->scheds) sc.reset(); }
 void clw_ext_set_variant(cl_wrap* wrap, int variant) { impl_of(wrap)->variant = variant; }
 int clw_ext_last_trace_flags(cl_wrap* wrap) { return impl_of(wrap)->last_trace_flags; }
+uint32_t clw_ext_read_primary_cull(cl_wrap* wrap, uint8_t* out, uint32_t capacity, uint64_t* builds) {
+    Impl* I = impl_of(wrap);
+    use_device(I);
+    finish(I);
+    const Impl::Cull& C = I->culls[0];
+    if (builds) *builds = C.builds;
+    if (!C.last_used || !C.table) return 0;
+    if (out && capacity >= C.tiles) HIP_OK(hipMemcpy(out, C.table, C.tiles, hipMemcpyDeviceToHost), "Failed to transfer device memory to host");
+    return C.tiles;
+}
 void clw_ext_set_tpt(cl_wrap* wrap, int max_lanes, int min_paths, int pool_mb) {
     Impl* I = impl_of(wrap);
     if (max_lanes >= 0) I->tpt_max = (unsigned)std::min(max_lanes, 64);
diff --git a/example_gui_opencl_raytracer_amd/csrc/hip_wrap_impl.h b/example_gui_opencl_raytracer_amd/csrc/hip_wrap_impl.h
--- a/example_gui_opencl_raytracer_amd/csrc/hip_wrap_impl.h
+++ b/example_gui_opencl_raytracer_amd/csrc/hip_wrap_impl.h
@@ -19,6 +19,7 @@
 #include "objects_host.h"
 #include "overlay_host.h"
 #include "png_codec.h"
+#include "primary_cull_host.h"
 #include "projection_host.h"
 #include "scene_prep.h"
 #include "whitted_launch.h"
@@ -238,6 +239,18 @@
     hipStream_t sched_stream = nullptr;
     static constexpr int MAX_CHUNKS = 4;
     Sched scheds[1 + MAX_CHUNKS];
+    struct Cull {
+        unsigned char* table = nullptr; size_t bytes = 0;
+        bool valid = false;
+        wt_cull_view view{}; uint64_t scene = 0;
+        uint32_t tiles = 0;
+        bool seen = false;
+        wt_cull_view seen_view{}; uint64_t seen_scene = 0; uint32_t seen_tiles = 0;
+        uint64_t builds = 0;
+        bool last_used = false;
+        void free_all() { if (table) (void)hipFree(table); table = nullptr; bytes = 0; valid = false; last_used = false; tiles = 0; }
+    };
+    Cull culls[1 + MAX_CHUNKS];
     int pipeline = 1;
     hipStream_t copy_stream = nullptr;
     hipEvent_t chunk_done[MAX_CHUNKS] = {nullptr, nullptr, nullptr, nullptr};
diff --git a/example_gui_opencl_raytracer_amd/csrc/launch_plan.c b/example_gui_opencl_raytracer_amd/csrc/launch_plan.c
--- a/example_gui_opencl_raytracer_amd/csrc/launch_plan.c
+++ b/example_gui_opencl_raytracer_amd/csrc/launch_plan.c
@@ -277,6 +277,13 @@
     return o->status = WT_PLAN_LAUNCH;
 }
 
+int wt_plan_cull(const wt_plan_in* in, const wt_plan_out* o) {
+    if (o->status != WT_PLAN_LAUNCH || (in->variant & WT_V_NO_CULL)) return 0;
+    if (!o->fused || !o->P.tiled || o->ss != 1 || o->P.ss_lg != 0u || o->n_cams != 0u || o->motion_floats != 0u) return 0;
+    if (o->flags & (WT_F_DEEP | WT_F_GRID | WT_F_RAYS | WT_F_SS)) return 0;
+    return (uint64_t)o->trows * o->tpr < (1ull << 31);
+}
+
 wt_order_choice wt_order_choose(wt_order_state* s) {
     wt_order_choice c;
     c.rd = s->have[s->newest] ? s->newest : -1;
diff --git a/example_gui_opencl_raytracer_amd/csrc/launch_plan.h b/example_gui_opencl_raytracer_amd/csrc/launch_plan.h
--- a/example_gui_opencl_raytracer_amd/csrc/launch_plan.h
+++ b/example_gui_opencl_raytracer_amd/csrc/launch_plan.h
@@ -12,7 +12,7 @@
 
 enum { WT_V_GEOM_GLOBAL = 1, WT_V_LINEAR_IDS = 2, WT_V_NO_TILE_ORDER = 4, WT_V_NO_GRID = 8, WT_V_NO_TAIL = 16, WT_V_NO_OCC = 64,
        WT_V_NO_LPT = 128, WT_V_NO_VIS = 256, WT_V_TIMELINE = 512, WT_V_VIS_VERIFY = 1024, WT_V_FULL_STACK = 2048, WT_V_NO_SPLIT = 4096,
-       WT_V_NO_SHAPE = 8192, WT_V_UNTRIMMED = 16384 };
+       WT_V_NO_SHAPE = 8192, WT_V_UNTRIMMED = 16384, WT_V_NO_CULL = 32768 };
 
 enum {
     WT_LAUNCH_ROUND = 256,
@@ -122,6 +122,8 @@
 int wt_order_rebuild(wt_order_state* s, int sig_changed, int grid_build);
 void wt_order_launched(wt_order_state* s, int rebuilt);
 
+int wt_plan_cull(const wt_plan_in* in, const wt_plan_out* out);
+
 int wt_fast_has_trace(int flags);
 int wt_strict_has_trace(int flags);
 void wt_plan_sizes(uint32_t out[3]);
diff --git a/example_gui_opencl_raytracer_amd/csrc/primary_cull_host.c b/example_gui_opencl_raytracer_amd/csrc/primary_cull_host.c
--- /dev/null
+++ b/example_gui_opencl_raytracer_amd/csrc/primary_cull_host.c
@@ -0,0 +1,42 @@
+#include "primary_cull_host.h"
+
+#include <stdlib.h>
+#include <string.h>
+
+#include "../../include/hip_wrap_ext.h"
+#include "scene_prep.h"
+
+uint32_t wt_cull_tiles(uint32_t width, uint32_t rows) {
+    const uint64_t n = (((uint64_t)width + 7u) / 8u) * (((uint64_t)rows + 7u) / 8u);
+    return (width == 0u || rows == 0u || n >= (1ull << 31)) ? 0u : (uint32_t)n;
+}
+
+uint32_t wt_cull_table(const wt_cull_view* V, const float* spheres, uint32_t ns, const float* lights, uint32_t nl, uint8_t* out) {
+    const uint32_t n = V ? wt_cull_tiles(V->width, V->rows) : 0u;
+    if (n == 0u || !out || (ns > 0u && !spheres) || (nl > 0u && !lights)) return 0u;
+    memset(out, 0, n);
+    if (!wt_cull_view_ok(V)) return n;
+    const uint32_t tpr = (V->width + 7u) / 8u;
+    for (uint32_t t = 0; t < n; t++) out[t] = wt_cull_tile(V, t % tpr, t / tpr, spheres, ns, lights, nl);
+    return n;
+}
+
+uint32_t clw_host_primary_cull(const clw_camera* cam, uint32_t row_offset, uint32_t rows, uint32_t band_stride, uint32_t band_phase, const void* spheres,
+                               uint32_t ns, const void* lights, uint32_t nl, uint8_t* out) {
+    if (!cam || !out || (ns > 0u && !spheres) || (nl > 0u && !lights) || wt_cull_tiles(cam->width, rows) == 0u) return 0u;
+    if (band_stride > 1u && band_phase >= band_stride) return 0u;
+    wt_cull_view V;
+    memcpy(V.corner, cam->im_corner, sizeof V.corner); memcpy(V.origin, cam->origin, sizeof V.origin);
+    memcpy(V.up, cam->up, sizeof V.up); memcpy(V.right, cam->right, sizeof V.right);
+    V.w_factor = cam->w_factor; V.h_factor = cam->h_factor;
+    V.width = cam->width; V.rows = rows; V.row_offset = row_offset; V.band_stride = band_stride; V.band_phase = band_phase;
+    const size_t f4 = wprep_geom_f4(ns, 0u, nl);
+    float* geom = (float*)malloc(16 * (f4 ? f4 : 1));
+    float* ptex = (float*)malloc(32);
+    if (!geom || !ptex) { free(geom); free(ptex); return 0u; }
+    wprep_build((const uint8_t*)spheres, ns, NULL, 0u, (const uint8_t*)lights, nl, geom, ptex);
+    const uint32_t n = wt_cull_table(&V, geom, ns, geom + 4 * (size_t)ns, nl, out);
+    free(geom);
+    free(ptex);
+    return n;
+}
diff --git a/example_gui_opencl_raytracer_amd/csrc/primary_cull_host.h b/example_gui_opencl_raytracer_amd/csrc/primary_cull_host.h
--- /dev/null
+++ b/example_gui_opencl_raytracer_amd/csrc/primary_cull_host.h
@@ -0,0 +1,101 @@
+#ifndef PRIMARY_CULL_HOST_H
+#define PRIMARY_CULL_HOST_H
+#include <math.h>
+#include <stddef.h>
+#include <stdint.h>
+
+#define WT_CULL_SPHERES 1u
+#define WT_CULL_LIGHTS 2u
+#define WT_CULL_REL 1e-3
+#define WT_CULL_F32_MAX 1e37
+#define WT_CULL_COS_ABS 0.9999955000033750
+#define WT_CULL_SIN_ABS 0.0029999955000020
+
+#if defined(__HIPCC__) || defined(__CUDACC__)
+#define WT_CULL_FN static __host__ __device__ __forceinline__
+#else
+#define WT_CULL_FN static inline
+#endif
+
+typedef struct {
+    float corner[3], origin[3], up[3], right[3];
+    float w_factor, h_factor;
+    uint32_t width, rows, row_offset, band_stride, band_phase;
+} wt_cull_view;
+
+WT_CULL_FN int wt_cull_finite(double x) { return x - x == 0.0; }
+
+WT_CULL_FN int wt_cull_view_ok(const wt_cull_view* V) {
+    double s = (double)V->w_factor - (double)V->w_factor + ((double)V->h_factor - (double)V->h_factor);
+    for (int a = 0; a < 3; a++)
+        s += ((double)V->corner[a] - (double)V->corner[a]) + ((double)V->origin[a] - (double)V->origin[a]) + ((double)V->up[a] - (double)V->up[a]) +
+             ((double)V->right[a] - (double)V->right[a]);
+    return s == 0.0;
+}
+
+WT_CULL_FN void wt_cull_dir(const wt_cull_view* V, double px, double py, double v[3]) {
+    for (int a = 0; a < 3; a++)
+        v[a] = ((double)V->corner[a] + (double)V->right[a] * (double)V->w_factor * px) - (double)V->up[a] * (double)V->h_factor * py;
+}
+
+WT_CULL_FN int wt_cull_group_clear(const float* geom, uint32_t n, uint32_t stride, const double o[3], const double ax[3], double ch, double sh) {
+    for (uint32_t i = 0; i < n; i++) {
+        const float* s = geom + (size_t)stride * i;
+        const double w[3] = {(double)s[0] - o[0], (double)s[1] - o[1], (double)s[2] - o[2]};
+        const double r2 = fabs((double)s[3]);
+        const double L2 = w[0] * w[0] + w[1] * w[1] + w[2] * w[2];
+        if (!wt_cull_finite(L2) || !wt_cull_finite(r2)) return 0;
+        if (!(L2 < WT_CULL_F32_MAX) || !(r2 < WT_CULL_F32_MAX)) return 0;
+        if (!(L2 > r2 * (1.0 + WT_CULL_REL))) return 0;
+        const double L = sqrt(L2);
+        const double cphi = fabs(ax[0] * w[0] + ax[1] * w[1] + ax[2] * w[2]) / L;
+        double sa = sqrt(r2 / L2) * (1.0 + WT_CULL_REL);
+        if (!(sa < 1.0)) return 0;
+        const double ca = sqrt(1.0 - sa * sa);
+        const double c1 = ch * ca - sh * sa, s1 = sh * ca + ch * sa;
+        const double cb = c1 * WT_CULL_COS_ABS - s1 * WT_CULL_SIN_ABS;
+        if (!(c1 > 0.0 && cb > 0.0 && cphi < cb)) return 0;
+    }
+    return 1;
+}
+
+WT_CULL_FN uint8_t wt_cull_tile(const wt_cull_view* V, uint32_t tcol, uint32_t trow, const float* spheres, uint32_t ns, const float* lights, uint32_t nl) {
+    const uint32_t x0 = tcol * 8u, y0l = trow * 8u;
+    const uint32_t x1 = x0 + 7u < V->width ? x0 + 7u : V->width - 1u;
+    const uint32_t y1l = y0l + 7u < V->rows ? y0l + 7u : V->rows - 1u;
+    const double gy0 = V->band_stride > 1u ? (double)(((uint64_t)trow * V->band_stride + V->band_phase) * 8u) : (double)V->row_offset + (double)y0l;
+    const double gy1 = gy0 + (double)(y1l - y0l);
+    const double fx0 = (double)x0, fx1 = (double)x1;
+    double ax[3], u[3];
+    wt_cull_dir(V, 0.5 * (fx0 + fx1), 0.5 * (gy0 + gy1), ax);
+    const double al = sqrt(ax[0] * ax[0] + ax[1] * ax[1] + ax[2] * ax[2]);
+    if (!(al > 0.0) || !wt_cull_finite(al)) return 0;
+    for (int a = 0; a < 3; a++) ax[a] = ax[a] / al;
+    double ch = 1.0;
+    for (int k = 0; k < 4; k++) {
+        wt_cull_dir(V, (k & 1) ? fx1 : fx0, (k & 2) ? gy1 : gy0, u);
+        const double ul = sqrt(u[0] * u[0] + u[1] * u[1] + u[2] * u[2]);
+        if (!(ul > 0.0) || !wt_cull_finite(ul)) return 0;
+        const double c = (ax[0] * u[0] + ax[1] * u[1] + ax[2] * u[2]) / ul;
+        if (!(c >= 0.5)) return 0;
+        if (c < ch) ch = c;
+    }
+    double sh = sqrt(1.0 - ch * ch) * (1.0 + WT_CULL_REL);
+    if (!(sh < 1.0)) return 0;
+    ch = sqrt(1.0 - sh * sh);
+    const double o[3] = {(double)V->origin[0], (double)V->origin[1], (double)V->origin[2]};
+    uint8_t bits = 0;
+    if (wt_cull_group_clear(spheres, ns, 4u, o, ax, ch, sh)) bits |= WT_CULL_SPHERES;
+    if (wt_cull_group_clear(lights, nl, 8u, o, ax, ch, sh)) bits |= WT_CULL_LIGHTS;
+    return bits;
+}
+
+#ifdef __cplusplus
+extern "C" {
+#endif
+uint32_t wt_cull_tiles(uint32_t width, uint32_t rows);
+uint32_t wt_cull_table(const wt_cull_view* V, const float* spheres, uint32_t ns, const float* lights, uint32_t nl, uint8_t* out);
+#ifdef __cplusplus
+}
+#endif
+#endif
diff --git a/example_gui_opencl_raytracer_amd/csrc/whitted_cull.inc b/example_gui_opencl_raytracer_amd/csrc/whitted_cull.inc
--- /dev/null
+++ b/example_gui_opencl_raytracer_amd/csrc/whitted_cull.inc
@@ -0,0 +1,11 @@
+struct wt_cull_args {
+    wt_cull_view V;
+    const float* spheres; const float* lights;
+    unsigned ns, nl, tiles, tpr;
+    unsigned char* table;
+};
+__global__ void __launch_bounds__(256) wt_primary_cull_build(const wt_cull_args A) {
+    const unsigned t = blockIdx.x * 256u + threadIdx.x;
+    if (t >= A.tiles) return;
+    A.table[t] = wt_cull_tile(&A.V, t % A.tpr, t / A.tpr, A.spheres, A.ns, A.lights, A.nl);
+}
diff --git a/example_gui_opencl_raytracer_amd/csrc/whitted_hit.inc b/example_gui_opencl_raytracer_amd/csrc/whitted_hit.inc
--- a/example_gui_opencl_raytracer_amd/csrc/whitted_hit.inc
+++ b/example_gui_opencl_raytracer_amd/csrc/whitted_hit.inc
@@ -37,6 +37,7 @@
                     }
                 }
             };
+            if (!(CULL && (cullb & WT_CULL_LIGHTS)))
             for (unsigned base = 0; base < SH::nl(P); base += 4u) {
                 const unsigned left = SH::nl(P) - base;
                 if (left >= 4u) probe_chunk(wt_int<4>{}, base);
@@ -74,7 +75,7 @@
                 int best = -1;
                 if (GRID) {
                     best = wt_grid_nearest(P, r, tbest);
-                } else {
+                } else if (!(CULL && (cullb & WT_CULL_SPHERES))) {
                     for (unsigned base = 0; base < SH::ns(P); base += 4u) {
                         float4 s4[4]; float bq[4], Dq[4]; bool ok[4]; bool any = false;
 #pragma unroll
diff --git a/example_gui_opencl_raytracer_amd/csrc/whitted_launch.h b/example_gui_opencl_raytracer_amd/csrc/whitted_launch.h
--- a/example_gui_opencl_raytracer_amd/csrc/whitted_launch.h
+++ b/example_gui_opencl_raytracer_amd/csrc/whitted_launch.h
@@ -7,7 +7,8 @@
 #define WT_BOTH(ret, name, args) extern "C" ret wt_fast_##name args; extern "C" ret wt_strict_##name args;
 #define WT_FAST_ONLY(ret, name, args) extern "C" ret wt_fast_##name args;
 
-WT_BOTH(hipError_t, launch_trace, (const whitted_params* P, int flags, unsigned grid, size_t dyn_lds, hipStream_t s))
+WT_BOTH(hipError_t, launch_trace, (const whitted_params* P, const unsigned char* tile_cull, int flags, unsigned grid, size_t dyn_lds, hipStream_t s))
+WT_FAST_ONLY(hipError_t, launch_cull, (const whitted_params* P, unsigned char* table, hipStream_t s))
 WT_BOTH(int, has_trace, (int flags))
 WT_BOTH(hipError_t, launch_raygen, (const raygen_params* P, hipStream_t s))
 WT_BOTH(hipError_t, launch_raygen_proj, (const raygen_params* P, const wt_projection* T, hipStream_t s))
diff --git a/example_gui_opencl_raytracer_amd/csrc/whitted_launch.inc b/example_gui_opencl_raytracer_amd/csrc/whitted_launch.inc
--- a/example_gui_opencl_raytracer_amd/csrc/whitted_launch.inc
+++ b/example_gui_opencl_raytracer_amd/csrc/whitted_launch.inc
@@ -1,3 +1,4 @@
+#include "primary_cull_host.h"
 namespace WT_NS {
 #include "whitted_trace.inc"
 #include "whitted_gbuffer.inc"
@@ -6,15 +7,23 @@
 #include "whitted_cast.inc"
 #include "whitted_overlay.inc"
 #include "whitted_objects.inc"
+#include "whitted_cull.inc"
 }
 
 template <int FLAGS>
-static hipError_t wt_launch_one(const whitted_params* P, unsigned grid, size_t dyn_lds, hipStream_t s) {
+static hipError_t wt_launch_one(const whitted_params* P, const unsigned char* tile_cull, unsigned grid, size_t dyn_lds, hipStream_t s) {
+    if constexpr (WT_NS::wt_cull_flavour(FLAGS)) {
+        if (tile_cull) {
+            const whitted_kargs K = {*P, tile_cull};
+            hipLaunchKernelGGL(WT_NS::wt_trace_cull<FLAGS>, dim3(grid), dim3(WT_BLOCK), dyn_lds, s, K);
+            return hipGetLastError();
+        }
+    } else if (tile_cull) return hipErrorInvalidValue;
     hipLaunchKernelGGL(WT_NS::wt_trace<FLAGS>, dim3(grid), dim3(WT_BLOCK), dyn_lds, s, *P);
     return hipGetLastError();
 }
 
-typedef hipError_t (*wt_trace_launcher)(const whitted_params*, unsigned, size_t, hipStream_t);
+typedef hipError_t (*wt_trace_launcher)(const whitted_params*, const unsigned char*, unsigned, size_t, hipStream_t);
 static wt_trace_launcher wt_find_trace(int flags) {
 #if !WT_STRICT
     if (flags & WT_F_SHAPE) {
@@ -57,11 +66,26 @@
     return nullptr;
 }
 
-WT_LAUNCHER(trace)(const whitted_params* P, int flags, unsigned grid, size_t dyn_lds,
+WT_LAUNCHER(trace)(const whitted_params* P, const unsigned char* tile_cull, int flags, unsigned grid, size_t dyn_lds,
                                       hipStream_t s) {
     const wt_trace_launcher run = wt_find_trace(flags);
-    return run ? run(P, grid, dyn_lds, s) : hipErrorInvalidValue;
-}
+    return run ? run(P, tile_cull, grid, dyn_lds, s) : hipErrorInvalidValue;
+}
+
+#if !WT_STRICT
+WT_LAUNCHER(cull)(const whitted_params* P, unsigned char* table, hipStream_t s) {
+    const unsigned long long tpr = (P->width + 7ull) / 8ull, trows = (P->rows + 7ull) / 8ull;
+    if (!P->tiled || P->width == 0u || P->rows == 0u || tpr * trows >= (1ull << 31) || !table || !P->geom) return hipErrorInvalidValue;
+    WT_NS::wt_cull_args A = {};
+    for (int a = 0; a < 3; a++) { A.V.corner[a] = P->corner[a]; A.V.origin[a] = P->origin[a]; A.V.up[a] = P->up[a]; A.V.right[a] = P->right[a]; }
+    A.V.w_factor = P->w_factor; A.V.h_factor = P->h_factor;
+    A.V.width = P->width; A.V.rows = P->rows; A.V.row_offset = P->row_offset; A.V.band_stride = P->band_stride; A.V.band_phase = P->band_phase;
+    A.spheres = P->geom; A.lights = P->geom + 4 * ((size_t)P->ns + 2 * (size_t)P->np);
+    A.ns = P->ns; A.nl = P->nl; A.tiles = (unsigned)(tpr * trows); A.tpr = (unsigned)tpr; A.table = table;
+    hipLaunchKernelGGL(WT_NS::wt_primary_cull_build, dim3((A.tiles + 255u) / 256u), dim3(256), 0, s, A);
+    return hipGetLastError();
+}
+#endif
 
 extern "C" int WT_NAME(has_trace)(int flags) { return wt_find_trace(flags) != nullptr; }
 
diff --git a/example_gui_opencl_raytracer_amd/csrc/whitted_params.h b/example_gui_opencl_raytracer_amd/csrc/whitted_params.h
--- a/example_gui_opencl_raytracer_amd/csrc/whitted_params.h
+++ b/example_gui_opencl_raytracer_amd/csrc/whitted_params.h
@@ -75,6 +75,11 @@
     uint32_t seed_offset;
 } whitted_params;
 
+typedef struct {
+    whitted_params P;
+    const uint8_t* tile_cull;
+} whitted_kargs;
+
 #define WT_LIST_COUNT_STRIDE 32
 #define WT_CAM_TABLE_FLOATS (64 * 12)
 typedef struct { float v[WT_CAM_TABLE_FLOATS]; } wt_cam_table;
diff --git a/example_gui_opencl_raytracer_amd/csrc/whitted_trace.inc b/example_gui_opencl_raytracer_amd/csrc/whitted_trace.inc
--- a/example_gui_opencl_raytracer_amd/csrc/whitted_trace.inc
+++ b/example_gui_opencl_raytracer_amd/csrc/whitted_trace.inc
@@ -1074,7 +1074,8 @@
 }
 
 typedef const __attribute__((address_space(4))) whitted_params* wt_kparams_t;
-template <int FLAGS>
+constexpr bool wt_cull_flavour(int flags) { return (flags & (WT_F_DEEP | WT_F_GRID | WT_F_RAYS | WT_F_SS)) == 0; }
+template <int FLAGS, bool TABLE>
 __device__ __forceinline__ void wt_trace_body(const wt_kparams_t Pk, const unsigned wg) {
     constexpr bool COUNT = (FLAGS & WT_F_COUNT) != 0;
     constexpr bool DEEP = (FLAGS & WT_F_DEEP) != 0;
@@ -1088,6 +1089,8 @@
     constexpr bool ACC = SEEDED && !FROM_RAYS;
     constexpr bool UNIT_CT = !WT_STRICT && GEOM_LDS && !FROM_RAYS && !GRID;
     constexpr bool CLASSES = WT_STRICT != 0 && GEOM_LDS && !GRID;
+    constexpr bool CULL = TABLE && wt_cull_flavour(FLAGS);
+    static_assert(!TABLE || wt_cull_flavour(FLAGS), "no table twin of this flavour");
 
     constexpr int LDSL = wt_cfg<FLAGS>::lds_levels;
     __shared__ float s_stk[LDSL * WT_REC * WT_BLOCK];
@@ -1118,6 +1121,7 @@
     unsigned x = 0, y = 0;
     unsigned tile = 0xFFFFFFFFu;
     unsigned part_lg = 0u, part = 0u;
+    unsigned cullb = 0u;
     if (P.tiled) {
         const unsigned tpr = (P.width + 7u) >> 3;
         const unsigned b = wg;
@@ -1137,6 +1141,12 @@
         y = trow * 8u + (lane >> 3);
         valid = (tile != 0xFFFFFFFFu) && (x < P.width) && (y < P.rows) && ((lane >> (6u - part_lg)) == part);
         item = y * P.width + x;
+        if (CULL) {
+            typedef const __attribute__((address_space(1))) unsigned* wt_gwords_t;
+            const uint8_t* tc = ((const __attribute__((address_space(4))) whitted_kargs*)Pk)->tile_cull;
+            if (tc && tile != 0xFFFFFFFFu && trow * 8u < P.rows)
+                cullb = (unsigned)__builtin_amdgcn_readfirstlane((int)((((wt_gwords_t)tc)[tile >> 2] >> ((tile & 3u) * 8u)) & 3u));
+        }
     } else {
         item = wg * WT_BLOCK + tid;
         valid = item < P.n_items;
@@ -1228,6 +1238,7 @@
 #include "whitted_pop.inc"
             WT_STAMP(WT_ST_POP);
         }
+        if (CULL) cullb = 0u;
     }
     if (!TPT || __builtin_amdgcn_ballot_w64(active) == 0) break;
     {
@@ -1318,7 +1329,14 @@
 template <int FLAGS>
 __global__ void __launch_bounds__(WT_BLOCK, wt_cfg<FLAGS>::min_waves) wt_trace(const whitted_params P_arg) {
     const wt_kparams_t Pk = (wt_kparams_t)__builtin_amdgcn_kernarg_segment_ptr();
-    wt_trace_body<FLAGS>(Pk, blockIdx.x);
+    wt_trace_body<FLAGS, false>(Pk, blockIdx.x);
+}
+static_assert(__builtin_offsetof(whitted_kargs, P) == 0 && __builtin_offsetof(whitted_kargs, tile_cull) == sizeof(whitted_params) && sizeof(whitted_params) % 8 == 0,
+              "wt_trace_body<FLAGS, true> reads tile_cull behind the whitted_params its Pk points at");
+template <int FLAGS>
+__global__ void __launch_bounds__(WT_BLOCK, wt_cfg<FLAGS>::min_waves) wt_trace_cull(const whitted_kargs K_arg) {
+    const wt_kparams_t Pk = (wt_kparams_t)__builtin_amdgcn_kernarg_segment_ptr();
+    wt_trace_body<FLAGS, true>(Pk, blockIdx.x);
 }
 
 __global__ void __launch_bounds__(64) wt_cams_store(const wt_cam_table T_arg, float4* __restrict__ dst) {
@@ -1571,6 +1589,7 @@
     float* res = out + (size_t)i * stride_out;
     WT_STAMP_DECL
     constexpr bool COUNT = false, FROM_RAYS = false;
+    constexpr bool CULL = false; constexpr unsigned cullb = 0u;
     unsigned cost = 0, c_iter = 0, c_witer = 0, c_probe = 0, c_seg = 0, c_sky = 0, c_tex = 0;
     const wt_motion mv = {false, 0.0f, 0u};
     (void)lane; (void)c_iter; (void)c_witer; (void)c_probe; (void)c_seg; (void)c_sky; (void)c_tex;
diff --git a/include/hip_wrap_ext.h b/include/hip_wrap_ext.h
--- a/include/hip_wrap_ext.h
+++ b/include/hip_wrap_ext.h
@@ -214,6 +214,11 @@
 void clw_ext_set_variant(cl_wrap* wrap, int variant);
 int clw_ext_last_trace_flags(cl_wrap* wrap);
 
+struct clw_camera;
+uint32_t clw_host_primary_cull(const struct clw_camera* cam, uint32_t row_offset, uint32_t rows, uint32_t band_stride, uint32_t band_phase, const void* spheres,
+                               uint32_t ns, const void* lights, uint32_t nl, uint8_t* out);
+uint32_t clw_ext_read_primary_cull(cl_wrap* wrap, uint8_t* out, uint32_t capacity, uint64_t* builds);
+
 void clw_ext_set_tpt(cl_wrap* wrap, int max_lanes, int min_paths, int pool_mb);
 void clw_ext_get_tpt(const cl_wrap* wrap, uint32_t* max_lanes, uint32_t* min_paths, uint32_t* pool_mb);
 
```

Measured after the change: 355,200 Mrays/s, median of 6. 1.01x the previous value.
